# tchamp1912/Spittle

Measured on AMD Instinct MI355X. Metric: RTFx (audio-sec/wall-sec) Whisper-large-v3 30s chunks @1/2/4/8 MI355X, higher is better.
Workload: dtype bf16; 1 GPU; whisper-large-v3 30s chunks, batch 8/GPU, greedy en, 4-token prompt + 128 decode steps, host PCM in, text out; model=synthetic:large-v3, global_batch=8, seq_len=1500, decode_steps=128, parallelism=replicas x1 (utterance shards)

## Files before the change

include/spittle_hip.h:

```cpp
#ifndef SPITTLE_HIP_H
#define SPITTLE_HIP_H

#include <stddef.h>
#include <stdint.h>

#ifdef __cplusplus
extern "C" {
#endif

#define SPT_ABI_VERSION 14

typedef enum {
    SPT_OK = 0,
    SPT_ERR_INVALID_ARG = 1,
    SPT_ERR_LOAD = 2,
    SPT_ERR_DEVICE = 3,
    SPT_ERR_OOM = 4,
    SPT_ERR_UNSUPPORTED = 5,
    SPT_ERR_INTERNAL = 6
} spt_status;

typedef enum {
    SPT_DTYPE_F32 = 0, SPT_DTYPE_BF16 = 1,
    SPT_DTYPE_F16 = 2 ,
// ... 28 lines not shown
    const int32_t* prompt_tokens;
    int32_t n_prompt_tokens;
    float temperature_inc;
    int32_t best_of;
    float entropy_thold;
    float logprob_thold;
    float max_initial_ts;
    int32_t reserved0;
    uint64_t seed;
} spt_infer_params;

typedef struct {
    int64_t t0, t1;
    char* text;
    int32_t i0, n_tokens;
} spt_segment;

typedef struct {
    char* text;
    int32_t* tokens;
    float* top1;
    float* top2;
    int32_t n_tokens;
    int32_t n_windows;
    int32_t language;
    int32_t n_segments;
    spt_segment* segments;
    int32_t n_fallbacks;
    int32_t reserved0;
} spt_result;

typedef struct {
    int32_t n_mels, d, n_head, n_enc, n_dec, n_vocab, n_audio_ctx, n_text_ctx;
    int32_t dtype, max_batch;
    int64_t weight_bytes;
    int64_t workspace_bytes;
} spt_model_info;

typedef struct {
    double mel_ms, encoder_ms, cross_kv_ms, decode_ms, total_ms, h2d_ms;
    int32_t n_decode_passes;
    int32_t batch;
} spt_timings;

typedef struct spt_ctx spt_ctx;

const char* spt_version(void);
void spt_default_model_params(spt_model_params* p);
void spt_default_infer_params(spt_infer_params* p);

spt_status spt_ctx_create(const char* model_spec, const spt_model_params* params, spt_ctx** out,
                          char* err, size_t errlen);
void spt_ctx_destroy(spt_ctx* ctx);
const char* spt_last_error(const spt_ctx* ctx);
spt_status spt_ctx_info(const spt_ctx* ctx, spt_model_info* info);

spt_status spt_transcribe(spt_ctx* ctx, const float* pcm16k, size_t n_samples, const spt_infer_params* params,
                          spt_result** out);
spt_status spt_transcribe_batch(spt_ctx* ctx, const float* const* pcm, const size_t* n_samples, size_t batch,
                                const spt_infer_params* params, spt_result** out);
spt_status spt_transcribe_batch_device(spt_ctx* ctx, const float* pcm_dev, size_t stride, const size_t* n_samples,
                                       size_t batch, const spt_infer_params* params, spt_result** out);
void spt_result_free(spt_result* r);
const char* spt_language_code(int32_t lang_id);

spt_status spt_tokenize(spt_ctx* ctx, const char* text, int32_t* tokens, int32_t n_max, int32_t* n_out);
const char* spt_token_to_str(const spt_ctx* ctx, int32_t id);

spt_status spt_get_timings(const spt_ctx* ctx, spt_timings* t);

typedef struct {
    int32_t engine_calls;
    int32_t decoder_passes;
    int32_t beam_steps;
    int32_t encoder_windows;
    double device_ms;
    double encoder_ms;
    double decode_ms;
    int32_t pd_passes;
    int32_t pd_fallbacks;
} spt_call_stats;

spt_status spt_get_call_stats(const spt_ctx* ctx, spt_call_stats* s);

spt_status spt_weights_export(spt_ctx* ctx, void* dev_dst, size_t bytes);
spt_status spt_weights_import(spt_ctx* ctx, const void* dev_src, size_t bytes);
spt_status spt_weights_arena(spt_ctx* ctx, void** dev_ptr, size_t* bytes);
spt_status spt_weights_commit(spt_ctx* ctx);

spt_status spt_ctx_create_replicas(const char* model_spec, const spt_model_params* params, const int32_t* devices,
                                   int32_t n_devices, spt_ctx** out, double* bcast_ms, char* err, size_t errlen);
spt_status spt_transcribe_batch_replicas(spt_ctx* const* ctxs, int32_t n_ctx, const float* const* pcm,
                                         const size_t* n_samples, size_t batch, const spt_infer_params* params,
                                         spt_result** out);

typedef enum {
    SPT_PROBE_DEC_CROSS_ATTN = 0,
    SPT_PROBE_DEC_SELF_ATTN = 1,
    SPT_PROBE_DEC_LOGITS = 2,
    SPT_PROBE_DEC_FC1 = 3,
    SPT_PROBE_ENC_FC1_GEMM = 4,
    SPT_PROBE_ENC_ATTN = 5
} spt_probe_kind;
spt_status spt_probe_kernel(spt_ctx* ctx, int32_t kind, int32_t iters, double* avg_us, double* work,
                            int32_t* work_is_flops);

spt_status spt_debug_mel(spt_ctx* ctx, const float* pcm16k, size_t n_samples, float* out);
spt_status spt_debug_mel_at(spt_ctx* ctx, const float* pcm16k, size_t n_samples, int32_t seek, float* out);
spt_status spt_debug_encode(spt_ctx* ctx, const float* mel, float* out);
spt_status spt_debug_weight_checksum(spt_ctx* ctx, int32_t tensor_id, double* out2);
spt_status spt_debug_ggml_tokenize(const char* model_path, const char* text, int32_t* tokens, int32_t n_max,
                                   int32_t* n_out);
spt_status spt_debug_ggml_dequant(int32_t ggml_type, const void* src, int64_t n, float* dst);

typedef struct spt_pk_ctx spt_pk_ctx;

typedef struct {
    int32_t dtype;
    int32_t device;
    int32_t max_batch;
    float max_seconds;
    uint64_t seed;
    uint32_t flags;
    int32_t reserved0;
} spt_pk_model_params;

#define SPT_PK_WEIGHTS_EMPTY 1u

typedef enum { SPT_PK_TS_TOKEN = 0, SPT_PK_TS_WORD = 1, SPT_PK_TS_SEGMENT = 2 } spt_pk_granularity;

typedef struct {
    int32_t max_symbols;
    int32_t timestamp_granularity;
} spt_pk_infer_params;

typedef struct {
    double start, end;
    char* text;
    int32_t i0, n_tokens;
} spt_pk_segment;

typedef struct {
    char* text;
    int32_t* tokens;
    int32_t* frames;
    float* logit;
    float* runner_up;
    int32_t n_tokens;
    int32_t n_segments;
    spt_pk_segment* segments;
    int32_t n_chunks;
    int32_t reserved0;
} spt_pk_result;

typedef struct {
    int32_t n_mels, d, n_layers, n_heads, ff, sub_ch, conv_k, pred, n_vocab, n_dur;
    int32_t dtype, max_batch, max_samples, reserved0;
    int64_t weight_bytes, workspace_bytes;
} spt_pk_model_info;

typedef struct {
    double mel_ms, encoder_ms, decode_ms, total_ms, h2d_ms;
    int32_t n_steps;
    int32_t batch;
    int32_t enc_frames;
    int32_t reserved0;
// ... 236 lines not shown
```

rust/spittle-hip-sys/src/lib.rs:

```rust
#![allow(non_camel_case_types)]

use std::os::raw::{c_char, c_int, c_void};

pub const SPT_ABI_VERSION: c_int = 14;
pub const SPT_PK_STAGE_COUNT: c_int = 9;

pub type spt_status = c_int;
pub const SPT_OK: spt_status = 0;
pub const SPT_ERR_INVALID_ARG: spt_status = 1;
pub const SPT_ERR_LOAD: spt_status = 2;
pub const SPT_ERR_DEVICE: spt_status = 3;
pub const SPT_ERR_OOM: spt_status = 4;
pub const SPT_ERR_UNSUPPORTED: spt_status = 5;
pub const SPT_ERR_INTERNAL: spt_status = 6;

pub type spt_dtype = c_int;
pub const SPT_DTYPE_F32: spt_dtype = 0;
pub const SPT_DTYPE_BF16: spt_dtype = 1;
pub const SPT_DTYPE_F16: spt_dtype = 2;
pub const SPT_DTYPE_I8: spt_dtype = 3;
pub const SPT_PK_ACT_NONE: i32 = 0;
pub const SPT_PK_ACT_RELU: i32 = 1;
pub const SPT_PK_ACT_SWISH: i32 = 2;

// ... 94 lines not shown
    pub pd_fallbacks: i32,
}

#[repr(C)]
#[derive(Clone, Copy, Debug, Default)]
pub struct spt_timings {
    pub mel_ms: f64,
    pub encoder_ms: f64,
    pub cross_kv_ms: f64,
    pub decode_ms: f64,
    pub total_ms: f64,
    pub h2d_ms: f64,
    pub n_decode_passes: i32,
    pub batch: i32,
}

#[repr(C)]
pub struct spt_ctx {
    _private: [u8; 0],
}

pub type spt_probe_kind = c_int;
pub const SPT_PROBE_DEC_CROSS_ATTN: spt_probe_kind = 0;
pub const SPT_PROBE_DEC_SELF_ATTN: spt_probe_kind = 1;
pub const SPT_PROBE_DEC_LOGITS: spt_probe_kind = 2;
pub const SPT_PROBE_DEC_FC1: spt_probe_kind = 3;
pub const SPT_PROBE_ENC_FC1_GEMM: spt_probe_kind = 4;
pub const SPT_PROBE_ENC_ATTN: spt_probe_kind = 5;

extern "C" {
    pub fn spt_version() -> *const c_char;
    pub fn spt_default_model_params(p: *mut spt_model_params);
    pub fn spt_default_infer_params(p: *mut spt_infer_params);

    pub fn spt_ctx_create(
        model_spec: *const c_char,
        params: *const spt_model_params,
        out: *mut *mut spt_ctx,
        err: *mut c_char,
        errlen: usize,
    ) -> spt_status;
    pub fn spt_ctx_destroy(ctx: *mut spt_ctx);
    pub fn spt_last_error(ctx: *const spt_ctx) -> *const c_char;
    pub fn spt_ctx_info(ctx: *const spt_ctx, info: *mut spt_model_info) -> spt_status;

    pub fn spt_transcribe(
        ctx: *mut spt_ctx,
        pcm16k: *const f32,
        n_samples: usize,
        params: *const spt_infer_params,
        out: *mut *mut spt_result,
    ) -> spt_status;
    pub fn spt_transcribe_batch(
        ctx: *mut spt_ctx,
        pcm: *const *const f32,
        n_samples: *const usize,
        batch: usize,
        params: *const spt_infer_params,
        out: *mut *mut spt_result,
    ) -> spt_status;
    pub fn spt_transcribe_batch_device(
        ctx: *mut spt_ctx,
        pcm_dev: *const f32,
        stride: usize,
        n_samples: *const usize,
        batch: usize,
        params: *const spt_infer_params,
        out: *mut *mut spt_result,
    ) -> spt_status;
    pub fn spt_result_free(r: *mut spt_result);
    pub fn spt_language_code(lang_id: i32) -> *const c_char;

    pub fn spt_tokenize(
        ctx: *mut spt_ctx,
        text: *const c_char,
        tokens: *mut i32,
        n_max: i32,
        n_out: *mut i32,
    ) -> spt_status;
    pub fn spt_token_to_str(ctx: *const spt_ctx, id: i32) -> *const c_char;

    pub fn spt_get_timings(ctx: *const spt_ctx, t: *mut spt_timings) -> spt_status;
    pub fn spt_get_call_stats(ctx: *const spt_ctx, s: *mut spt_call_stats) -> spt_status;

    pub fn spt_weights_export(ctx: *mut spt_ctx, dev_dst: *mut c_void, bytes: usize) -> spt_status;
    pub fn spt_weights_import(ctx: *mut spt_ctx, dev_src: *const c_void, bytes: usize) -> spt_status;
    pub fn spt_weights_arena(ctx: *mut spt_ctx, dev_ptr: *mut *mut c_void, bytes: *mut usize) -> spt_status;
    pub fn spt_weights_commit(ctx: *mut spt_ctx) -> spt_status;

    pub fn spt_ctx_create_replicas(
        model_spec: *const c_char,
        params: *const spt_model_params,
        devices: *const i32,
        n_devices: i32,
        out: *mut *mut spt_ctx,
        bcast_ms: *mut f64,
        err: *mut c_char,
        errlen: usize,
    ) -> spt_status;
    pub fn spt_transcribe_batch_replicas(
        ctxs: *const *mut spt_ctx,
        n_ctx: i32,
        pcm: *const *const f32,
        n_samples: *const usize,
        batch: usize,
        params: *const spt_infer_params,
        out: *mut *mut spt_result,
    ) -> spt_status;

    pub fn spt_probe_kernel(
        ctx: *mut spt_ctx,
        kind: i32,
        iters: i32,
        avg_us: *mut f64,
        work: *mut f64,
        work_is_flops: *mut i32,
    ) -> spt_status;

    pub fn spt_debug_mel(ctx: *mut spt_ctx, pcm16k: *const f32, n_samples: usize, out: *mut f32) -> spt_status;
    pub fn spt_debug_mel_at(ctx: *mut spt_ctx, pcm16k: *const f32, n_samples: usize, seek: i32, out: *mut f32) -> spt_status;
    pub fn spt_debug_encode(ctx: *mut spt_ctx, mel: *const f32, out: *mut f32) -> spt_status;
    pub fn spt_debug_weight_checksum(ctx: *mut spt_ctx, tensor_id: i32, out2: *mut f64) -> spt_status;
    pub fn spt_debug_ggml_tokenize(
        model_path: *const c_char,
        text: *const c_char,
        tokens: *mut i32,
        n_max: i32,
        n_out: *mut i32,
    ) -> spt_status;
    pub fn spt_debug_ggml_dequant(ggml_type: i32, src: *const c_void, n: i64, dst: *mut f32) -> spt_status;

    pub fn spt_parakeet_default_model_params(p: *mut spt_pk_model_params);
    pub fn spt_parakeet_default_infer_params(p: *mut spt_pk_infer_params);
    pub fn spt_parakeet_create(
        model_spec: *const c_char,
        params: *const spt_pk_model_params,
        out: *mut *mut spt_pk_ctx,
        err: *mut c_char,
        errlen: usize,
    ) -> spt_status;
    pub fn spt_parakeet_destroy(ctx: *mut spt_pk_ctx);
    pub fn spt_parakeet_last_error(ctx: *const spt_pk_ctx) -> *const c_char;
    pub fn spt_parakeet_info(ctx: *const spt_pk_ctx, info: *mut spt_pk_model_info) -> spt_status;
    pub fn spt_parakeet_tensor_numel(ctx: *const spt_pk_ctx, tensor_id: i32, n: *mut i64) -> spt_status;
    pub fn spt_parakeet_set_tensor(ctx: *mut spt_pk_ctx, tensor_id: i32, data: *const f32, n: i64) -> spt_status;
    pub fn spt_parakeet_set_vocab(ctx: *mut spt_pk_ctx, pieces: *const *const c_char, n: i32) -> spt_status;
    pub fn spt_parakeet_transcribe(
        ctx: *mut spt_pk_ctx,
        pcm16k: *const f32,
        n_samples: usize,
        params: *const spt_pk_infer_params,
        out: *mut *mut spt_pk_result,
    ) -> spt_status;
    pub fn spt_parakeet_transcribe_batch(
        ctx: *mut spt_pk_ctx,
        pcm: *const *const f32,
        n_samples: *const usize,
        batch: usize,
        params: *const spt_pk_infer_params,
        out: *mut *mut spt_pk_result,
    ) -> spt_status;
    pub fn spt_parakeet_transcribe_batch_device(
        ctx: *mut spt_pk_ctx,
        pcm_dev: *const f32,
        stride: usize,
        n_samples: *const usize,
// ... 479 lines not shown
```

spittle_amd/_lib.py:

```python
from __future__ import annotations

import ctypes as C
import os

HERE = os.path.dirname(os.path.abspath(__file__))
LIB_PATH = os.path.join(HERE, "libspittle_hip.so")

SPT_OK, SPT_ERR_INVALID_ARG, SPT_ERR_LOAD, SPT_ERR_DEVICE, SPT_ERR_OOM, SPT_ERR_UNSUPPORTED, SPT_ERR_INTERNAL = range(7)
STATUS_NAMES = {0: "OK", 1: "INVALID_ARG", 2: "LOAD", 3: "DEVICE", 4: "OOM", 5: "UNSUPPORTED", 6: "INTERNAL"}
SPT_DTYPE_F32, SPT_DTYPE_BF16, SPT_DTYPE_F16, SPT_DTYPE_I8 = 0, 1, 2, 3
SPT_SUPPRESS_BLANK, SPT_NO_TIMESTAMPS, SPT_IGNORE_EOT, SPT_SUPPRESS_NST = 1, 2, 4, 8

EXPORTS = [
    "spt_version", "spt_default_model_params", "spt_default_infer_params", "spt_ctx_create",
    "spt_ctx_destroy", "spt_last_error", "spt_ctx_info", "spt_transcribe", "spt_transcribe_batch",
    "spt_transcribe_batch_device", "spt_result_free", "spt_get_timings", "spt_get_call_stats", "spt_debug_mel",
    "spt_debug_mel_at", "spt_debug_encode", "spt_debug_weight_checksum", "spt_probe_kernel", "spt_language_code",
    "spt_tokenize", "spt_token_to_str", "spt_debug_ggml_tokenize", "spt_debug_ggml_dequant",
    "spt_weights_export", "spt_weights_import", "spt_weights_arena", "spt_weights_commit",
    "spt_ctx_create_replicas", "spt_transcribe_batch_replicas",
    "spt_parakeet_default_model_params", "spt_parakeet_default_infer_params", "spt_parakeet_create",
    "spt_parakeet_destroy", "spt_parakeet_last_error", "spt_parakeet_info", "spt_parakeet_tensor_numel",
    "spt_parakeet_set_tensor", "spt_parakeet_set_vocab", "spt_parakeet_transcribe", "spt_parakeet_transcribe_batch",
    "spt_parakeet_transcribe_batch_device", "spt_parakeet_result_free", "spt_parakeet_get_timings",
    "spt_parakeet_debug_mel", "spt_parakeet_debug_encode", "spt_parakeet_debug_decode", "spt_parakeet_debug_last_encoder",
    "spt_parakeet_debug_weight_checksum", "spt_parakeet_onnx_open", "spt_parakeet_onnx_tensor",
    "spt_parakeet_onnx_piece", "spt_parakeet_onnx_close",
    "spt_resampler_create", "spt_resampler_info", "spt_resample_output_len", "spt_resample",
    "spt_resampler_last_error", "spt_resampler_destroy",
    "spt_vad_default_params", "spt_vad_create", "spt_vad_push", "spt_vad_result_free", "spt_vad_reset",
    "spt_vad_last_error", "spt_vad_destroy",
    "spt_parakeet_profile_encoder",
    "spt_parakeet_onnx_qtensor", "spt_parakeet_debug_qgemm", "spt_parakeet_debug_tap", "spt_parakeet_debug_tap_read",
    "spt_moonshine_default_model_params", "spt_moonshine_default_infer_params", "spt_moonshine_create",
    "spt_moonshine_destroy", "spt_moonshine_last_error", "spt_moonshine_info", "spt_moonshine_tensor_numel",
    "spt_moonshine_set_tensor", "spt_moonshine_missing_tensors", "spt_moonshine_set_vocab", "spt_moonshine_transcribe",
    "spt_moonshine_transcribe_batch", "spt_moonshine_result_free", "spt_moonshine_get_timings",
    "spt_moonshine_debug_stem", "spt_moonshine_debug_encode", "spt_moonshine_debug_logits",
    "spt_sensevoice_default_model_params", "spt_sensevoice_default_infer_params", "spt_sensevoice_create",
    "spt_sensevoice_destroy", "spt_sensevoice_last_error", "spt_sensevoice_info", "spt_sensevoice_tensor_numel",
    "spt_sensevoice_set_tensor", "spt_sensevoice_missing_tensors", "spt_sensevoice_set_cmvn",
    "spt_sensevoice_set_vocab", "spt_sensevoice_n_rows", "spt_sensevoice_transcribe",
    "spt_sensevoice_transcribe_batch", "spt_sensevoice_result_free", "spt_sensevoice_get_timings",
    "spt_sensevoice_debug_features", "spt_sensevoice_debug_encode", "spt_sensevoice_debug_frames",
]
SPT_SV_LANG_AUTO, SPT_SV_LANG_ZH, SPT_SV_LANG_EN, SPT_SV_LANG_YUE, SPT_SV_LANG_JA, SPT_SV_LANG_KO = range(6)
SPT_PK_WEIGHTS_EMPTY = 1
SPT_PK_TS_TOKEN, SPT_PK_TS_WORD, SPT_PK_TS_SEGMENT = 0, 1, 2
SPT_MODEL_WEIGHTS_EXTERNAL = 1
PK_STAGES = ("subsampling", "pos", "layernorm", "ffn", "qkv_out", "attn", "conv_pw", "conv_dw", "joint_enc")
PROBES = {"dec_cross_attn": 0, "dec_self_attn": 1, "dec_logits": 2, "dec_fc1": 3, "enc_fc1_gemm": 4,
          "enc_attn": 5}


class ModelParams(C.Structure):
    _fields_ = [("dtype", C.c_int32), ("device", C.c_int32), ("max_batch", C.c_int32),
                ("flags", C.c_uint32), ("seed", C.c_uint64)]


class InferParams(C.Structure):
    _fields_ = [("language", C.c_char_p), ("translate", C.c_int32), ("initial_prompt", C.c_char_p),
                ("flags", C.c_uint32), ("max_new_tokens", C.c_int32), ("temperature", C.c_float),
                ("beam_size", C.c_int32), ("forced_tokens", C.POINTER(C.c_int32)), ("n_forced", C.c_int32),
                ("prompt_tokens", C.POINTER(C.c_int32)), ("n_prompt_tokens", C.c_int32),
                ("temperature_inc", C.c_float), ("best_of", C.c_int32), ("entropy_thold", C.c_float),
                ("logprob_thold", C.c_float), ("max_initial_ts", C.c_float), ("reserved0", C.c_int32),
                ("seed", C.c_uint64)]


class Segment(C.Structure):
    _fields_ = [("t0", C.c_int64), ("t1", C.c_int64), ("text", C.c_char_p), ("i0", C.c_int32),
                ("n_tokens", C.c_int32)]


class Result(C.Structure):
    _fields_ = [("text", C.c_char_p), ("tokens", C.POINTER(C.c_int32)), ("top1", C.POINTER(C.c_float)),
                ("top2", C.POINTER(C.c_float)), ("n_tokens", C.c_int32), ("n_windows", C.c_int32),
                ("language", C.c_int32), ("n_segments", C.c_int32), ("segments", C.POINTER(Segment)),
                ("n_fallbacks", C.c_int32), ("reserved0", C.c_int32)]


class ModelInfo(C.Structure):
    _fields_ = [(n, C.c_int32) for n in ("n_mels", "d", "n_head", "n_enc", "n_dec", "n_vocab", "n_audio_ctx",
                                          "n_text_ctx", "dtype", "max_batch")] + \
               [("weight_bytes", C.c_int64), ("workspace_bytes", C.c_int64)]


class Timings(C.Structure):
    _fields_ = [(n, C.c_double) for n in ("mel_ms", "encoder_ms", "cross_kv_ms", "decode_ms", "total_ms",
                                           "h2d_ms")] + [("n_decode_passes", C.c_int32), ("batch", C.c_int32)]


class CallStats(C.Structure):
    _fields_ = [(n, C.c_int32) for n in ("engine_calls", "decoder_passes", "beam_steps", "encoder_windows")] + \
               [(n, C.c_double) for n in ("device_ms", "encoder_ms", "decode_ms")] + \
               [(n, C.c_int32) for n in ("pd_passes", "pd_fallbacks")]


class PkModelParams(C.Structure):
# ... 53 lines not shown
    _fields_ = [(n, C.c_double) for n in ("stem_ms", "encoder_ms", "cross_kv_ms", "decode_ms", "total_ms")] + \
               [("n_steps", C.c_int32), ("batch", C.c_int32)]


class SvModelParams(C.Structure):
    _fields_ = [("dtype", C.c_int32), ("device", C.c_int32), ("max_batch", C.c_int32), ("max_samples", C.c_int32),
                ("seed", C.c_uint64), ("ln_eps", C.c_float), ("sanm_shift", C.c_int32), ("lfr_m", C.c_int32),
                ("lfr_n", C.c_int32), ("blank_id", C.c_int32), ("n_prefix", C.c_int32), ("lang_rows", C.c_int32 * 6),
                ("event_row", C.c_int32), ("emo_row", C.c_int32), ("itn_row", C.c_int32), ("no_itn_row", C.c_int32)]


class SvInferParams(C.Structure):
    _fields_ = [("language", C.c_int32), ("use_itn", C.c_int32)]


class SvResult(C.Structure):
    _fields_ = [("text", C.c_char_p), ("tokens", C.POINTER(C.c_int32)), ("frames", C.POINTER(C.c_int32)),
                ("top1", C.POINTER(C.c_float)), ("top2", C.POINTER(C.c_float)), ("n_tokens", C.c_int32),
                ("prefix", C.c_int32 * 4)]


class SvModelInfo(C.Structure):
    _fields_ = [(n, C.c_int32) for n in ("d", "n_heads", "head_dim", "ff", "n_enc0_layers", "n_enc_layers",
                                          "n_tp_layers", "n_vocab", "input_dim", "dtype", "max_batch",
                                          "max_samples", "max_rows", "reserved")] + \
               [("weight_bytes", C.c_int64), ("workspace_bytes", C.c_int64)]


class SvTimings(C.Structure):
    _fields_ = [(n, C.c_double) for n in ("frontend_ms", "encoder_ms", "ctc_ms", "total_ms")] + \
               [("rows", C.c_int32), ("batch", C.c_int32)]


class VadParams(C.Structure):
    _fields_ = [("threshold", C.c_float), ("prefill_frames", C.c_int32), ("hangover_frames", C.c_int32),
                ("onset_frames", C.c_int32), ("device", C.c_int32), ("reserved0", C.c_int32)]


class VadResult(C.Structure):
    _fields_ = [("samples", C.POINTER(C.c_float)), ("n_samples", C.c_size_t), ("prob", C.POINTER(C.c_float)),
                ("kind", C.POINTER(C.c_uint8)), ("n_frames", C.c_int32), ("reserved0", C.c_int32),
                ("device_ms", C.c_double)]


_lib = None


def load():
    global _lib
    if _lib is not None:
        return _lib
    path = LIB_PATH
    if os.environ.get("SPT_DEBUG_LIB"):
        path = os.path.join(os.path.dirname(LIB_PATH), "libspittle_hip_dbg.so")
    if not os.path.exists(path):
        raise ImportError(f"spittle_amd: HIP library not built: {path} (run `make -C spittle_amd/csrc`)")
    L = C.CDLL(path)
    vp, fp = C.c_void_p, C.POINTER(C.c_float)
    L.spt_version.restype = C.c_char_p
    L.spt_default_model_params.argtypes = [C.POINTER(ModelParams)]
    L.spt_default_infer_params.argtypes = [C.POINTER(InferParams)]
    L.spt_ctx_create.argtypes = [C.c_char_p, C.POINTER(ModelParams), C.POINTER(vp), C.c_char_p, C.c_size_t]
    L.spt_ctx_create.restype = C.c_int
    L.spt_ctx_destroy.argtypes = [vp]
    L.spt_last_error.argtypes = [vp]
    L.spt_last_error.restype = C.c_char_p
    L.spt_ctx_info.argtypes = [vp, C.POINTER(ModelInfo)]
    L.spt_transcribe.argtypes = [vp, fp, C.c_size_t, C.POINTER(InferParams), C.POINTER(C.POINTER(Result))]
    L.spt_transcribe_batch.argtypes = [vp, C.POINTER(fp), C.POINTER(C.c_size_t), C.c_size_t,
                                       C.POINTER(InferParams), C.POINTER(C.POINTER(Result))]
    L.spt_transcribe_batch_device.argtypes = [vp, C.c_void_p, C.c_size_t, C.POINTER(C.c_size_t), C.c_size_t,
                                              C.POINTER(InferParams), C.POINTER(C.POINTER(Result))]
    L.spt_result_free.argtypes = [C.POINTER(Result)]
    L.spt_language_code.argtypes = [C.c_int32]
    L.spt_language_code.restype = C.c_char_p
    ip = C.POINTER(C.c_int32)
    L.spt_tokenize.argtypes = [vp, C.c_char_p, ip, C.c_int32, ip]
    L.spt_token_to_str.argtypes = [vp, C.c_int32]
    L.spt_token_to_str.restype = C.c_char_p
    L.spt_debug_ggml_tokenize.argtypes = [C.c_char_p, C.c_char_p, ip, C.c_int32, ip]
    L.spt_debug_ggml_dequant.argtypes = [C.c_int32, C.c_void_p, C.c_int64, fp]
    L.spt_get_timings.argtypes = [vp, C.POINTER(Timings)]
    L.spt_get_call_stats.argtypes = [vp, C.POINTER(CallStats)]
    L.spt_debug_mel.argtypes = [vp, fp, C.c_size_t, fp]
    L.spt_debug_mel_at.argtypes = [vp, fp, C.c_size_t, C.c_int32, fp]
    L.spt_debug_encode.argtypes = [vp, fp, fp]
    L.spt_debug_weight_checksum.argtypes = [vp, C.c_int32, C.POINTER(C.c_double)]
    L.spt_probe_kernel.argtypes = [vp, C.c_int32, C.c_int32, C.POINTER(C.c_double), C.POINTER(C.c_double),
                                   C.POINTER(C.c_int32)]
    L.spt_weights_export.argtypes = [vp, C.c_void_p, C.c_size_t]
    L.spt_weights_import.argtypes = [vp, C.c_void_p, C.c_size_t]
    L.spt_weights_arena.argtypes = [vp, C.POINTER(vp), C.POINTER(C.c_size_t)]
    L.spt_weights_commit.argtypes = [vp]
    L.spt_ctx_create_replicas.argtypes = [C.c_char_p, C.POINTER(ModelParams), C.POINTER(C.c_int32), C.c_int32,
                                          C.POINTER(vp), C.POINTER(C.c_double), C.c_char_p, C.c_size_t]
    L.spt_transcribe_batch_replicas.argtypes = [C.POINTER(vp), C.c_int32, C.POINTER(fp), C.POINTER(C.c_size_t),
                                                C.c_size_t, C.POINTER(InferParams), C.POINTER(C.POINTER(Result))]
    PR = C.POINTER(C.POINTER(PkResult))
    L.spt_parakeet_default_model_params.argtypes = [C.POINTER(PkModelParams)]
    L.spt_parakeet_default_infer_params.argtypes = [C.POINTER(PkInferParams)]
    L.spt_parakeet_create.argtypes = [C.c_char_p, C.POINTER(PkModelParams), C.POINTER(vp), C.c_char_p, C.c_size_t]
    L.spt_parakeet_onnx_open.argtypes = [C.c_char_p, C.POINTER(vp), C.POINTER(PkModelInfo), C.c_char_p, C.c_size_t]
    L.spt_parakeet_onnx_tensor.restype = C.c_int64
    L.spt_parakeet_onnx_tensor.argtypes = [vp, C.c_int32, C.POINTER(C.POINTER(C.c_float))]
    L.spt_parakeet_onnx_qtensor.restype = C.c_int64
    L.spt_parakeet_onnx_qtensor.argtypes = [vp, C.c_int32, C.POINTER(C.POINTER(C.c_int16)), C.POINTER(fp),
                                            C.POINTER(C.POINTER(C.c_int32)), C.POINTER(C.c_int32)]
    L.spt_parakeet_onnx_piece.restype = C.c_char_p
    L.spt_parakeet_onnx_piece.argtypes = [vp, C.c_int32]
    L.spt_parakeet_onnx_close.argtypes = [vp]
    L.spt_parakeet_destroy.argtypes = [vp]
    L.spt_parakeet_last_error.argtypes = [vp]
    L.spt_parakeet_last_error.restype = C.c_char_p
    L.spt_parakeet_info.argtypes = [vp, C.POINTER(PkModelInfo)]
    L.spt_parakeet_tensor_numel.argtypes = [vp, C.c_int32, C.POINTER(C.c_int64)]
    L.spt_parakeet_set_tensor.argtypes = [vp, C.c_int32, fp, C.c_int64]
    L.spt_parakeet_set_vocab.argtypes = [vp, C.POINTER(C.c_char_p), C.c_int32]
    L.spt_parakeet_transcribe.argtypes = [vp, fp, C.c_size_t, C.POINTER(PkInferParams), PR]
    L.spt_parakeet_transcribe_batch.argtypes = [vp, C.POINTER(fp), C.POINTER(C.c_size_t), C.c_size_t,
                                                C.POINTER(PkInferParams), PR]
    L.spt_parakeet_transcribe_batch_device.argtypes = [vp, C.c_void_p, C.c_size_t, C.POINTER(C.c_size_t), C.c_size_t,
                                                       C.POINTER(PkInferParams), PR]
    L.spt_parakeet_result_free.argtypes = [C.POINTER(PkResult)]
    L.spt_parakeet_get_timings.argtypes = [vp, C.POINTER(PkTimings)]
    L.spt_parakeet_profile_encoder.argtypes = [vp, C.c_int32, C.POINTER(C.c_double), C.c_int32]
    L.spt_parakeet_debug_mel.argtypes = [vp, fp, C.c_size_t, fp]
    L.spt_parakeet_debug_encode.argtypes = [vp, fp, C.c_int32, fp]
    L.spt_parakeet_debug_decode.argtypes = [vp, fp, C.c_int32, C.c_int32, PR]
    L.spt_parakeet_debug_last_encoder.argtypes = [vp, C.c_int32, fp, C.POINTER(C.c_int32)]
    L.spt_parakeet_debug_weight_checksum.argtypes = [vp, C.c_int32, C.POINTER(C.c_double)]
    i32p = C.POINTER(C.c_int32)
    L.spt_parakeet_debug_qgemm.argtypes = [C.c_int32, fp, C.c_int32, C.c_int32, i32p, C.c_int32, C.POINTER(C.c_int16),
                                           C.c_int32, fp, i32p, C.c_int32, fp, C.c_int32, C.POINTER(C.c_uint8), fp, i32p,
                                           i32p, fp, C.c_char_p, C.c_size_t]
    L.spt_parakeet_debug_tap.argtypes = [vp, C.c_int32]
    L.spt_parakeet_debug_tap_read.argtypes = [vp, i32p, fp, C.c_int64, fp, C.c_int64]
    L.spt_resampler_create.argtypes = [C.c_int32, C.c_int32, C.c_int32, C.c_int32, C.POINTER(vp), C.c_char_p,
                                       C.c_size_t]
    L.spt_resampler_create.restype = C.c_int
    L.spt_resampler_info.argtypes = [vp, C.POINTER(C.c_int32), C.POINTER(C.c_int32)]
    L.spt_resampler_info.restype = C.c_int
    L.spt_resample_output_len.argtypes = [vp, C.c_size_t]
    L.spt_resample_output_len.restype = C.c_size_t
    L.spt_resample.argtypes = [vp, fp, C.c_size_t, fp, C.c_size_t, C.POINTER(C.c_size_t)]
    L.spt_resample.restype = C.c_int
    L.spt_resampler_last_error.argtypes = [vp]
    L.spt_resampler_last_error.restype = C.c_char_p
    L.spt_resampler_destroy.argtypes = [vp]
    L.spt_resampler_destroy.restype = None
    L.spt_vad_default_params.argtypes = [C.POINTER(VadParams)]
    L.spt_vad_default_params.restype = None
    L.spt_vad_create.argtypes = [C.c_char_p, C.POINTER(VadParams), C.POINTER(vp), C.c_char_p, C.c_size_t]
    L.spt_vad_create.restype = C.c_int
    L.spt_vad_push.argtypes = [vp, fp, C.c_size_t, C.POINTER(C.POINTER(VadResult))]
    L.spt_vad_push.restype = C.c_int
    L.spt_vad_result_free.argtypes = [C.POINTER(VadResult)]
    L.spt_vad_result_free.restype = None
    L.spt_vad_reset.argtypes = [vp, C.c_int32]
    L.spt_vad_reset.restype = C.c_int
    L.spt_vad_last_error.argtypes = [vp]
    L.spt_vad_last_error.restype = C.c_char_p
    L.spt_vad_destroy.argtypes = [vp]
    L.spt_vad_destroy.restype = None
    MR = C.POINTER(C.POINTER(MsResult))
    L.spt_moonshine_default_model_params.argtypes = [C.POINTER(MsModelParams)]
    L.spt_moonshine_default_model_params.restype = None
    L.spt_moonshine_default_infer_params.argtypes = [C.POINTER(MsInferParams)]
    L.spt_moonshine_default_infer_params.restype = None
    L.spt_moonshine_create.argtypes = [C.c_char_p, C.POINTER(MsModelParams), C.POINTER(vp), C.c_char_p, C.c_size_t]
    L.spt_moonshine_destroy.argtypes = [vp]
    L.spt_moonshine_destroy.restype = None
    L.spt_moonshine_last_error.argtypes = [vp]
    L.spt_moonshine_last_error.restype = C.c_char_p
    L.spt_moonshine_info.argtypes = [vp, C.POINTER(MsModelInfo)]
    L.spt_moonshine_tensor_numel.argtypes = [vp, C.c_char_p, C.POINTER(C.c_int64)]
    L.spt_moonshine_set_tensor.argtypes = [vp, C.c_char_p, fp, C.c_int64]
    L.spt_moonshine_missing_tensors.argtypes = [vp]
    L.spt_moonshine_missing_tensors.restype = C.c_int32
    L.spt_moonshine_set_vocab.argtypes = [vp, C.POINTER(C.c_char_p), C.c_int32]
    L.spt_moonshine_transcribe.argtypes = [vp, fp, C.c_size_t, C.POINTER(MsInferParams), MR]
    L.spt_moonshine_transcribe_batch.argtypes = [vp, C.POINTER(fp), C.POINTER(C.c_size_t), C.c_size_t,
                                                 C.POINTER(MsInferParams), MR]
    L.spt_moonshine_result_free.argtypes = [C.POINTER(MsResult)]
    L.spt_moonshine_result_free.restype = None
    L.spt_moonshine_get_timings.argtypes = [vp, C.POINTER(MsTimings)]
    L.spt_moonshine_debug_stem.argtypes = [vp, fp, C.c_size_t, fp]
    L.spt_moonshine_debug_encode.argtypes = [vp, fp, C.c_size_t, fp]
    L.spt_moonshine_debug_logits.argtypes = [vp, fp, C.c_size_t, i32p, C.c_int32, fp]
    for fn in ("spt_moonshine_create", "spt_moonshine_info", "spt_moonshine_tensor_numel", "spt_moonshine_set_tensor",
               "spt_moonshine_set_vocab", "spt_moonshine_transcribe", "spt_moonshine_transcribe_batch",
               "spt_moonshine_get_timings", "spt_moonshine_debug_stem", "spt_moonshine_debug_encode",
               "spt_moonshine_debug_logits"):
        getattr(L, fn).restype = C.c_int
    SR = C.POINTER(C.POINTER(SvResult))
    svip = C.POINTER(SvInferParams)
    L.spt_sensevoice_default_model_params.argtypes = [C.POINTER(SvModelParams)]
    L.spt_sensevoice_default_model_params.restype = None
    L.spt_sensevoice_default_infer_params.argtypes = [svip]
    L.spt_sensevoice_default_infer_params.restype = None
    L.spt_sensevoice_create.argtypes = [C.c_char_p, C.POINTER(SvModelParams), C.POINTER(vp), C.c_char_p, C.c_size_t]
    L.spt_sensevoice_destroy.argtypes = [vp]
    L.spt_sensevoice_destroy.restype = None
    L.spt_sensevoice_last_error.argtypes = [vp]
    L.spt_sensevoice_last_error.restype = C.c_char_p
    L.spt_sensevoice_info.argtypes = [vp, C.POINTER(SvModelInfo)]
    L.spt_sensevoice_tensor_numel.argtypes = [vp, C.c_char_p, C.POINTER(C.c_int64)]
    L.spt_sensevoice_set_tensor.argtypes = [vp, C.c_char_p, fp, C.c_int64]
    L.spt_sensevoice_missing_tensors.argtypes = [vp]
    L.spt_sensevoice_missing_tensors.restype = C.c_int32
    L.spt_sensevoice_set_cmvn.argtypes = [vp, fp, fp, C.c_int32]
    L.spt_sensevoice_set_vocab.argtypes = [vp, C.POINTER(C.c_char_p), C.c_int32]
    L.spt_sensevoice_n_rows.argtypes = [vp, C.c_size_t]
    L.spt_sensevoice_n_rows.restype = C.c_int32
    L.spt_sensevoice_transcribe.argtypes = [vp, fp, C.c_size_t, svip, SR]
    L.spt_sensevoice_transcribe_batch.argtypes = [vp, C.POINTER(fp), C.POINTER(C.c_size_t), C.c_size_t, svip, SR]
    L.spt_sensevoice_result_free.argtypes = [C.POINTER(SvResult)]
    L.spt_sensevoice_result_free.restype = None
    L.spt_sensevoice_get_timings.argtypes = [vp, C.POINTER(SvTimings)]
    L.spt_sensevoice_debug_features.argtypes = [vp, fp, C.c_size_t, fp]
    L.spt_sensevoice_debug_encode.argtypes = [vp, fp, C.c_size_t, svip, fp]
    L.spt_sensevoice_debug_frames.argtypes = [vp, fp, C.c_size_t, svip, i32p, fp, fp]
    for fn in ("spt_sensevoice_create", "spt_sensevoice_info", "spt_sensevoice_tensor_numel", "spt_sensevoice_set_tensor",
               "spt_sensevoice_set_cmvn", "spt_sensevoice_set_vocab", "spt_sensevoice_transcribe",
               "spt_sensevoice_transcribe_batch", "spt_sensevoice_get_timings", "spt_sensevoice_debug_features",
               "spt_sensevoice_debug_encode", "spt_sensevoice_debug_frames"):
        getattr(L, fn).restype = C.c_int
    for fn in EXPORTS:
        if fn.startswith("spt_parakeet_") and fn not in ("spt_parakeet_default_model_params",
                                                          "spt_parakeet_default_infer_params", "spt_parakeet_destroy",
                                                          "spt_parakeet_last_error", "spt_parakeet_result_free",
                                                          "spt_parakeet_onnx_tensor", "spt_parakeet_onnx_piece",
                                                          "spt_parakeet_onnx_close", "spt_parakeet_onnx_qtensor"):
            getattr(L, fn).restype = C.c_int
    for fn in ("spt_weights_arena", "spt_weights_commit", "spt_ctx_create_replicas", "spt_transcribe_batch_replicas",
               "spt_weights_export", "spt_weights_import", "spt_ctx_info", "spt_transcribe", "spt_transcribe_batch", "spt_transcribe_batch_device",
               "spt_get_timings", "spt_get_call_stats", "spt_debug_mel", "spt_debug_mel_at", "spt_debug_encode", "spt_debug_weight_checksum",
               "spt_probe_kernel", "spt_tokenize", "spt_debug_ggml_tokenize", "spt_debug_ggml_dequant"):
        getattr(L, fn).restype = C.c_int
    _lib = L
    return L
```

spittle_amd/csrc/capi.cpp:

```cpp
#include <hip/hip_runtime.h>
#include <string.h>

#include <algorithm>
#include <memory>
#include <new>
#include <string>
#include <vector>

#include "../../include/spittle_hip.h"
#include "common.h"
#include "engine.h"
#include "full.h"
#include "ggml_file.h"
#include "vocab.h"

using spt::Engine;

#include "capi_internal.h"

namespace {

constexpr int kWindow = 480000;

void set_err(char* buf, size_t len, const std::string& msg) {
// ... 495 lines not shown
        std::vector<int> ns(batch);
        if (autolang) {
            rq.lang_tok.resize(batch);
            for (size_t b = 0; b < batch; ++b) rq.lang_tok[b] = -(int)(b + 1);
        }
        for (size_t b = 0; b < batch; ++b) {
            if (n_samples[b] > (size_t)kWindow) return fail(ctx, SPT_ERR_INVALID_ARG, "device windows hold <= 480000 samples");
            ns[b] = (int)n_samples[b];
        }
        Engine& e = *ctx->eng;
        const int B = (int)batch;
        std::vector<int> otok((size_t)B * rq.n_steps), lang(B, -1);
        std::vector<float> o1((size_t)B * rq.n_steps), o2((size_t)B * rq.n_steps);
        e.transcribe_device(pcm_dev, (int64_t)stride, ns.data(), B, rq, otok.data(), o1.data(), o2.data(), lang.data());
        const spt::Specials sp = spt::specials_for(e.dims().n_vocab);
        const int eot = sp.eot;
        for (int b = 0; b < B; ++b) {
            std::vector<int> t; std::vector<float> a, c2; std::string txt;
            for (int s2 = 0; s2 < rq.n_steps; ++s2) {
                const int tk = otok[(size_t)b * rq.n_steps + s2];
                if (tk < 0) break;
                t.push_back(tk);
                a.push_back(o1[(size_t)b * rq.n_steps + s2]);
                c2.push_back(o2[(size_t)b * rq.n_steps + s2]);
                if (tk < eot) append_text(ctx, &txt, tk);
                if (tk == eot && !(rq.flags & SPT_IGNORE_EOT)) break;
            }
            out[b] = make_result(1, lang_index(lang[b], sp), &t, &a, &c2, &txt);
        }
        return SPT_OK;
    } catch (const std::exception& e) {
        return fail(ctx, classify(e), e.what());
    }
}

void spt_result_free(spt_result* r) {
    if (!r) return;
    for (int32_t i = 0; i < r->n_segments && r->segments; ++i) free(r->segments[i].text);
    free(r->segments);
    free(r->text);
    free(r->tokens);
    free(r->top1);
    free(r->top2);
    free(r);
}

spt_status spt_tokenize(spt_ctx* ctx, const char* text, int32_t* tokens, int32_t n_max, int32_t* n_out) {
    if (!ctx || !text || !n_out || (n_max > 0 && !tokens)) return fail(ctx, SPT_ERR_INVALID_ARG, "null argument");
    if (!ctx->vocab) return fail(ctx, SPT_ERR_UNSUPPORTED, "synthetic models have no vocabulary");
    try {
        const std::vector<int> t = ctx->vocab->tokenize(text, nullptr);
        *n_out = (int32_t)t.size();
        if ((int64_t)t.size() > n_max) return fail(ctx, SPT_ERR_INVALID_ARG, "token buffer too small");
        for (size_t i = 0; i < t.size(); ++i) tokens[i] = t[i];
        return SPT_OK;
    } catch (const std::exception& e) {
        return fail(ctx, classify(e), e.what());
    }
}

const char* spt_token_to_str(const spt_ctx* ctx, int32_t id) {
    if (!ctx || !ctx->vocab || id < 0 || id >= ctx->vocab->size()) return nullptr;
    return ctx->vocab->str(id).c_str();
}

spt_status spt_get_timings(const spt_ctx* ctx, spt_timings* t) {
    if (!ctx || !t) return SPT_ERR_INVALID_ARG;
    const spt::Timings& m = ctx->eng->timings();
    t->mel_ms = m.mel_ms; t->encoder_ms = m.encoder_ms; t->cross_kv_ms = m.cross_kv_ms; t->decode_ms = m.decode_ms;
    t->total_ms = m.total_ms; t->h2d_ms = m.h2d_ms; t->n_decode_passes = m.n_decode_passes; t->batch = m.batch;
    return SPT_OK;
}

spt_status spt_get_call_stats(const spt_ctx* ctx, spt_call_stats* s) {
    if (!ctx || !s) return SPT_ERR_INVALID_ARG;
    const spt::CallStats& c = ctx->eng->call_stats();
    s->engine_calls = c.engine_calls; s->decoder_passes = c.decoder_passes; s->beam_steps = c.beam_steps;
    s->encoder_windows = c.encoder_windows;
    s->device_ms = c.device_ms; s->encoder_ms = c.encoder_ms; s->decode_ms = c.decode_ms;
    s->pd_passes = c.pd_passes; s->pd_fallbacks = c.pd_fallbacks;
    return SPT_OK;
}

spt_status spt_weights_export(spt_ctx* ctx, void* dev_dst, size_t bytes) {
    if (!ctx || !dev_dst) return fail(ctx, SPT_ERR_INVALID_ARG, "null argument");
    try {
        ctx->eng->export_weights(dev_dst, (int64_t)bytes);
        return SPT_OK;
    } catch (const std::exception& e) {
        return fail(ctx, classify(e), e.what());
    }
}

spt_status spt_weights_import(spt_ctx* ctx, const void* dev_src, size_t bytes) {
    if (!ctx || !dev_src) return fail(ctx, SPT_ERR_INVALID_ARG, "null argument");
    try {
        ctx->eng->import_weights(dev_src, (int64_t)bytes);
        return SPT_OK;
    } catch (const std::exception& e) {
        return fail(ctx, classify(e), e.what());
    }
}

spt_status spt_debug_mel(spt_ctx* ctx, const float* pcm16k, size_t n_samples, float* out) {
    if (!ctx || !out || (n_samples && !pcm16k)) return fail(ctx, SPT_ERR_INVALID_ARG, "null argument");
    if (n_samples > (size_t)kWindow) return fail(ctx, SPT_ERR_INVALID_ARG, "window longer than 30 s");
    return spt_debug_mel_at(ctx, pcm16k, n_samples, 0, out);
}

spt_status spt_debug_mel_at(spt_ctx* ctx, const float* pcm16k, size_t n_samples, int32_t seek, float* out) {
    if (!ctx || !out || (n_samples && !pcm16k)) return fail(ctx, SPT_ERR_INVALID_ARG, "null argument");
    if (n_samples > (size_t)INT32_MAX / 2) return fail(ctx, SPT_ERR_INVALID_ARG, "utterance too long");
    try {
        ctx->eng->debug_mel(pcm16k, (int)n_samples, seek, out);
        return SPT_OK;
    } catch (const std::exception& e) {
        return fail(ctx, classify(e), e.what());
    }
}

spt_status spt_debug_encode(spt_ctx* ctx, const float* mel, float* out) {
    if (!ctx || !mel || !out) return fail(ctx, SPT_ERR_INVALID_ARG, "null argument");
    try {
        ctx->eng->debug_encode(mel, out);
        return SPT_OK;
    } catch (const std::exception& e) {
        return fail(ctx, classify(e), e.what());
    }
}

spt_status spt_debug_weight_checksum(spt_ctx* ctx, int32_t tensor_id, double* out2) {
    if (!ctx || !out2) return fail(ctx, SPT_ERR_INVALID_ARG, "null argument");
    try {
        if (!ctx->eng->debug_weight_checksum(tensor_id, out2)) return fail(ctx, SPT_ERR_INVALID_ARG, "unknown tensor id");
        return SPT_OK;
    } catch (const std::exception& e) {
        return fail(ctx, classify(e), e.what());
    }
}

spt_status spt_debug_ggml_tokenize(const char* model_path, const char* text, int32_t* tokens, int32_t n_max,
                                   int32_t* n_out) {
    if (!model_path || !text || !n_out || (n_max > 0 && !tokens)) return SPT_ERR_INVALID_ARG;
    spt::GgmlFile f;
    std::string err;
    if (!f.open(model_path, &err)) return SPT_ERR_LOAD;
    spt::Vocab v(f.vocab(), f.hparams().n_vocab, spt::specials_for(f.hparams().n_vocab));
    const std::vector<int> t = v.tokenize(text, nullptr);
    *n_out = (int32_t)t.size();
    if ((int64_t)t.size() > n_max) return SPT_ERR_INVALID_ARG;
    for (size_t i = 0; i < t.size(); ++i) tokens[i] = t[i];
    return SPT_OK;
}

spt_status spt_debug_ggml_dequant(int32_t ggml_type, const void* src, int64_t n, float* dst) {
    if (!src || !dst || n < 0) return SPT_ERR_INVALID_ARG;
    int blck, bytes;
    spt::GgmlFile::type_block(ggml_type, &blck, &bytes);
    if (!blck) return SPT_ERR_UNSUPPORTED;
    if (n % blck) return SPT_ERR_INVALID_ARG;
    return spt::ggml_dequant_host(ggml_type, (const uint8_t*)src, n, dst) ? SPT_OK : SPT_ERR_UNSUPPORTED;
}

}

extern "C" spt_status spt_probe_kernel(spt_ctx* ctx, int32_t kind, int32_t iters, double* avg_us, double* work,
// ... 12 lines not shown
```

spittle_amd/csrc/dec_attn.h:

```cpp
#pragma once
#include "common.h"

namespace spt {
namespace {

constexpr int AW = 8;
constexpr float kLog2Scale = 0.125f * 1.4426950408889634f;

template <typename T> struct KVChunk;
template <> struct KVChunk<bf16> {
    bf16x8 v;
    __device__ __forceinline__ void load(const bf16* p) { v = *(const bf16x8*)p; }
    __device__ __forceinline__ float at(int e) const { return bf2f((bf16)v[e]); }
};
template <> struct KVChunk<f16> {
    f16x8 v;
    __device__ __forceinline__ void load(const f16* p) { v = *(const f16x8*)p; }
    __device__ __forceinline__ float at(int e) const { return (float)v[e]; }
};
template <> struct KVChunk<float> {
    f32x4 a, b;
    __device__ __forceinline__ void load(const float* p) { a = *(const f32x4*)p; b = *(const f32x4*)(p + 4); }
    __device__ __forceinline__ float at(int e) const { return e < 4 ? a[e] : b[e - 4]; }
};
// ... 47 lines not shown
                for (int e = 0; e < 8; ++e) v = __builtin_fmaf(qv[t][e], kc[i].at(e), v);
                v += __shfl_xor(v, 1, 64);
                v += __shfl_xor(v, 2, 64);
                v += __shfl_xor(v, 4, 64);
                if (kbase + 8 * i + slot >= lim[t]) v = -INFINITY;
                s[i] = v;
                mb = fmaxf(mb, v);
            }
            mb = fmaxf(mb, __shfl_xor(mb, 8, 64));
            mb = fmaxf(mb, __shfl_xor(mb, 16, 64));
            mb = fmaxf(mb, __shfl_xor(mb, 32, 64));
            if (mb == -INFINITY) continue;
            const float mn = fmaxf(m[t], mb);
            const float alpha = exp2f(m[t] - mn);
            float ls = 0.f;
#pragma unroll
            for (int e = 0; e < 8; ++e) o[t][e] *= alpha;
#pragma unroll
            for (int i = 0; i < NI; ++i) {
                const float p = exp2f(s[i] - mn);
                ls += p;
#pragma unroll
                for (int e = 0; e < 8; ++e) o[t][e] = __builtin_fmaf(p, vc[i].at(e), o[t][e]);
            }
            l[t] = __builtin_fmaf(l[t], alpha, ls);
            m[t] = mn;
        }
    }
    template <int MAXB>
    __device__ __forceinline__ void run(int blk, int nblk, const float (&qv)[NQ][8], const int (&lim)[NQ], int Tq) {
        if (blk >= nblk) return;
        const int cnt = (nblk - 1 - blk) / NW + 1;
        const int mine = blk + (cnt - 1) * NW;
        if (MAXB <= 8 && cnt <= MAXB) {
#pragma unroll
            for (int d = 0; d < PF - 1 && d < MAXB; ++d) load_blk(kc_[d], vc_[d], min(blk + d * NW, mine));
#pragma unroll
            for (int i = 0; i < (MAXB <= 8 ? MAXB : 1); ++i) {
                if (i >= cnt) break;
                if (i + PF - 1 < (MAXB <= 8 ? MAXB : 1))
                    load_blk(kc_[(i + PF - 1) % PF], vc_[(i + PF - 1) % PF], min(blk + (i + PF - 1) * NW, mine));
                process(kc_[i % PF], vc_[i % PF], (blk + i * NW) * KB, qv, lim, Tq);
            }
            return;
        }
        load_blk(kc_[0], vc_[0], blk);
        while (blk < nblk) {
            load_blk(kc_[1], vc_[1], min(blk + NW, mine));
            process(kc_[0], vc_[0], blk * KB, qv, lim, Tq);
            blk += NW;
            if (blk >= nblk) break;
            load_blk(kc_[0], vc_[0], min(blk + NW, mine));
            process(kc_[1], vc_[1], blk * KB, qv, lim, Tq);
            blk += NW;
        }
    }
    template <int MAXB>
    __device__ __forceinline__ void run_pre(int blk, int nblk, const float (&qv)[NQ][8], const int (&lim)[NQ], int Tq) {
        if (blk >= nblk) return;
        const int cnt = (nblk - 1 - blk) / NW + 1;
        const int mine = blk + (cnt - 1) * NW;
        if (MAXB <= 8 && cnt <= MAXB) {
#pragma unroll
            for (int d = 1; d < PF - 1 && d < MAXB; ++d) load_blk(kc_[d], vc_[d], min(blk + d * NW, mine));
#pragma unroll
            for (int i = 0; i < (MAXB <= 8 ? MAXB : 1); ++i) {
                if (i >= cnt) break;
                if (i + PF - 1 < (MAXB <= 8 ? MAXB : 1))
                    load_blk(kc_[(i + PF - 1) % PF], vc_[(i + PF - 1) % PF], min(blk + (i + PF - 1) * NW, mine));
                process(kc_[i % PF], vc_[i % PF], (blk + i * NW) * KB, qv, lim, Tq);
            }
            return;
        }
        while (blk < nblk) {
            load_blk(kc_[1], vc_[1], min(blk + NW, mine));
            process(kc_[0], vc_[0], blk * KB, qv, lim, Tq);
            blk += NW;
            if (blk >= nblk) break;
            load_blk(kc_[0], vc_[0], min(blk + NW, mine));
            process(kc_[1], vc_[1], blk * KB, qv, lim, Tq);
            blk += NW;
        }
    }
    __device__ __forceinline__ void to_lds(float (*s_m)[NQ], float (*s_l)[NQ], float (*s_o)[NQ][64], int wid,
                                           int lane) {
        const int g = lane & 7;
#pragma unroll
        for (int t = 0; t < NQ; ++t) {
            float lt = l[t];
            lt += __shfl_xor(lt, 8, 64);
            lt += __shfl_xor(lt, 16, 64);
            lt += __shfl_xor(lt, 32, 64);
#pragma unroll
            for (int e = 0; e < 8; ++e) {
                float v = o[t][e];
                v += __shfl_xor(v, 8, 64);
                v += __shfl_xor(v, 16, 64);
                v += __shfl_xor(v, 32, 64);
                o[t][e] = v;
            }
            if (lane < 8) {
#pragma unroll
                for (int e = 0; e < 8; ++e) s_o[wid][t][8 * g + e] = o[t][e];
            }
            if (lane == 0) {
                s_m[wid][t] = m[t];
                s_l[wid][t] = lt;
            }
        }
    }
};

template <int NQ, int NW = AW>
__device__ __forceinline__ void attn_merge(const float (*s_m)[NQ], const float (*s_l)[NQ], const float (*s_o)[NQ][64],
                                           int t, int e, float& M, float& L, float& O) {
#pragma clang fp contract(off)
    M = -INFINITY;
#pragma unroll
    for (int w = 0; w < NW; ++w) M = fmaxf(M, s_m[w][t]);
    L = 0.f;
    O = 0.f;
#pragma unroll
    for (int w = 0; w < NW; ++w) {
        if (s_m[w][t] == -INFINITY) continue;
        const float f = exp2f(s_m[w][t] - M);
        L = __builtin_fmaf(s_l[w][t], f, L);
        O = __builtin_fmaf(s_o[w][t][e], f, O);
    }
}

}
}
```

spittle_amd/csrc/engine.cpp:

```cpp
#include "engine.h"
#include "ggml_file.h"

#include <cstdio>

#include <math.h>
#include <string.h>

#include <algorithm>
#include <functional>
#include <cstdlib>
#include <sstream>
#include <stdexcept>

#include "common.h"

namespace spt {

bool parse_synthetic_spec(const std::string& spec, ModelDims* dm, uint64_t* seed, std::string* err) {
    const std::string pfx = "synthetic:";
    if (spec.compare(0, pfx.size(), pfx) != 0) return false;
    std::vector<std::string> parts;
    std::stringstream ss(spec.substr(pfx.size()));
    std::string tok;
    while (std::getline(ss, tok, ':')) parts.push_back(tok);
    if (parts.empty()) { *err = "empty synthetic spec"; return true; }
    struct Cfg { const char* name; int n_mels, d, h, ne, nd, V; };
    static const Cfg cfgs[] = {
        {"tiny.en", 80, 384, 6, 4, 4, 51864},     {"tiny", 80, 384, 6, 4, 4, 51865},
        {"base.en", 80, 512, 8, 6, 6, 51864},     {"base", 80, 512, 8, 6, 6, 51865},
        {"small.en", 80, 768, 12, 12, 12, 51864}, {"small", 80, 768, 12, 12, 12, 51865},
        {"medium.en", 80, 1024, 16, 24, 24, 51864}, {"medium", 80, 1024, 16, 24, 24, 51865},
        {"large-v3", 128, 1280, 20, 32, 32, 51866}, {"large-v3-turbo", 128, 1280, 20, 32, 4, 51866},
    };
    bool found = false;
    for (const Cfg& c : cfgs)
        if (parts[0] == c.name) {
            dm->name = c.name;
            dm->n_mels = c.n_mels; dm->d = c.d; dm->n_head = c.h; dm->n_enc = c.ne; dm->n_dec = c.nd;
            dm->n_vocab = c.V;
            found = true;
        }
    if (!found) { *err = "unknown synthetic model '" + parts[0] + "'"; return true; }
    for (size_t i = 1; i < parts.size(); ++i) {
        const std::string& p = parts[i];
        const size_t eq = p.find('=');
        if (eq == std::string::npos) { *err = "bad option '" + p + "'"; return true; }
        const std::string k = p.substr(0, eq), v = p.substr(eq + 1);
        char* end = nullptr;
        const unsigned long long x = strtoull(v.c_str(), &end, 10);
        if (!end || *end) { *err = "bad value in '" + p + "'"; return true; }
        if (k == "enc") dm->n_enc = (int)x;
        else if (k == "dec") dm->n_dec = (int)x;
        else if (k == "seed") *seed = (uint64_t)x;
        else { *err = "unknown option '" + k + "'"; return true; }
    }
    if (dm->n_enc < 0 || dm->n_dec < 1 || dm->n_enc > 64 || dm->n_dec > 64) *err = "layer count out of range";
    return true;
}

namespace {
int fanin_exp(int K) { return (int)floor(log2(sqrt(3.0 / (double)K)) + 0.5); }

struct Carver {
    char* base;
    int64_t off = 0;
    void* take(int64_t bytes) {
        off = (off + 255) & ~(int64_t)255;
        void* p = base ? base + off : nullptr;
        off += bytes;
        return p;
    }
};
}

void Engine::select() const { HIP_CHECK(hipSetDevice(dev_)); }

Engine::Engine(const ModelDims& dm, int dtype, int device, int max_batch, uint64_t seed, const GgmlFile* src,
               bool external_weights)
    : dm_(dm), dt_(dtype), dev_(device), max_batch_(max_batch), seed_(seed) {
    if (dm_.d % 128 || dm_.d / 64 != dm_.n_head) throw std::runtime_error("unsupported model width");
    if (max_batch_ < 1 || max_batch_ > 64) throw std::runtime_error("max_batch must be in 1..64");
    if (dt_ == DT_F32 && dm_.d > 1024)
        throw std::runtime_error("the f32 engine supports model widths up to 1024 (tiny..medium); load " +
                                 std::to_string(dm_.d) + "-wide models in bf16");
    if (dt_ != DT_F32 && dt_ != DT_BF16 && dt_ != DT_F16) throw std::runtime_error("unsupported engine dtype");
    esz_ = dtype_size(dt_);
    cp_ = ((dm_.n_mels + 63) / 64) * 64;
    if ((3 * cp_ * esz_) % 128) cp_ = ((dm_.n_mels + 127) / 128) * 128;
    if (const char* g = getenv("SPT_DECODE_GROUPS")) n_groups_ = std::max(1, std::min(4, atoi(g)));
    if (const char* v = getenv("SPT_XATTN_SPLIT")) xsplit_ = std::max(1, std::min(4, atoi(v)));
    select();
    HIP_CHECK(hipStreamCreateWithFlags(&st_, hipStreamNonBlocking));
    ev_.resize(12);
    for (auto& e : ev_) HIP_CHECK(hipEventCreate(&e));
    enc_st_.assign(kEncGroupsMax - 1, nullptr);
    for (auto& s : enc_st_) HIP_CHECK(hipStreamCreateWithFlags(&s, hipStreamNonBlocking));
    enc_ev_.assign(kEncGroupsMax, nullptr);
    for (auto& e : enc_ev_) HIP_CHECK(hipEventCreateWithFlags(&e, hipEventDisableTiming));
    max_rows_ = gemv_max_image_rows(dt_, dm_.d);
    groups_.resize(std::max(n_groups_, cdiv(max_batch_, max_rows_)));
    for (auto& g : groups_) {
        HIP_CHECK(hipStreamCreateWithFlags(&g.st, hipStreamNonBlocking));
        HIP_CHECK(hipEventCreateWithFlags(&g.ev, hipEventDisableTiming));
    }
    try {
        gemv_prepare(dt_);
        gemm_prepare();
        alloc_weights();
        if (external_weights) {
            HIP_CHECK(hipMemsetAsync(warena_, 0, wbytes_, st_));
        } else if (src) {
            load_ggml(*src);
        } else {
            generate_weights();
        }
        weights_ready_ = !external_weights;
        upload_tables(src ? &src->mel_filters() : nullptr);
        alloc_workspace();
        HIP_CHECK(hipStreamSynchronize(st_));
    } catch (...) {
        release();
        throw;
    }
}

Engine::~Engine() { release(); }

void Engine::release() {
    (void)hipSetDevice(dev_);
    if (st_) (void)hipStreamSynchronize(st_);
    for (auto& g : groups_) {
        if (g.st) (void)hipStreamSynchronize(g.st);
        for (auto& kv : g.graphs) (void)hipGraphExecDestroy(kv.second);
        if (g.ev) (void)hipEventDestroy(g.ev);
        if (g.st) (void)hipStreamDestroy(g.st);
    }
    for (auto& kv : enc_graphs_) (void)hipGraphExecDestroy(kv.second);
    enc_graphs_.clear();
    for (auto& s : enc_st_)
        if (s) {
            (void)hipStreamSynchronize(s);
            (void)hipStreamDestroy(s);
        }
    enc_st_.clear();
    for (auto& e : enc_ev_)
        if (e) (void)hipEventDestroy(e);
    enc_ev_.clear();
    if (warena_) (void)hipFree(warena_);
    if (aarena_) (void)hipFree(aarena_);
    if (kvtmp_) (void)hipFree(kvtmp_);
    for (void* p : {(void*)upcm_, (void*)umel_, (void*)uinfo_})
        if (p) (void)hipFree(p);
    upcm_ = umel_ = nullptr;
    uinfo_ = nullptr;
    upcm_cap_ = umel_cap_ = 0;
    uinfo_cap_ = 0;
    for (void* p : {(void*)hann_, (void*)sinv_, (void*)cosv_, (void*)filt_, (void*)grp_})
        if (p) (void)hipFree(p);
    for (auto& e : ev_) (void)hipEventDestroy(e);
    for (auto& e : probe_ev_) (void)hipEventDestroy(e);
    probe_ev_.clear();
    if (st_) (void)hipStreamDestroy(st_);
    groups_.clear();
    ev_.clear();
    warena_ = aarena_ = nullptr;
    kvtmp_ = nullptr;
    hann_ = sinv_ = cosv_ = filt_ = nullptr;
    grp_ = nullptr;
    st_ = nullptr;
}

void Engine::require_weights() const {
    if (!weights_ready_)
        throw std::runtime_error("weights not loaded: the context was created with SPT_MODEL_WEIGHTS_EXTERNAL and "
                                 "spt_weights_import has not been called");
}

void Engine::export_weights(void* dev_dst, int64_t bytes) {
    require_weights();
    if (!dev_dst || bytes != wbytes_)
        throw std::runtime_error("weight export: expected " + std::to_string(wbytes_) + " bytes, got " +
                                 std::to_string(bytes));
    select();
    HIP_CHECK(hipMemcpyAsync(dev_dst, warena_, (size_t)wbytes_, hipMemcpyDeviceToDevice, st_));
    HIP_CHECK(hipStreamSynchronize(st_));
}

void Engine::import_weights(const void* dev_src, int64_t bytes) {
    if (!dev_src || bytes != wbytes_)
        throw std::runtime_error("weight import: expected " + std::to_string(wbytes_) + " bytes (this model and dtype), got " +
                                 std::to_string(bytes));
    select();
    HIP_CHECK(hipMemcpyAsync(warena_, dev_src, (size_t)wbytes_, hipMemcpyDeviceToDevice, st_));
    HIP_CHECK(hipStreamSynchronize(st_));
    weights_ready_ = true;
}

void Engine::commit_weights() {
    select();
    HIP_CHECK(hipDeviceSynchronize());
    weights_ready_ = true;
}

void Engine::alloc_weights() {
    const int64_t d = dm_.d, dd = d * d, V = dm_.n_vocab, L = dm_.n_dec;
    enc_.resize(dm_.n_enc);
    dec_.resize(dm_.n_dec);
    for (int pass = 0; pass < 2; ++pass) {
        Carver c{pass ? warena_ : nullptr};
        auto W = [&](int64_t n) { return c.take(n * esz_); };
        auto F = [&](int64_t n) { return (float*)c.take(n * 4); };
        conv1_w_ = W(d * 3 * cp_); conv1_b_ = F(d);
        conv2_w_ = W(dd * 3); conv2_b_ = F(d);
        enc_pos_ = F((int64_t)dm_.n_audio_ctx * d);
        lnp_w_ = F(d); lnp_b_ = F(d);
        for (auto& e : enc_) {
// ... 255 lines not shown
void Engine::upload_tables(const std::vector<float>* filters) {
    std::vector<float> hann(400), sv(400), cv(400);
    for (int i = 0; i < 400; ++i) {
        const double theta = (2 * M_PI * i) / 400;
        sv[i] = sinf((float)theta);
        cv[i] = cosf((float)theta);
        hann[i] = (float)(0.5 * (1.0 - cosf((float)((2.0 * M_PI * i) / 400))));
    }
    const int nm = dm_.n_mels;
    auto hz2mel = [](double f) {
        const double lg = 27.0 / log(6.4);
        return f >= 1000.0 ? 15.0 + log(f / 1000.0) * lg : 3.0 * f / 200.0;
    };
    auto mel2hz = [](double m) {
        const double lg = log(6.4) / 27.0;
        return m >= 15.0 ? 1000.0 * exp(lg * (m - 15.0)) : 200.0 * m / 3.0;
    };
    std::vector<double> ff(nm + 2);
    const double mmin = hz2mel(0.0), mmax = hz2mel(8000.0);
    for (int i = 0; i < nm + 2; ++i) {
        double mm = mmin + (mmax - mmin) * i / (double)(nm + 1);
        if (i == nm + 1) mm = mmax;
        ff[i] = mel2hz(mm);
    }
    std::vector<float> filt((size_t)nm * 201);
    std::vector<int> grp(2 * nm);
    if (filters) filt = *filters;
    for (int j = 0; j < nm; ++j) {
        const double en = 2.0 / (ff[j + 2] - ff[j]);
        int lo = -1, hi = -1;
        for (int k = 0; k < 201; ++k) {
            if (!filters) {
                const double fk = 8000.0 * k / 200.0;
                const double down = -(ff[j] - fk) / (ff[j + 1] - ff[j]);
                const double up = (ff[j + 2] - fk) / (ff[j + 2] - ff[j + 1]);
                double v = std::min(down, up);
                if (v < 0) v = 0;
                filt[(size_t)j * 201 + k] = (float)(v * en);
            }
            const float fv = filt[(size_t)j * 201 + k];
            if (fv != 0.0f) {
                if (lo < 0) lo = k;
                hi = k;
            }
        }
        if (lo < 0) { grp[2 * j] = 0; grp[2 * j + 1] = 0; }
        else {
            grp[2 * j] = lo < 200 ? lo / 4 : 50;
            grp[2 * j + 1] = (hi < 200 ? hi / 4 : 50) + 1;
        }
    }
    HIP_CHECK(hipMalloc(&hann_, 400 * 4));
    HIP_CHECK(hipMalloc(&sinv_, 400 * 4));
    HIP_CHECK(hipMalloc(&cosv_, 400 * 4));
    HIP_CHECK(hipMalloc(&filt_, filt.size() * 4));
    HIP_CHECK(hipMalloc(&grp_, grp.size() * 4));
    HIP_CHECK(hipMemcpy(hann_, hann.data(), 1600, hipMemcpyHostToDevice));
    HIP_CHECK(hipMemcpy(sinv_, sv.data(), 1600, hipMemcpyHostToDevice));
    HIP_CHECK(hipMemcpy(cosv_, cv.data(), 1600, hipMemcpyHostToDevice));
    HIP_CHECK(hipMemcpy(filt_, filt.data(), filt.size() * 4, hipMemcpyHostToDevice));
    HIP_CHECK(hipMemcpy(grp_, grp.data(), grp.size() * 4, hipMemcpyHostToDevice));
}

void Engine::alloc_workspace() {
    const int64_t B = max_batch_, d = dm_.d, T = dm_.n_audio_ctx, L = dm_.n_dec, ctx = dm_.n_text_ctx;
    const int64_t V = dm_.n_vocab, R = B * 4;
    for (int pass = 0; pass < 2; ++pass) {
        Carver c{pass ? aarena_ : nullptr};
        auto A = [&](int64_t n) { return c.take(n * esz_); };
        win_utt_ = (int*)c.take(B * 4);
        win_seek_ = (int*)c.take(B * 4);
        mel_in_ = A(B * MEL_ROWS * cp_);
        y1p_ = A(B * MEL_ROWS * d);
        x_ = (float*)c.take(B * T * d * 4);
        xn_ = A(B * T * d);
        qkv_ = A(B * T * 3 * d);
        ao_ = A(B * T * d);
        ff_ = A(B * T * 4 * d);
        enc_out_ = A(B * T * d);
        ckv_ = A(L * kv_layer_elems((int)B, dm_.n_head, (int)T));
        suppress_ = (uint32_t*)c.take((V / 32 + 1) * 4);
        suppress_lang_ = (uint32_t*)c.take((V / 32 + 1) * 4);
        scratch_ = (double*)c.take(64);
        for (DecGroup& g : groups_) {
            g.dx = (float*)c.take(R * d * 4);
            g.dq = A(R * d);
            g.dao = A(R * d);
            g.dff = A(R * 4 * d);
            g.skv = A(L * 2 * B * ctx * d);
            g.logits = (float*)c.take(B * V * 4);
            g.part = c.take(B * ((V + 15) / 16) * 16);
            g.arrive = (unsigned*)c.take(64);
            g.tok_in = (int*)c.take(R * 4);
            g.out_tok = (int*)c.take(B * ctx * 4);
            g.out_t1 = (float*)c.take(B * ctx * 4);
            g.out_t2 = (float*)c.take(B * ctx * 4);
            g.done = (int*)c.take(B * 4);
            g.forced = (int*)c.take(B * ctx * 4);
            g.ds = (DecState*)c.take(sizeof(DecState));
            g.dx2 = (float*)c.take(R * d * 4);
            g.pend = (float*)c.take((int64_t)kMaxPend * R * d * 4);
            g.xpart = (float*)c.take((int64_t)R * dm_.n_head * 8 * 66 * 4);
            g.seek = (int*)c.take(B * 4);
            g.seek_end = (int*)c.take(B * 4);
            g.ts_state = (int*)c.take(B * 16);
            g.ts_stat = (float*)c.take((int64_t)B * TS_CHUNKS * 6 * 4);
            g.beam_stat = (float*)c.take((int64_t)B * TS_CHUNKS * BEAM_STAT * 4);
            g.prm = (TsParams*)c.take(sizeof(TsParams));
            g.beam_row = (int*)c.take(B * 16);
            g.beam_step = (int*)c.take(64);
            g.beam_src = (int*)c.take(B * 4);
            g.cand_id = (int*)c.take(B * 8 * 4);
            g.cand_lp = (float*)c.take(B * 8 * 4);
            g.beam_tid = (int*)c.take(B * 4);
            g.kvrow = (int*)c.take(B * 4);
        }
        zero_ = (float*)c.take(R * d * 4);
        if (!pass) {
            abytes_ = c.off;
            if (hipMalloc(&aarena_, abytes_) != hipSuccess) {
                aarena_ = nullptr;
                throw std::runtime_error("out of device memory for workspace (" + std::to_string(abytes_) + " B)");
            }
        }
    }
    HIP_CHECK(hipMemsetAsync(aarena_, 0, abytes_, st_));
}

void Engine::ensure_capacity(void** p, int64_t* cap, int64_t need, size_t esz, const char* what) {
    if (need <= *cap) return;
    const int64_t want = std::max<int64_t>(need, *cap + *cap / 4);
    HIP_CHECK(hipDeviceSynchronize());
    if (*p) HIP_CHECK(hipFree(*p));
    *p = nullptr;
    *cap = 0;
    if (hipMalloc(p, (size_t)want * esz) != hipSuccess) {
        *p = nullptr;
        (void)hipGetLastError();
        throw std::runtime_error(std::string("out of device memory for ") + what + " (" +
                                 std::to_string((size_t)want * esz) + " B)");
    }
    *cap = want;
}

void Engine::run_mel_utts(const float* pcm, const std::vector<int64_t>& pcm_off, const int* n, int U) {
    if (U < 1) throw std::runtime_error("no utterances");
    int64_t rows = 0;
    int max_rows = 0;
    uhost_.assign((size_t)U * 3, 0);
    for (int u = 0; u < U; ++u) {
        if (n[u] < 0) throw std::runtime_error("negative sample count");
        const int r = mel_rows(n[u]);
        uhost_[u] = pcm_off[u];
        uhost_[U + u] = rows;
        rows += r;
        max_rows = std::max(max_rows, r);
    }
    void* pm = umel_;
    ensure_capacity(&pm, &umel_cap_, std::max<int64_t>(rows, 1), (size_t)dm_.n_mels * 4, "the utterance log-mel");
    umel_ = (float*)pm;
    const int64_t info_bytes = (int64_t)U * 24;
    if (U > uinfo_cap_) {
        int64_t cap = uinfo_cap_ ? (int64_t)uinfo_cap_ * 24 : 0;
        void* pi = uinfo_;
        ensure_capacity(&pi, &cap, info_bytes, 1, "utterance descriptors");
        uinfo_ = (char*)pi;
        uinfo_cap_ = (int)(cap / 24);
    }
    mel_img_.assign((size_t)info_bytes, 0);
    memcpy(mel_img_.data(), uhost_.data(), (size_t)U * 16);
    for (int u = 0; u < U; ++u) memcpy(mel_img_.data() + (size_t)U * 16 + 4 * u, &n[u], 4);
    HIP_CHECK(hipMemcpyAsync(uinfo_, mel_img_.data(), (size_t)U * 20, hipMemcpyHostToDevice, st_));
    mu_.pcm_off = (const int64_t*)uinfo_;
    mu_.row_off = (const int64_t*)(uinfo_ + (size_t)U * 8);
    mu_.n = (const int*)(uinfo_ + (size_t)U * 16);
    umax_ = (unsigned*)(uinfo_ + (size_t)U * 20);
    un_.assign(n, n + U);
    HIP_CHECK(hipEventRecord(ev_[0], st_));
    MelTables t{hann_, sinv_, cosv_, filt_, grp_};
    mel_frames(pcm, mu_, U, max_rows, dm_.n_mels, t, umel_, umax_, st_);
    HIP_CHECK(hipEventRecord(ev_[1], st_));
    mel_pending_ = true;
    enc_E_ = 0;
}

void Engine::load_utterances(const float* const* pcm, const int* n, int U) {
    select();
    require_weights();
    std::vector<int64_t> off(U);
    int64_t tot = 0;
    for (int u = 0; u < U; ++u) {
        if (n[u] < 0) throw std::runtime_error("negative sample count");
        if (n[u] > 0 && !pcm[u]) throw std::runtime_error("null pcm");
        off[u] = tot;
        tot += n[u];
    }
    void* pp = upcm_;
    ensure_capacity(&pp, &upcm_cap_, std::max<int64_t>(tot, 1), 4, "utterance PCM");
// ... 110 lines not shown
    gemm_nt(dt_, EPI_BIAS_GELU_POS, g, B, st_);
    const int G = enc_groups(B);
    int b0[kEncGroupsMax + 1];
    for (int i = 0; i <= G; ++i) b0[i] = (int)((int64_t)B * i / G);
    auto stream_of = [&](int i) { return i == 0 ? st_ : enc_st_[i - 1]; };
    if (G > 1) {
        HIP_CHECK(hipEventRecord(enc_ev_[0], st_));
        for (int i = 1; i < G; ++i) HIP_CHECK(hipStreamWaitEvent(stream_of(i), enc_ev_[0], 0));
    }
    auto rows = [&](void* base, int64_t row, int64_t ld, int es) { return (char*)base + row * ld * es; };
    enc_groups_cur_ = G;
    for (int l = 0; l < dm_.n_enc; ++l)
        for (int i = 0; i < G; ++i)
            enc_layer(l, b0[i + 1] - b0[i], (int64_t)b0[i] * T, stream_of(i));
    for (int i = 0; i < G; ++i) {
        const int64_t r0 = (int64_t)b0[i] * T;
        layernorm(dt_, (float*)rows(x_, r0, d, 4), (b0[i + 1] - b0[i]) * T, d, lnp_w_, lnp_b_,
                  rows(enc_out_, r0, d, esz_), stream_of(i));
    }
    for (int i = 1; i < G; ++i) {
        HIP_CHECK(hipEventRecord(enc_ev_[i], stream_of(i)));
        HIP_CHECK(hipStreamWaitEvent(st_, enc_ev_[i], 0));
    }
}

int Engine::enc_groups(int B) const {
    int G = B >= 8 ? 2 : 1;
    if (const char* v = getenv("SPT_ENC_GROUPS")) G = atoi(v);
    return std::max(1, std::min({G, kEncGroupsMax, B}));
}

void Engine::enqueue_encoder(int B) {
    static const bool eager = getenv("SPT_NO_GRAPH") || (getenv("SPT_ENC_GRAPH") && atoi(getenv("SPT_ENC_GRAPH")) == 0);
    const std::pair<int, int> key{B, enc_groups(B)};
    if (eager || !enc_seen_.count(key)) {
        enc_seen_.insert(key);
        run_encoder(B);
        return;
    }
    auto it = enc_graphs_.find(key);
    if (it == enc_graphs_.end()) {
        hipGraph_t graph;
        HIP_CHECK(hipStreamBeginCapture(st_, hipStreamCaptureModeThreadLocal));
        try {
            run_encoder(B);
        } catch (...) {
            (void)hipStreamEndCapture(st_, &graph);
            throw;
        }
        HIP_CHECK(hipStreamEndCapture(st_, &graph));
        hipGraphExec_t exec;
        HIP_CHECK(hipGraphInstantiate(&exec, graph, nullptr, nullptr, 0));
        HIP_CHECK(hipGraphDestroy(graph));
        it = enc_graphs_.emplace(key, exec).first;
    }
    HIP_CHECK(hipGraphLaunch(it->second, st_));
}

void Engine::run_cross_kv(int B) {
    const int d = dm_.d, T = dm_.n_audio_ctx;
    GemmArgs g{};
    g.A = enc_out_; g.lda = d; g.W = ckv_w_; g.ldw = d; g.M = B * T; g.N = dm_.n_dec * 2 * d; g.K = d;
    g.bias = ckv_b_; g.C = ckv_; g.kv_B = B; g.kv_T = T; g.kv_H = dm_.n_head;
    gemm_nt(dt_, EPI_KVSPLIT, g, 1, st_);
}

void Engine::enqueue_decoder_pass(DecGroup& g, int E, int Tq, const DecodeRequest& rq, int out_cap) {
    float* x = enqueue_layers(g, E, Tq);
    enqueue_head(g, Tq, rq, out_cap, x, suppress_, (rq.flags & 1u) != 0);
}

float* Engine::enqueue_layers(DecGroup& g, int E, int Tq) {
    const int d = dm_.d, H = dm_.n_head, ctx = dm_.n_text_ctx, T = dm_.n_audio_ctx, B = g.B, R = B * Tq;
    const int64_t self_layer = (int64_t)2 * B * H * ctx * 64, cross_layer = kv_layer_elems(E, H, T);
    const bool mapped = g.share > 0;
    const int runs = B / std::max(1, g.share);
    const int vw_env = getenv("SPT_XATTN_VW") ? atoi(getenv("SPT_XATTN_VW")) : 1;
    const bool vw = vw_env == 2 || (vw_env != 0 && runs * H < 96);
    const bool per_query = vw && Tq == 1 && vw_env != 3;
    const bool vw_merge = vw && R > 1;
    const int xs = vw ? (vw_merge ? 1 : 8) : mapped ? 1 : xsplit_;
    const int ks = esz_ == 2 ? 128 : 64;
    hipStream_t st = g.st;
    float* xc = g.dx;
    float* xo = g.dx2;
    int np = 0;
    pend_fold_ = !getenv("SPT_DEC_XFOLD") || atoi(getenv("SPT_DEC_XFOLD")) != 0;
    auto ln_input = [&](GemvArgs& a) {
        ln_source(a, xc, g.pend, np, (int64_t)R * d);
        a.x_out = np > 0 ? xo : nullptr;
    };
    auto consumed = [&] {
        if (np > 0) std::swap(xc, xo);
        np = 0;
    };
    auto pmark = [&](int kind, int l, int which) {
        if (probe_kind_ == kind) HIP_CHECK(hipEventRecord(probe_ev_[2 * l + which], st));
    };
    auto partial = [&](GemvArgs& a, int split) {
        a.C = g.pend; a.ldc = d; a.c_split = (int64_t)R * d;
        a.ksplit = split;
        a.p_resid = pend_fold_ ? xc : nullptr;
        if (a.K / ks < split) throw std::runtime_error("decoder projection too narrow for its K split");
        np = split;
    };
    for (int l = 0; l < dm_.n_dec; ++l) {
        const DecL& e = dec_[l];
        void* skv_l = (char*)g.skv + self_layer * l * esz_;
        const void* ckv_l = (const char*)ckv_ + (cross_layer * l + (mapped ? 0 : (int64_t)g.b0 * H * 4096)) * esz_;
        {
            GemvArgs a{};
            ln_input(a); a.lda = d; a.ln_w = e.ln1_w; a.ln_b = e.ln1_b; a.R = R;
            a.W = e.qkv_w; a.N = 3 * d; a.K = d; a.bias = e.qkv_b; a.C = g.dq; a.ldc = d;
            a.cache = skv_l; a.cache_B = B; a.cache_H = H; a.cache_ctx = ctx; a.Tq = Tq; a.st = g.ds;
            gemv(dt_, GV_QKV_CACHE, A_LN, a, st);
            consumed();
            pmark(1, l, 0);
            dec_self_attn(dt_, g.dq, skv_l, B, H, ctx, Tq, g.ds, g.dao, st);
            pmark(1, l, 1);
        }
        GemvArgs a{};
        a.A = g.dao; a.lda = d; a.R = R; a.W = e.so_w; a.N = d; a.K = d; a.bias = e.so_b;
        a.C = xc; a.ldc = d;
        gemv(dt_, GV_BIAS_RESID, A_DIRECT, a, st);
        a = GemvArgs{};
        ln_input(a); a.lda = d; a.ln_w = e.ln2_w; a.ln_b = e.ln2_b; a.R = R;
        a.W = e.cq_w; a.N = d; a.K = d; a.bias = e.cq_b; a.C = g.dq; a.ldc = d;
        gemv(dt_, GV_BIAS, A_LN, a, st);
        consumed();
        pmark(0, l, 0);
        if (vw)
        {
            dec_cross_attn_vw(dt_, g.dq, ckv_l, B, E, H, T, Tq, g.xpart, st, mapped ? g.kvrow : nullptr,
                              mapped ? g.share : 1, per_query);
            if (vw_merge) dec_attn_part_merge(dt_, g.xpart, R, H, g.dao, st);
        }
        else
            dec_cross_attn(dt_, g.dq, ckv_l, B, E, H, T, Tq, g.dao, st, xs, g.xpart, mapped ? g.kvrow : nullptr,
                           mapped ? g.share : 1);
        pmark(0, l, 1);
        a = GemvArgs{};
        a.A = g.dao; a.lda = d; a.R = R; a.W = e.co_w; a.N = d; a.K = d; a.bias = e.co_b; a.C = xc; a.ldc = d;
        if (xs > 1) { a.apart = g.xpart; a.a_splits = xs; a.a_heads = H; }
        gemv(dt_, GV_BIAS_RESID, xs > 1 ? A_ATTN : A_DIRECT, a, st);
        a = GemvArgs{};
        ln_input(a); a.lda = d; a.ln_w = e.ln3_w; a.ln_b = e.ln3_b; a.R = R;
        a.W = e.fc1_w; a.N = 4 * d; a.K = d; a.bias = e.fc1_b; a.C = g.dff; a.ldc = 4 * d;
        pmark(3, l, 0);
        gemv(dt_, GV_BIAS_GELU, A_LN, a, st);
        pmark(3, l, 1);
        consumed();
        a = GemvArgs{};
        a.A = g.dff; a.lda = 4 * d; a.R = R; a.W = e.fc2_w; a.N = d; a.K = 4 * d; a.bias = e.fc2_b;
        partial(a, fc2_split_);
        gemv(dt_, GV_PARTIAL, A_DIRECT, a, st);
    }
    return xc;
}

void Engine::ln_source(GemvArgs& a, float* xc, float* pend, int np, int64_t slab) const {
    const int f = np > 0 && pend_fold_ ? 1 : 0;
    a.A = f ? pend : xc;
    for (int p = 0; p < kMaxPend; ++p) a.pend[p] = p < np - f ? pend + (int64_t)(p + f) * slab : zero_;
    a.n_pend = np - f;
}

void Engine::enqueue_head(DecGroup& g, int Tq, const DecodeRequest& rq, int out_cap, float* xc,
                          const uint32_t* sup, bool blank) {
    const int d = dm_.d, ctx = dm_.n_text_ctx, B = g.B, R = B * Tq;
    hipStream_t st = g.st;
    const Specials sp = specials_for(dm_.n_vocab);
    const int n_tiles = (dm_.n_vocab + 15) / 16;
    GemvArgs a{};
    ln_source(a, xc, g.pend, fc2_split_, (int64_t)R * d);
    a.lda = Tq * d; a.a_row0 = (Tq - 1) * d; a.ln_w = lnf_w_; a.ln_b = lnf_b_; a.R = B;
    a.W = tok_emb_; a.N = dm_.n_vocab; a.K = d; a.C = g.logits; a.ldc = dm_.n_vocab; a.st = g.ds;
    a.suppress = sup;
    a.blank0 = blank ? sp.eot : -1;
    a.blank1 = blank ? 220 : -1;
    a.part = g.part; a.n_tiles = n_tiles;
    gemv(dt_, GV_LOGITS, A_LN, a, st);
    if (rq.beam_k > 0) {
        BeamArgs bm{};
        bm.logits = g.logits; bm.ldl = dm_.n_vocab;
        bm.n_vocab = dm_.n_vocab; bm.eot = sp.eot; bm.beg = sp.beg; bm.blank = rq.blank_tok;
        bm.suppress = sup; bm.prm = g.prm; bm.row = g.beam_row; bm.step = g.beam_step; bm.k = rq.beam_k;
        bm.cand_id = g.cand_id; bm.cand_lp = g.cand_lp; bm.tid = g.beam_tid;
        static const bool one_wg = getenv("SPT_BEAM_ONE_WG") != nullptr;
        bm.stat = one_wg ? nullptr : g.beam_stat;
        dec_beam_topk(bm, B, st);
        dec_advance(g.ds, Tq, st);
        return;
    }
    if (rq.full) {
        TsArgs t{};
        t.logits = g.logits; t.ldl = dm_.n_vocab;
        t.n_vocab = dm_.n_vocab; t.eot = sp.eot; t.beg = sp.beg; t.blank = rq.blank_tok;
        t.suppress = sup; t.prm = g.prm; t.seek = g.seek; t.seek_end = g.seek_end; t.state = g.ts_state;
        t.forced = rq.n_forced > 0 ? g.forced : nullptr; t.forced_len = rq.n_forced;
        t.next_tok = g.tok_in; t.out_tok = g.out_tok; t.out_plog = g.out_t1; t.out_tid = g.out_t2; t.out_cap = out_cap;
        t.done = g.done;
        t.emb = tok_emb_; t.pos = dec_pos_; t.d = d; t.ctx = ctx; t.Tq = Tq; t.x = g.dx;
        t.ds = g.ds; t.arrive = g.arrive; t.stat = g.ts_stat;
        dec_ts_stats(t, B, st);
        dec_finalize_ts(dt_, t, B, st);
        return;
    }
    FinalizeArgs f{};
    f.part = g.part; f.n_tiles = n_tiles;
    f.eot = sp.eot; f.ignore_eot = (rq.flags & 4u) ? 1 : 0; f.n_vocab = dm_.n_vocab;
    f.forced = rq.n_forced > 0 ? g.forced : nullptr; f.forced_len = rq.n_forced;
    f.next_tok = g.tok_in; f.out_tok = g.out_tok; f.out_top1 = g.out_t1; f.out_top2 = g.out_t2; f.out_cap = out_cap;
    f.done = g.done;
    f.emb = tok_emb_; f.pos = dec_pos_; f.d = d; f.ctx = ctx; f.Tq = Tq; f.x = g.dx;
    f.ds = g.ds; f.arrive = g.arrive;
// ... 52 lines not shown
    const uint32_t sflags = (rq.flags & 2u) | (rq.full ? 0x100u : 0u);
    if (suppress_flags_ != sflags || suppress_extra_ != rq.extra_suppress) {
        const int V = dm_.n_vocab;
        host_suppress_.assign(V / 32 + 1, 0u);
        auto set = [&](int i) { if (i >= 0 && i < V) host_suppress_[i >> 5] |= 1u << (i & 31); };
        set(sp.not_);
        if ((rq.flags & 2u) && !rq.full)
            for (int i = sp.beg; i < V; ++i) set(i);
        set(sp.sot); set(sp.nosp); set(sp.solm); set(sp.translate); set(sp.transcribe); set(sp.prev);
        for (int i = 0; i < sp.n_langs; ++i) set(sp.sot + 1 + i);
        for (int i : rq.extra_suppress) set(i);
        HIP_CHECK(hipMemcpyAsync(suppress_, host_suppress_.data(), host_suppress_.size() * 4, hipMemcpyHostToDevice, st_));
        HIP_CHECK(hipStreamSynchronize(st_));
        suppress_flags_ = sflags;
        suppress_extra_ = rq.extra_suppress;
    }
    if (rq.full && ((int)rq.seek.size() != B || (int)rq.seek_end.size() != B))
        throw std::runtime_error("whisper_full decoding needs seek / seek_end per sequence");
    if (!rq.row_prefix.empty()) {
        if ((int)rq.row_prefix.size() != B) throw std::runtime_error("row_prefix needs one prefix per sequence");
        for (const auto& r : rq.row_prefix) {
            if (r.size() != rq.row_prefix[0].size()) throw std::runtime_error("row prefixes must have equal lengths");
            for (int t : r)
                if (t < 0 || t >= dm_.n_vocab) throw std::runtime_error("prompt token out of the vocabulary");
        }
    }
    HIP_CHECK(hipEventRecord(ev_[6], st_));
    std::vector<DecGroup*> act;
    kvrow_host_ = rq.kv_row;
    for (int gi = 0, b0 = 0; gi < G; ++gi) {
        DecGroup& g = groups_[gi];
        g.b0 = b0;
        g.B = (nU / G + (gi < nU % G ? 1 : 0)) * unit;
        g.share = S;
        b0 += g.B;
        act.push_back(&g);
        HIP_CHECK(hipStreamWaitEvent(g.st, ev_[6], 0));
        if (S > 0)
            HIP_CHECK(hipMemcpyAsync(g.kvrow, kvrow_host_.data() + g.b0, (size_t)g.B * 4, hipMemcpyHostToDevice, g.st));
        g.host_tok.assign((size_t)g.B * (P + Tq + 8), 0);
        g.host_used = 0;
        if (rq.n_forced > 0)
            HIP_CHECK(hipMemcpyAsync(g.forced, rq.forced + (size_t)g.b0 * rq.n_forced, (size_t)g.B * rq.n_forced * 4,
                                     hipMemcpyHostToDevice, g.st));
        if (rq.full) {
            HIP_CHECK(hipMemcpyAsync(g.seek, rq.seek.data() + g.b0, g.B * 4, hipMemcpyHostToDevice, g.st));
            HIP_CHECK(hipMemcpyAsync(g.seek_end, rq.seek_end.data() + g.b0, g.B * 4, hipMemcpyHostToDevice, g.st));
            HIP_CHECK(hipMemcpyAsync(g.prm, &rq.ts, sizeof(TsParams), hipMemcpyHostToDevice, g.st));
        }
    }
    auto upload_tokens = [&](DecGroup& g, const std::function<int(int, int)>& tok, int n) {
        int* h = g.host_tok.data() + g.host_used;
        for (int b = 0; b < g.B; ++b)
            for (int t = 0; t < n; ++t) h[b * n + t] = tok(g.b0 + b, t);
        g.host_used += g.B * n;
        HIP_CHECK(hipMemcpyAsync(g.tok_in, h, (size_t)g.B * n * 4, hipMemcpyHostToDevice, g.st));
    };
    ts_init_.clear();
    for (int b = 0; b < B; ++b) ts_init_.insert(ts_init_.end(), {0, 3000, 0, 0});
    auto reset_outputs = [&](DecGroup& g) {
        HIP_CHECK(hipMemsetAsync(g.done, 0, g.B * 4, g.st));
        HIP_CHECK(hipMemsetAsync(g.out_tok, 0xFF, (size_t)g.B * out_cap * 4, g.st));
        fill_f32(g.out_t1, (int64_t)g.B * out_cap, -INFINITY, g.st);
        fill_f32(g.out_t2, (int64_t)g.B * out_cap, -INFINITY, g.st);
        dec_reset(g.ds, g.arrive, g.st);
        if (rq.full)
            HIP_CHECK(hipMemcpyAsync(g.ts_state, ts_init_.data() + (size_t)g.b0 * 4, g.B * 16, hipMemcpyHostToDevice,
                                     g.st));
    };
    std::vector<int> lang(B, -1);
    bool detect = false;
    for (int v : rq.lang_tok) detect = detect || v < 0;
    if (detect) {
        if (sp.n_langs <= 0) throw std::runtime_error("language detection needs a multilingual model");
        if (!suppress_lang_ready_) {
            const int V = dm_.n_vocab;
            std::vector<uint32_t> m(V / 32 + 1, ~0u);
            for (int i = 0; i < sp.n_langs; ++i) m[(sp.sot + 1 + i) >> 5] &= ~(1u << ((sp.sot + 1 + i) & 31));
            HIP_CHECK(hipMemcpy(suppress_lang_, m.data(), m.size() * 4, hipMemcpyHostToDevice));
            suppress_lang_ready_ = true;
        }
        DecodeRequest dq;
        dq.flags = 4u;
        for (DecGroup* g : act) {
            reset_outputs(*g);
            upload_tokens(*g, [&](int, int) { return sp.sot; }, 1);
            dec_embed(dt_, g->tok_in, g->B, 1, dm_.d, tok_emb_, dec_pos_, g->ds, g->dx, g->st);
            float* x = enqueue_layers(*g, E, 1);
            enqueue_head(*g, 1, dq, out_cap, x, suppress_lang_, false);
        }
        std::vector<int> first((size_t)B * out_cap);
        for (DecGroup* g : act) {
            HIP_CHECK(hipMemcpyAsync(first.data() + (size_t)g->b0 * out_cap, g->out_tok, (size_t)g->B * out_cap * 4,
                                     hipMemcpyDeviceToHost, g->st));
            HIP_CHECK(hipStreamSynchronize(g->st));
        }
        for (int b = 0; b < B; ++b) {
            const int v = rq.lang_tok[b];
            lang[b] = v >= 0 ? v : first[(size_t)(-v - 1) * out_cap];
            if (lang[b] <= sp.sot || lang[b] > sp.sot + sp.n_langs) throw std::runtime_error("language detection failed");
        }
    } else if (!rq.lang_tok.empty()) {
        for (int b = 0; b < B; ++b) lang[b] = rq.lang_tok[b];
    }
    if (lang_out)
        for (int b = 0; b < B; ++b) lang_out[b] = lang[b] >= 0 ? lang[b] : (Tq >= 3 ? rq.prompt[1] : -1);
    for (DecGroup* gp : act) {
        DecGroup& g = *gp;
        reset_outputs(g);
        const bool rows = !rq.row_prefix.empty();
        const int P = rows ? (int)rq.row_prefix[0].size() : (int)rq.prefix.size();
        for (int c0 = 0; c0 < P; c0 += cmax) {
            const int n = std::min(cmax, P - c0);
            upload_tokens(g, [&](int b, int t) { return rows ? rq.row_prefix[b][c0 + t] : rq.prefix[c0 + t]; }, n);
            dec_embed(dt_, g.tok_in, g.B * n, n, dm_.d, tok_emb_, dec_pos_, g.ds, g.dx, g.st);
            enqueue_layers(g, E, n);
            dec_advance(g.ds, n, g.st);
        }
        auto prompt_tok = [&](int b, int t) { return (t == 1 && lang[b] >= 0) ? lang[b] : rq.prompt[t]; };
        for (int c0 = 0; c0 < Tq - Tq_head; c0 += cmax) {
            const int n = std::min(cmax, Tq - Tq_head - c0);
            upload_tokens(g, [&](int b, int t) { return prompt_tok(b, c0 + t); }, n);
            dec_embed(dt_, g.tok_in, g.B * n, n, dm_.d, tok_emb_, dec_pos_, g.ds, g.dx, g.st);
            enqueue_layers(g, E, n);
            dec_advance(g.ds, n, g.st);
        }
        upload_tokens(g, [&](int b, int t) { return prompt_tok(b, Tq - Tq_head + t); }, Tq_head);
        dec_embed(dt_, g.tok_in, g.B * Tq_head, Tq_head, dm_.d, tok_emb_, dec_pos_, g.ds, g.dx, g.st);
        if (rq.beam_k > 0) {
            beam_host_.assign((size_t)g.B * 4 + 1, 0);
            for (int b = 0; b < g.B; ++b) beam_host_[b * 4 + 3] = 3000;
            HIP_CHECK(hipMemcpyAsync(g.beam_row, beam_host_.data(), (size_t)g.B * 16, hipMemcpyHostToDevice, g.st));
            HIP_CHECK(hipMemcpyAsync(g.beam_step, beam_host_.data() + (size_t)g.B * 4, 4, hipMemcpyHostToDevice, g.st));
        }
        enqueue_decoder_pass(g, E, Tq_head, rq, out_cap);
    }
    if (rq.beam_k > 0) {
        tm_.n_decode_passes = 1;
        for (DecGroup* g : act) {
            HIP_CHECK(hipEventRecord(g->ev, g->st));
            HIP_CHECK(hipStreamWaitEvent(st_, g->ev, 0));
        }
        return;
    }
    int passes = 1;
    static const bool no_graph = getenv("SPT_NO_GRAPH") != nullptr;
    static const bool sync_debug = getenv("SPT_DEBUG_SYNC") != nullptr;
    if (rq.n_steps > 1 && no_graph) {
        for (int s = 1; s < rq.n_steps; ++s, ++passes)
            for (DecGroup* g : act) {
                enqueue_decoder_pass(*g, E, 1, rq, out_cap);
                if (!sync_debug) continue;
                const hipError_t e = hipStreamSynchronize(g->st);
                DecState h{};
                if (e == hipSuccess) HIP_CHECK(hipMemcpy(&h, g->ds, sizeof(h), hipMemcpyDeviceToHost));
                if (e != hipSuccess || h.step != s + 1 || (s % 16) == 0)
                    fprintf(stderr, "[spt] pass %d: %s step=%d pos0=%d\n", s, hipGetErrorString(e), h.step, h.pos0);
                if (e != hipSuccess) throw HipError(std::string("pass failed: ") + hipGetErrorString(e));
            }
    } else if (rq.n_steps > 1) {
        std::vector<hipGraphExec_t> ex;
        for (DecGroup* g : act) {
            GraphKey key{g->B, E, g->b0, out_cap, rq.n_forced, rq.flags, rq.full};
            key.share = S;
            auto it = g->graphs.find(key);
            if (it == g->graphs.end()) {
                hipGraph_t graph;
                HIP_CHECK(hipStreamBeginCapture(g->st, hipStreamCaptureModeThreadLocal));
                enqueue_decoder_pass(*g, E, 1, rq, out_cap);
                HIP_CHECK(hipStreamEndCapture(g->st, &graph));
                hipGraphExec_t exec;
                HIP_CHECK(hipGraphInstantiate(&exec, graph, nullptr, nullptr, 0));
                HIP_CHECK(hipGraphDestroy(graph));
                it = g->graphs.emplace(key, exec).first;
            }
            ex.push_back(it->second);
        }
        const bool early_exit = !(rq.flags & 4u);
        std::vector<int> hdone(B);
        for (int s = 1; s < rq.n_steps; ++s) {
            for (size_t i = 0; i < act.size(); ++i) HIP_CHECK(hipGraphLaunch(ex[i], act[i]->st));
            ++passes;
            if (early_exit && (s % 16) == 0) {
                bool all = true;
                for (DecGroup* g : act) {
                    HIP_CHECK(hipMemcpyAsync(hdone.data(), g->done, g->B * 4, hipMemcpyDeviceToHost, g->st));
                    HIP_CHECK(hipStreamSynchronize(g->st));
                    all = all && std::all_of(hdone.begin(), hdone.begin() + g->B, [](int v) { return v != 0; });
                }
                if (all) break;
            }
        }
    }
    tm_.n_decode_passes = passes;
    for (DecGroup* g : act) {
        const size_t off = (size_t)g->b0 * out_cap, n = (size_t)g->B * out_cap * 4;
        HIP_CHECK(hipMemcpyAsync(tokens + off, g->out_tok, n, hipMemcpyDeviceToHost, g->st));
        if (top1) HIP_CHECK(hipMemcpyAsync(top1 + off, g->out_t1, n, hipMemcpyDeviceToHost, g->st));
        if (top2) HIP_CHECK(hipMemcpyAsync(top2 + off, g->out_t2, n, hipMemcpyDeviceToHost, g->st));
        if (ts_state_out && rq.full)
            HIP_CHECK(hipMemcpyAsync(ts_state_out + (size_t)g->b0 * 4, g->ts_state, (size_t)g->B * 16,
                                     hipMemcpyDeviceToHost, g->st));
        HIP_CHECK(hipEventRecord(g->ev, g->st));
        HIP_CHECK(hipStreamWaitEvent(st_, g->ev, 0));
    }
}

void Engine::decode(int B, const DecodeRequest& rq, int* tokens, float* top1, float* top2, int* lang_out,
                    int* ts_state_out) {
    select();
    require_weights();
    HIP_CHECK(hipEventRecord(ev_[6], st_));
    run_decode(B, rq, tokens, top1, top2, lang_out, ts_state_out);
    HIP_CHECK(hipEventRecord(ev_[7], st_));
    HIP_CHECK(hipStreamSynchronize(st_));
    HIP_CHECK(hipGetLastError());
    tm_.batch = B;
    cs_.engine_calls++;
    cs_.decoder_passes += tm_.n_decode_passes;
    finish_call_timing();
}

void Engine::finish_call_timing() {
    float ms;
    HIP_CHECK(hipEventElapsedTime(&ms, ev_[6], ev_[7]));
    tm_.decode_ms = ms;
    double total = ms;
    if (enc_pending_) {
        float m_norm, m_enc, m_kv;
        HIP_CHECK(hipEventElapsedTime(&m_norm, ev_[2], ev_[3]));
        HIP_CHECK(hipEventElapsedTime(&m_enc, ev_[3], ev_[4]));
        HIP_CHECK(hipEventElapsedTime(&m_kv, ev_[4], ev_[5]));
        tm_.encoder_ms = m_enc;
        tm_.cross_kv_ms = m_kv;
        tm_.mel_ms = m_norm;
        cs_.encoder_ms += m_enc;
        total += m_norm + m_enc + m_kv;
    } else {
        tm_.encoder_ms = tm_.cross_kv_ms = tm_.mel_ms = 0.0;
    }
    if (mel_pending_) {
        HIP_CHECK(hipEventElapsedTime(&ms, ev_[0], ev_[1]));
        tm_.mel_ms += ms;
        total += ms;
    }
    tm_.total_ms = total;
    cs_.device_ms += total;
    cs_.decode_ms += tm_.decode_ms;
    mel_pending_ = enc_pending_ = false;
}

void Engine::transcribe_device(const float* pcm_dev, int64_t stride, const int* n_samples, int B,
                               const DecodeRequest& rq, int* tokens, float* top1, float* top2, int* lang_out,
                               int* ts_state_out) {
    if (B < 1 || B > max_batch_) throw std::runtime_error("batch exceeds the context's max_batch");
    for (int b = 0; b < B; ++b)
        if (n_samples[b] < 0 || n_samples[b] > 480000 || (int64_t)n_samples[b] > stride)
            throw std::runtime_error("each window must hold 0..480000 samples within its stride");
    load_utterances_device(pcm_dev, stride, n_samples, B);
    std::vector<int> utt(B), seek(B, 0);
    for (int b = 0; b < B; ++b) utt[b] = b;
    encode_windows(utt.data(), seek.data(), B);
    decode(B, rq, tokens, top1, top2, lang_out, ts_state_out);
}

void Engine::transcribe_host(const float* const* pcm, const int* n_samples, int B, const DecodeRequest& rq,
                             int* tokens, float* top1, float* top2, int* lang_out, int* ts_state_out) {
    if (B < 1 || B > max_batch_) throw std::runtime_error("batch exceeds the context's max_batch");
    for (int b = 0; b < B; ++b)
        if (n_samples[b] < 0 || n_samples[b] > 480000) throw std::runtime_error("window longer than 30 s");
    load_utterances(pcm, n_samples, B);
    std::vector<int> utt(B), seek(B, 0);
    for (int b = 0; b < B; ++b) utt[b] = b;
    encode_windows(utt.data(), seek.data(), B);
    decode(B, rq, tokens, top1, top2, lang_out, ts_state_out);
}

void Engine::read_cands(int B, BeamCands* out) {
    DecGroup& g = groups_[0];
    out->id.resize((size_t)B * 8);
    out->lp.resize((size_t)B * 8);
    out->tid.resize(B);
    const char* lo = (const char*)g.cand_id;
    const size_t o_lp = (const char*)g.cand_lp - lo, o_tid = (const char*)g.beam_tid - lo;
    beam_rd_.resize(o_tid + (size_t)B * 4);
    HIP_CHECK(hipMemcpyAsync(beam_rd_.data(), lo, beam_rd_.size(), hipMemcpyDeviceToHost, g.st));
    HIP_CHECK(hipStreamSynchronize(g.st));
    memcpy(out->id.data(), beam_rd_.data(), (size_t)B * 32);
    memcpy(out->lp.data(), beam_rd_.data() + o_lp, (size_t)B * 32);
    memcpy(out->tid.data(), beam_rd_.data() + o_tid, (size_t)B * 4);
}

void Engine::beam_begin(int B, const DecodeRequest& rq, BeamCands* out, int* lang_out) {
    select();
    require_weights();
    if (rq.beam_k < 1 || rq.beam_k > 8) throw std::runtime_error("beam size must be in 1..8");
    if (n_groups_ != 1) throw std::runtime_error("beam search needs one decode group");
    if (B > max_rows_)
        throw std::runtime_error("beam search rows (utterances x beam_size) exceed the decoder's " +
                                 std::to_string(max_rows_) + " rows per pass for this model");
    if (!kvtmp_) {
        const size_t bytes = (size_t)dm_.n_dec * 2 * max_batch_ * dm_.n_head * dm_.n_text_ctx * 64 * esz_;
        if (hipMalloc(&kvtmp_, bytes) != hipSuccess) {
            kvtmp_ = nullptr;
            throw std::runtime_error("out of device memory for the beam search scratch");
        }
        HIP_CHECK(hipMemset(kvtmp_, 0, bytes));
    }
    beam_rq_ = rq;
    beam_B_ = B;
    beam_side_ = 0;
    std::vector<int> tok((size_t)B * rq.n_steps);
    decode(B, rq, tok.data(), nullptr, nullptr, lang_out, nullptr);
    read_cands(B, out);
}

void Engine::beam_next(const int* src, const int* tokens, const int* rowstate, int step, BeamCands* out) {
    select();
    const int B = beam_B_;
    if (B < 1) throw std::runtime_error("beam_next without beam_begin");
    DecGroup& g = groups_[0];
    for (int b = 0; b < B; ++b)
        if (src[b] < 0 || src[b] >= B || tokens[b] < 0 || tokens[b] >= dm_.n_vocab)
            throw std::runtime_error("beam_next: bad source row or token");
    char* lo = (char*)g.beam_row;
    const size_t o_step = (char*)g.beam_step - lo, o_src = (char*)g.beam_src - lo;
    beam_host_.assign((o_src + (size_t)B * 4 + 3) / 4, 0);
    char* hb = (char*)beam_host_.data();
    memcpy(hb, rowstate, (size_t)B * 16);
    memcpy(hb + o_step, &step, 4);
    memcpy(hb + o_src, src, (size_t)B * 4);
    beam_tok_.assign(tokens, tokens + B);
    HIP_CHECK(hipMemcpyAsync(lo, hb, o_src + (size_t)B * 4, hipMemcpyHostToDevice, g.st));
    HIP_CHECK(hipMemcpyAsync(g.tok_in, beam_tok_.data(), (size_t)B * 4, hipMemcpyHostToDevice, g.st));
    const int side = beam_side_;
    void* const own = g.skv;
    void* const kv_from = side ? kvtmp_ : own;
    void* const kv_to = side ? own : kvtmp_;
    auto beam_pass = [&] {
        dec_kv_gather(dt_, kv_from, kv_to, g.beam_src, dm_.n_dec, B, dm_.n_head, dm_.n_text_ctx, g.ds, g.st);
        dec_embed(dt_, g.tok_in, B, 1, dm_.d, tok_emb_, dec_pos_, g.ds, g.dx, g.st);
        struct SkvSide {
            DecGroup& g;
            void* own;
            ~SkvSide() { g.skv = own; }
        } side_guard{g, own};
        g.skv = kv_to;
        float* x = enqueue_layers(g, enc_E_, 1);
        g.skv = own;
        enqueue_head(g, 1, beam_rq_, beam_rq_.n_steps, x, suppress_, (beam_rq_.flags & 1u) != 0);
    };
    static const bool no_graph = getenv("SPT_NO_GRAPH") != nullptr;
    HIP_CHECK(hipEventRecord(ev_[8], g.st));
    if (no_graph) {
        beam_pass();
    } else {
        GraphKey key{B, enc_E_, side, beam_rq_.n_steps, -beam_rq_.beam_k, beam_rq_.flags, beam_rq_.full};
        key.share = g.share;
        auto it = g.graphs.find(key);
        if (it == g.graphs.end()) {
            hipGraph_t graph;
            HIP_CHECK(hipStreamBeginCapture(g.st, hipStreamCaptureModeThreadLocal));
            beam_pass();
            HIP_CHECK(hipStreamEndCapture(g.st, &graph));
            hipGraphExec_t exec;
            HIP_CHECK(hipGraphInstantiate(&exec, graph, nullptr, nullptr, 0));
            HIP_CHECK(hipGraphDestroy(graph));
            it = g.graphs.emplace(key, exec).first;
        }
        HIP_CHECK(hipGraphLaunch(it->second, g.st));
    }
    HIP_CHECK(hipEventRecord(ev_[9], g.st));
    read_cands(B, out);
    beam_side_ ^= 1;
    float ms = 0.0f;
    HIP_CHECK(hipEventElapsedTime(&ms, ev_[8], ev_[9]));
    cs_.beam_steps++;
    cs_.decoder_passes++;
    cs_.device_ms += ms;
    cs_.decode_ms += ms;
}

void Engine::debug_mel(const float* pcm_host, int n, int seek, float* out_host) {
    select();
    const float* p = pcm_host;
    load_utterances(&p, &n, 1);
    const int u = 0;
    upload_windows(&u, &seek, 1);
    mel_pending_ = false;
    float* dbg = nullptr;
    const size_t bytes = (size_t)dm_.n_mels * 3000 * 4;
    HIP_CHECK(hipMalloc(&dbg, bytes));
    mel_norm(dt_, umel_, umax_, mu_, win_utt_, win_seek_, 1, dm_.n_mels, cp_, mel_in_, dbg, st_);
    HIP_CHECK(hipMemcpyAsync(out_host, dbg, bytes, hipMemcpyDeviceToHost, st_));
    HIP_CHECK(hipStreamSynchronize(st_));
    HIP_CHECK(hipFree(dbg));
}

void Engine::debug_encode(const float* mel_host, float* out_host) {
    select();
    require_weights();
    const int nm = dm_.n_mels, d = dm_.d, T = dm_.n_audio_ctx;
    std::vector<char> img((size_t)MEL_ROWS * cp_ * esz_, 0);
    for (int t = 0; t < 3000; ++t)
        for (int c = 0; c < nm; ++c) {
            const float v = mel_host[(size_t)c * 3000 + t];
            const size_t o = (size_t)(t + 1) * cp_ + c;
            if (dt_ == DT_F16) ((uint16_t*)img.data())[o] = f2h_bits(v);
            else if (esz_ == 2) ((uint16_t*)img.data())[o] = f2bf(v);
            else ((float*)img.data())[o] = v;
        }
    HIP_CHECK(hipMemcpyAsync(mel_in_, img.data(), img.size(), hipMemcpyHostToDevice, st_));
    run_encoder(1);
    float* tmp = nullptr;
    HIP_CHECK(hipMalloc(&tmp, (size_t)T * d * 4));
    to_f32(dt_, enc_out_, tmp, (int64_t)T * d, st_);
    HIP_CHECK(hipMemcpyAsync(out_host, tmp, (size_t)T * d * 4, hipMemcpyDeviceToHost, st_));
    HIP_CHECK(hipStreamSynchronize(st_));
    HIP_CHECK(hipFree(tmp));
}

bool Engine::debug_weight_checksum(int tid, double* out2) {
    select();
    auto it = tref_.find(tid);
    if (it == tref_.end()) return false;
    HIP_CHECK(hipMemsetAsync(scratch_, 0, 16, st_));
    tensor_checksum(it->second.dt, it->second.p, it->second.n, scratch_, st_);
    HIP_CHECK(hipMemcpyAsync(out2, scratch_, 16, hipMemcpyDeviceToHost, st_));
    HIP_CHECK(hipStreamSynchronize(st_));
    return true;
}

}

namespace spt {

double Engine::probe(int kind, int iters, double* work, int* is_flops) {
    select();
    const int B = enc_E_;
    if (B < 1 || tm_.batch < 1) throw std::runtime_error("probe needs a completed transcription call first");
    if (iters < 1 || iters > 100000) throw std::runtime_error("iters out of range");
    const int d = dm_.d, H = dm_.n_head, T = dm_.n_audio_ctx, ctx = dm_.n_text_ctx, V = dm_.n_vocab;
    DecGroup& g = groups_[0];
    const int Bg = g.B > 0 ? g.B : B;
    const int nl = (kind == 0 || kind == 3) ? std::min(8, dm_.n_dec) : 1;
    std::function<void()> launch;
    *is_flops = 0;
    switch (kind) {
        case 0:
            launch = [&] {
                for (int l = 0; l < nl; ++l)
                    dec_cross_attn(dt_, g.dq, (const char*)ckv_ + kv_layer_elems(B, H, T) * l * esz_, std::min(Bg, B), B,
                                   H, T, 1, g.dao, st_, xsplit_, g.xpart);
// ... 149 lines not shown
```

spittle_amd/csrc/engine.h:

```cpp
#pragma once
#include <hip/hip_runtime.h>
#include <stdint.h>

#include <map>
#include <set>
#include <string>
#include <vector>

#include "kernels.h"
#include "vocab.h"

namespace spt {

class GgmlFile;

struct ModelDims {
    std::string name;
    int n_mels = 80, d = 384, n_head = 6, n_enc = 4, n_dec = 4, n_vocab = 51864;
    int n_audio_ctx = 1500, n_text_ctx = 448;
};


struct DecodeRequest {
    std::vector<int> prompt;
    std::vector<int> prefix;
    std::vector<int> lang_tok;
    int n_steps = 128;
    uint32_t flags = 3;
    const int32_t* forced = nullptr;
    int n_forced = 0;
    bool full = false;
    TsParams ts{};
    std::vector<int> seek, seek_end;
    std::vector<std::vector<int>> row_prefix;
    std::vector<int> extra_suppress;
    int blank_tok = 220;
    int beam_k = 0;
    std::vector<int> kv_row;
};

struct BeamCands {
    std::vector<int> id;
    std::vector<float> lp;
    std::vector<int> tid;
};

struct Timings {
    double mel_ms = 0, encoder_ms = 0, cross_kv_ms = 0, decode_ms = 0, total_ms = 0, h2d_ms = 0;
    int n_decode_passes = 0, batch = 0;
};

struct CallStats {
    int engine_calls = 0, decoder_passes = 0, beam_steps = 0, encoder_windows = 0;
    int pd_passes = 0;
    int pd_fallbacks = 0;
    double device_ms = 0, encoder_ms = 0, decode_ms = 0;
};

class Engine {
public:
    Engine(const ModelDims& dm, int dtype, int device, int max_batch, uint64_t seed, const GgmlFile* src = nullptr,
           bool external_weights = false);
    ~Engine();
    Engine(const Engine&) = delete;
    Engine& operator=(const Engine&) = delete;

    const ModelDims& dims() const { return dm_; }
    int dtype() const { return dt_; }
    int max_batch() const { return max_batch_; }
    int max_rows() const { return max_rows_; }
    int64_t weight_bytes() const { return wbytes_; }
    bool weights_ready() const { return weights_ready_; }
    void export_weights(void* dev_dst, int64_t bytes);
    void import_weights(const void* dev_src, int64_t bytes);
    void* weight_arena() const { return warena_; }
    int device() const { return dev_; }
    void commit_weights();
    int64_t workspace_bytes() const { return abytes_; }
    const Timings& timings() const { return tm_; }
    const CallStats& call_stats() const { return cs_; }
    void reset_call_stats() { cs_ = CallStats(); }

    void load_utterances(const float* const* pcm_host, const int* n, int U);
    void load_utterances_device(const float* pcm_dev, int64_t stride, const int* n, int U);
    void encode_windows(const int* utt, const int* seek, int E);
    int encoded_windows() const { return enc_E_; }
    void decode(int B, const DecodeRequest& rq, int* tokens, float* top1, float* top2, int* lang_out = nullptr,
                int* ts_state_out = nullptr);

    void transcribe_device(const float* pcm_dev, int64_t stride, const int* n_samples, int B, const DecodeRequest& rq,
                           int* tokens, float* top1, float* top2, int* lang_out = nullptr, int* ts_state_out = nullptr);
    void transcribe_host(const float* const* pcm, const int* n_samples, int B, const DecodeRequest& rq, int* tokens,
                         float* top1, float* top2, int* lang_out = nullptr, int* ts_state_out = nullptr);

    void beam_begin(int B, const DecodeRequest& rq, BeamCands* out, int* lang_out);
    void beam_next(const int* src, const int* tokens, const int* rowstate, int step, BeamCands* out);

    void debug_mel(const float* pcm_host, int n, int seek, float* out_host);
    void debug_encode(const float* mel_host, float* out_host);
    bool debug_weight_checksum(int tid, double* out2);
    double probe(int kind, int iters, double* work, int* is_flops);

private:
    struct GraphKey {
        int B, B_total, b0, out_cap, n_forced;
        uint32_t flags;
        bool full;
        int share = 0;
        bool operator<(const GraphKey& o) const {
            if (full != o.full) return full < o.full;
            if (B != o.B) return B < o.B;
            if (share != o.share) return share < o.share;
            if (B_total != o.B_total) return B_total < o.B_total;
            if (b0 != o.b0) return b0 < o.b0;
            if (out_cap != o.out_cap) return out_cap < o.out_cap;
            if (n_forced != o.n_forced) return n_forced < o.n_forced;
            return flags < o.flags;
        }
    };
    struct DecGroup {
        hipStream_t st = nullptr;
        hipEvent_t ev = nullptr;
        int b0 = 0, B = 0;
        float* dx = nullptr;
        void *dq = nullptr, *dao = nullptr, *dff = nullptr;
        void* skv = nullptr;
        float* logits = nullptr;
        void* part = nullptr;
        unsigned* arrive = nullptr;
        int *tok_in = nullptr, *out_tok = nullptr, *done = nullptr, *forced = nullptr;
        float *out_t1 = nullptr, *out_t2 = nullptr;
        DecState* ds = nullptr;
        float* dx2 = nullptr;
        float* pend = nullptr;
        float* xpart = nullptr;
        int *seek = nullptr, *seek_end = nullptr, *ts_state = nullptr;
        float* ts_stat = nullptr;
        float* beam_stat = nullptr;
        TsParams* prm = nullptr;
        int *beam_row = nullptr, *beam_step = nullptr, *beam_src = nullptr;
        int *cand_id = nullptr, *beam_tid = nullptr;
        float* cand_lp = nullptr;
        int* kvrow = nullptr;
        int share = 0;
        std::map<GraphKey, hipGraphExec_t> graphs;
        std::vector<int> host_tok;
        size_t host_used = 0;
    };

    void select() const;
    void release();
    void alloc_weights();
    void generate_weights();
    void load_ggml(const GgmlFile& f);
    void alloc_workspace();
    void upload_tables(const std::vector<float>* filters);
    void run_mel_utts(const float* pcm, const std::vector<int64_t>& pcm_off, const int* n, int U);
    void upload_windows(const int* utt, const int* seek, int E);
    void finish_call_timing();
    void run_encoder(int B);
    void enc_layer(int l, int Bg, int64_t r0, hipStream_t s, int probe = 0, hipEvent_t e0 = nullptr,
                   hipEvent_t e1 = nullptr);
    int enc_groups_cur_ = 1;
    void enqueue_encoder(int B);
    void run_cross_kv(int B);
    void run_decode(int B, const DecodeRequest& rq, int* tokens, float* top1, float* top2, int* lang_out,
                    int* ts_state_out);
    void enqueue_decoder_pass(DecGroup& g, int E, int Tq, const DecodeRequest& rq, int out_cap);
    float* enqueue_layers(DecGroup& g, int E, int Tq);
    void enqueue_head(DecGroup& g, int Tq, const DecodeRequest& rq, int out_cap, float* xc, const uint32_t* sup,
                      bool blank);

    ModelDims dm_;
    int dt_, dev_, max_batch_;
    uint64_t seed_;
    int esz_;
    int cp_;
    static constexpr int fc2_split_ = 2;
    bool pend_fold_ = true;
    void ln_source(GemvArgs& a, float* xc, float* pend, int np, int64_t slab) const;
    int xsplit_ = 1;
    int n_groups_ = 1;
    int max_rows_ = 64;
    hipStream_t st_ = nullptr;
    std::vector<hipEvent_t> ev_;
    static constexpr int kEncGroupsMax = 4;
    std::vector<hipStream_t> enc_st_;
    std::vector<hipEvent_t> enc_ev_;
    int enc_groups(int B) const;
    int probe_kind_ = -1;
    std::vector<hipEvent_t> probe_ev_;

    char* warena_ = nullptr;
    int64_t wbytes_ = 0;
    bool weights_ready_ = false;
    void require_weights() const;
    struct EncL { float *ln1_w, *ln1_b; void* qkv_w; float* qkv_b; void* o_w; float* o_b; float *ln2_w, *ln2_b;
                  void* fc1_w; float* fc1_b; void* fc2_w; float* fc2_b; };
    struct DecL { float *ln1_w, *ln1_b; void* qkv_w; float* qkv_b; void* so_w; float* so_b; float *ln2_w, *ln2_b;
                  void* cq_w; float* cq_b; void* co_w; float* co_b; float *ln3_w, *ln3_b; void* fc1_w; float* fc1_b;
                  void* fc2_w; float* fc2_b; };
    void *conv1_w_, *conv2_w_, *ckv_w_, *tok_emb_;
    float *conv1_b_, *conv2_b_, *enc_pos_, *lnp_w_, *lnp_b_, *ckv_b_, *dec_pos_, *lnf_w_, *lnf_b_;
    std::vector<EncL> enc_;
    std::vector<DecL> dec_;
    struct TRef { void* p; int64_t n; int dt; };
    std::map<int, TRef> tref_;
    std::map<std::pair<int, int>, hipGraphExec_t> enc_graphs_;
    std::set<std::pair<int, int>> enc_seen_;

    float *hann_ = nullptr, *sinv_ = nullptr, *cosv_ = nullptr, *filt_ = nullptr;
    int* grp_ = nullptr;

    char* aarena_ = nullptr;
    int64_t abytes_ = 0;
    int *win_utt_ = nullptr, *win_seek_ = nullptr;
    void* mel_in_ = nullptr;
    void* y1p_ = nullptr;
    float* x_ = nullptr;
    void *xn_ = nullptr, *qkv_ = nullptr, *ao_ = nullptr, *ff_ = nullptr, *enc_out_ = nullptr;
    void* ckv_ = nullptr;
    uint32_t* suppress_ = nullptr;
    uint32_t* suppress_lang_ = nullptr;
    bool suppress_lang_ready_ = false;
    double* scratch_ = nullptr;
    float* zero_ = nullptr;
    std::vector<DecGroup> groups_;

    std::vector<uint32_t> host_suppress_;
    uint32_t suppress_flags_ = ~0u;
    std::vector<int> suppress_extra_;
    std::vector<int> ts_init_;
    DecodeRequest beam_rq_;
    int beam_B_ = 0;
    int beam_side_ = 0;
    void* kvtmp_ = nullptr;
    std::vector<int> beam_host_;
    std::vector<int> beam_tok_;
    std::vector<char> beam_rd_;
    void read_cands(int B, BeamCands* out);

    float* upcm_ = nullptr;
    int64_t upcm_cap_ = 0;
    float* umel_ = nullptr;
    int64_t umel_cap_ = 0;
    char* uinfo_ = nullptr;
    int uinfo_cap_ = 0;
    MelUtts mu_{};
    unsigned* umax_ = nullptr;
    std::vector<int> un_;
    std::vector<int64_t> uhost_;
    std::vector<char> mel_img_;
    std::vector<int> whost_;
    std::vector<int> kvrow_host_;
    int enc_E_ = 0;
    bool mel_pending_ = false, enc_pending_ = false;
    void ensure_capacity(void** p, int64_t* cap, int64_t need, size_t esz, const char* what);

    Timings tm_;
    CallStats cs_;
};

bool ggml_dims(const GgmlFile& f, ModelDims* dm, std::string* err);
// ... 5 lines not shown
```

spittle_amd/csrc/k_dec.hip:

```cpp
#include "common.h"
#include "kernels.h"

#include <stdio.h>
#include <stdlib.h>

#include <algorithm>
#include <type_traits>

#ifndef SPT_STAMP
#define SPT_STAMP 0
#endif

namespace spt {

#if SPT_STAMP
__device__ unsigned long long* g_xattn_stamp;
void set_xattn_stamp(void* p) { HIP_CHECK(hipMemcpyToSymbol(HIP_SYMBOL(g_xattn_stamp), &p, sizeof(p))); }
#define XA_STAMP(i)                                                                          \
    do {                                                                                     \
        if (g_xattn_stamp && threadIdx.x == 0)                                               \
            g_xattn_stamp[3 * blockIdx.x + (i)] = __builtin_amdgcn_s_memrealtime();          \
    } while (0)
#else
#define XA_STAMP(i) do {} while (0)
#endif

namespace {

template <typename T>
__global__ void embed_kernel(const int* __restrict__ tok, int Tq, int d, const T* __restrict__ emb,
                             const float* __restrict__ pos, const DecState* __restrict__ ds, float* __restrict__ x) {
    const int r = blockIdx.x, t = r % Tq;
    const int p = ds->pos0 + t;
    const T* e = emb + (size_t)tok[r] * d;
    const float* pp = pos + (size_t)p * d;
    for (int i = threadIdx.x; i < d; i += blockDim.x) x[(size_t)r * d + i] = to_f<T>(e[i]) + pp[i];
}

template <typename T> struct GV;
template <> struct GV<bf16> {
    static constexpr int KS = 128;
    typedef bf16x8 frag;
};
template <> struct GV<f16> {
    static constexpr int KS = 128;
    typedef f16x8 frag;
};
template <> struct GV<float> {
    static constexpr int KS = 64;
    typedef f32x4 frag;
};

constexpr int GV_LDS_BYTES = 98304;
__host__ __device__ inline int gv_img_bytes(int R, int K, int esz) {
    return ((R * (K + 16 / esz) * esz) + 15) & ~15;
}

struct alignas(16) TopP { float v1; int i1; float v2; int pad; };
__device__ __forceinline__ TopP top_merge(TopP a, TopP b) {
    const bool aw = (a.v1 > b.v1) || (a.v1 == b.v1 && a.i1 < b.i1);
    TopP r;
    r.pad = 0;
    if (aw) { r.v1 = a.v1; r.i1 = a.i1; r.v2 = fmaxf(a.v2, b.v1); }
    else { r.v1 = b.v1; r.i1 = b.i1; r.v2 = fmaxf(b.v2, a.v1); }
    return r;
}
__device__ __forceinline__ TopP top_shfl(TopP t, int mask) {
    TopP u;
    u.v1 = __shfl_xor(t.v1, mask, 64);
    u.i1 = __shfl_xor(t.i1, mask, 64);
    u.v2 = __shfl_xor(t.v2, mask, 64);
    u.pad = 0;
    return u;
}

#ifndef SPT_GV_NT
#define SPT_GV_NT 0
#endif
template <typename F>
__device__ __forceinline__ F load_w(const F* p) {
#if SPT_GV_NT
    return __builtin_nontemporal_load(p);
#else
    return *p;
#endif
}

constexpr int LN_SRC(int np) { return 16 + np; }
constexpr bool is_ln(int asrc) { return asrc >= 16 && asrc < 32; }
constexpr int ln_np(int asrc) { return asrc - 16; }
constexpr int ATTN_SRC(int s) { return 32 + s; }
constexpr bool is_attn(int asrc) { return asrc >= 32; }
constexpr int attn_s(int asrc) { return asrc - 32; }

#define GV_STAMP(i)                                                                                       \
    do {                                                                                                  \
        if (SPT_STAMP && a.stamp && threadIdx.x == 0)                                                     \
            a.stamp[2 * (blockIdx.x + blockIdx.y * gridDim.x) + (i)] = __builtin_amdgcn_s_memrealtime(); \
    } while (0)

template <typename T, int MODE, int ASRC, int RG, int NWV, int CT, int MAXJ, bool EXACT = false>
__global__ __launch_bounds__(64 * NWV) void gemv_kernel(GemvArgs a) {
    GV_STAMP(0);
    constexpr int KS = GV<T>::KS;
    constexpr int CPE = 16 / sizeof(T);
    constexpr int KSPLIT = NWV / CT;
    constexpr bool IMG = ASRC != A_DIRECT;
    typedef typename GV<T>::frag frag;
    extern __shared__ __attribute__((aligned(16))) char smem[];
    const int tid = threadIdx.x, lane = tid & 63, wid = tid >> 6;
    const int fr = lane & 15, fq = lane >> 4;
    const int ct = wid % CT, ks = wid / CT;
    const int tile = blockIdx.x * CT + ct;
    const int n0 = tile * 16;
    const int K = a.K;
    const int lds_ld = K + CPE;
    const int kz = blockIdx.y, kzc = gridDim.y;
    const int nss_all = K / KS, per = (nss_all + kzc - 1) / kzc;
    const int ss0 = kz * per, ss1 = min(nss_all, ss0 + per);
    const T* wrow = (const T*)a.W + (size_t)min(n0 + fr, a.N - 1) * K + fq * CPE;

    frag w[MAXJ][4];
    auto load_chunk = [&](int j0) {
#pragma unroll
        for (int j = 0; j < MAXJ; ++j) {
            const int ss = ss0 + ks + (j0 + j) * KSPLIT;
            if (EXACT || ss < ss1) {
#pragma unroll
                for (int i = 0; i < 4; ++i) w[j][i] = load_w((const frag*)(wrow + (size_t)ss * KS + i * 4 * CPE));
            }
        }
    };
    constexpr int NP = is_ln(ASRC) ? ln_np(ASRC) : 0;
    float4 x0[NP + 1][6];
    if constexpr (is_ln(ASRC)) {
        if (wid < a.R) {
            const size_t ro = (size_t)wid * a.lda + a.a_row0;
#pragma unroll
            for (int i = 0; i < 6; ++i) {
                const int k = lane * 4 + 256 * i;
                if (k < K) {
                    x0[0][i] = *(const float4*)((const float*)a.A + ro + k);
#pragma unroll
                    for (int p = 0; p < NP; ++p) x0[p + 1][i] = *(const float4*)(a.pend[p] + ro + k);
                }
            }
        }
    }
    const int n_ep = n0 + fr;
    const bool ep_lane = ks == 0 && n_ep < a.N;
    float bias_pre = 0.f;
    if constexpr (MODE != GV_LOGITS) {
        if (ep_lane && a.bias && kz == 0) bias_pre = a.bias[n_ep];
    }
    float resid_pre[RG][4];
    const float* resid = MODE == GV_BIAS_RESID ? (const float*)a.C
                         : MODE == GV_PARTIAL && kz == 0 ? a.p_resid : nullptr;
    if constexpr (MODE == GV_BIAS_RESID || MODE == GV_PARTIAL) {
#pragma unroll
        for (int g = 0; g < RG; ++g)
#pragma unroll
            for (int r = 0; r < 4; ++r) {
                const int row = g * 16 + 4 * fq + r;
                resid_pre[g][r] = (resid && ep_lane && row < a.R) ? resid[(size_t)row * a.ldc + n_ep] : 0.f;
            }
    }
    int st_pre = 0;
    if constexpr (MODE == GV_QKV_CACHE) st_pre = a.st->pos0;
    if constexpr (MODE == GV_LOGITS) st_pre = a.st->step;
    uint32_t sup_pre = 0;
    if constexpr (MODE == GV_LOGITS) {
        if (n_ep < a.N) sup_pre = a.suppress[n_ep >> 5];
    }
    float4 lnw_pre[6], lnb_pre[6];
    if constexpr (is_ln(ASRC)) {
#pragma unroll
        for (int i = 0; i < 6; ++i) {
            const int k = lane * 4 + 256 * i;
            if (k < K) {
                lnw_pre[i] = *(const float4*)(a.ln_w + k);
                lnb_pre[i] = *(const float4*)(a.ln_b + k);
            }
        }
    }
    load_chunk(0);
// ... 112 lines not shown
                } else {
#pragma unroll
                    for (int i = 0; i < 4; ++i) af[i] = frag{};
                }
                if constexpr (std::is_same<T, f16>::value) {
#pragma unroll
                    for (int i = 0; i < 4; ++i)
                        acc[g] = __builtin_amdgcn_mfma_f32_16x16x32_f16(af[i], w[j][i], acc[g], 0, 0, 0);
                } else if constexpr (sizeof(T) == 2) {
#pragma unroll
                    for (int i = 0; i < 4; ++i)
                        acc[g] = __builtin_amdgcn_mfma_f32_16x16x32_bf16(af[i], w[j][i], acc[g], 0, 0, 0);
                } else {
#pragma unroll
                    for (int i = 0; i < 4; ++i)
#pragma unroll
                        for (int e = 0; e < 4; ++e)
                            acc[g] = __builtin_amdgcn_mfma_f32_16x16x4f32(af[i][e], w[j][i][e], acc[g], 0, 0, 0);
                }
            }
        }
    };
    if constexpr (EXACT) {
        compute_chunk(0);
    } else {
        for (int j0 = 0; ss0 + ks + j0 * KSPLIT < ss1; j0 += MAXJ) {
            if (j0 > 0) load_chunk(j0);
            compute_chunk(j0);
        }
    }

    if constexpr (KSPLIT > 1) {
        f32x4* red = (f32x4*)(smem + (IMG ? gv_img_bytes(a.R, K, sizeof(T)) : 0));
        if (IMG) __syncthreads();
#pragma unroll
        for (int g = 0; g < RG; ++g) red[(wid * RG + g) * 64 + lane] = acc[g];
        __syncthreads();
        if (ks != 0) return;
#pragma unroll
        for (int g = 0; g < RG; ++g) {
            f32x4 v = acc[g];
#pragma unroll
            for (int s = 1; s < KSPLIT; ++s) v += red[(((s * CT) + ct) * RG + g) * 64 + lane];
            acc[g] = v;
        }
    }
    const int n = n0 + fr;
    if constexpr (MODE == GV_LOGITS) {
        const int step = st_pre;
        const bool nvalid = n < a.N;
        bool sup = !nvalid;
        if (nvalid) {
            sup = (sup_pre >> (n & 31)) & 1u;
            if (step == 0 && (n == a.blank0 || n == a.blank1)) sup = true;
        }
#pragma unroll
        for (int g = 0; g < RG; ++g) {
#pragma unroll
            for (int r = 0; r < 4; ++r) {
                const int row = g * 16 + 4 * fq + r;
                const float v = acc[g][r];
                if (nvalid && row < a.R) ((float*)a.C)[(size_t)row * a.ldc + n] = v;
                TopP t{sup ? -INFINITY : v, nvalid ? n : 0x7fffffff, -INFINITY, 0};
                t = top_merge(t, top_shfl(t, 1));
                t = top_merge(t, top_shfl(t, 2));
                t = top_merge(t, top_shfl(t, 4));
                t = top_merge(t, top_shfl(t, 8));
                if (fr == 0 && row < a.R && tile < a.n_tiles) ((TopP*)a.part)[(size_t)row * a.n_tiles + tile] = t;
            }
        }
        GV_STAMP(1);
        return;
    }
    if (n >= a.N) return;
    const float bv = bias_pre;
#pragma unroll
    for (int g = 0; g < RG; ++g) {
#pragma unroll
        for (int r = 0; r < 4; ++r) {
            const int row = g * 16 + 4 * fq + r;
            if (row >= a.R) continue;
            const float y = acc[g][r] + bv;
            if constexpr (MODE == GV_BIAS) {
                ((T*)a.C)[(size_t)row * a.ldc + n] = from_f<T>(y);
            } else if constexpr (MODE == GV_BIAS_GELU) {
                ((T*)a.C)[(size_t)row * a.ldc + n] = from_f<T>(gelu_tanh(y));
            } else if constexpr (MODE == GV_PARTIAL) {
                ((float*)a.C + (size_t)kz * a.c_split)[(size_t)row * a.ldc + n] = resid ? resid_pre[g][r] + y : y;
            } else if constexpr (MODE == GV_BIAS_RESID) {
                ((float*)a.C)[(size_t)row * a.ldc + n] = resid_pre[g][r] + y;
            } else if constexpr (MODE == GV_QKV_CACHE) {
                const int d = a.cache_H * 64;
                if (n < d) {
                    ((T*)a.C)[(size_t)row * a.ldc + n] = from_f<T>(y);
                } else {
                    const int part = n / d - 1;
                    const int rem = n - (part + 1) * d;
                    const int hh = rem >> 6, e = rem & 63;
                    const int bb = row / a.Tq, t = row - bb * a.Tq;
                    const int pos = st_pre + t;
                    const size_t off = ((((size_t)part * a.cache_B + bb) * a.cache_H + hh) * a.cache_ctx + pos) * 64 + e;
                    ((T*)a.cache)[off] = to_cache<T>(y);
                }
            }
        }
    }
    GV_STAMP(1);
}

template <typename T, int MODE, int ASRC, int RG, int NWV, int CT, int MAXJ, bool EXACT = false>
void gemv_attr() {
    const int red = NWV * RG * 64 * (int)sizeof(f32x4);
    ensure_lds_attr((const void*)gemv_kernel<T, MODE, ASRC, RG, NWV, CT, MAXJ, EXACT>, GV_LDS_BYTES + red);
}

template <typename T, int MODE, int ASRC, int RG, int NWV, int CT, int MAXJ, bool EXACT = false>
void gemv_launch_cfg(const GemvArgs& a, hipStream_t st) {
    if (EXACT && cdiv(a.K / GV<T>::KS, a.ksplit) != MAXJ * (NWV / CT))
        throw std::runtime_error("gemv: exact configuration does not match the K slice");
    const int red = NWV * RG * 64 * (int)sizeof(f32x4);
    const int lds = (ASRC != A_DIRECT ? gv_img_bytes(a.R, a.K, sizeof(T)) : 0) + (NWV / CT > 1 ? red : 0);
    hipLaunchKernelGGL((gemv_kernel<T, MODE, ASRC, RG, NWV, CT, MAXJ, EXACT>), dim3(cdiv(a.N, 16 * CT), a.ksplit),
                       dim3(64 * NWV), lds, st, a);
    SPT_LAUNCH_CHECK();
}

#define SPT_GV_CONFIGS(X)   \
    X(4, 1, 2)   \
    X(8, 1, 2)   \
    X(16, 1, 3)

#define SPT_GV_PAIRS(X)                 \
    X(GV_QKV_CACHE, LN_SRC(0))          \
    X(GV_QKV_CACHE, LN_SRC(1))          \
    X(GV_QKV_CACHE, LN_SRC(2))          \
    X(GV_QKV_CACHE, LN_SRC(4))          \
    X(GV_BIAS, LN_SRC(0))               \
    X(GV_BIAS, LN_SRC(2))               \
    X(GV_BIAS_GELU, LN_SRC(0))          \
    X(GV_LOGITS, LN_SRC(0))             \
    X(GV_LOGITS, LN_SRC(1))             \
    X(GV_LOGITS, LN_SRC(2))             \
    X(GV_LOGITS, LN_SRC(4))             \
    X(GV_PARTIAL, A_DIRECT)             \
    X(GV_BIAS_RESID, A_DIRECT)          \
    X(GV_BIAS_RESID, ATTN_SRC(2))       \
    X(GV_BIAS_RESID, ATTN_SRC(3))       \
    X(GV_BIAS_RESID, ATTN_SRC(4))       \
    X(GV_BIAS_RESID, ATTN_SRC(8))

template <typename T, int MODE, int ASRC>
void gemv_attr_all() {
#define SPT_ATTR(NWV, CT, MAXJ)                          \
    gemv_attr<T, MODE, ASRC, 1, NWV, CT, MAXJ>();         \
    gemv_attr<T, MODE, ASRC, 2, NWV, CT, MAXJ>();         \
    gemv_attr<T, MODE, ASRC, 4, NWV, CT, MAXJ>();
    if constexpr (MODE == GV_LOGITS) {
        SPT_ATTR(4, 4, 4)
        SPT_ATTR(8, 8, 4)
    } else if constexpr (ASRC == A_DIRECT || is_attn(ASRC)) {
        SPT_GV_CONFIGS(SPT_ATTR)
        gemv_attr<T, MODE, ASRC, 1, 12, 1, 1, true>();
        gemv_attr<T, MODE, ASRC, 2, 12, 1, 1, true>();
        gemv_attr<T, MODE, ASRC, 4, 12, 1, 1, true>();
    } else {
        SPT_ATTR(4, 1, 2)
        SPT_ATTR(8, 1, 2)
        SPT_ATTR(8, 2, 3)
        gemv_attr<T, MODE, ASRC, 1, 10, 1, 1, true>();
        gemv_attr<T, MODE, ASRC, 2, 10, 1, 1, true>();
        gemv_attr<T, MODE, ASRC, 4, 10, 1, 1, true>();
        gemv_attr<T, MODE, ASRC, 1, 10, 2, 2, true>();
        gemv_attr<T, MODE, ASRC, 2, 10, 2, 2, true>();
        gemv_attr<T, MODE, ASRC, 4, 10, 2, 2, true>();
        gemv_attr<T, MODE, ASRC, 1, 12, 1, 1, true>();
        gemv_attr<T, MODE, ASRC, 2, 12, 1, 1, true>();
        gemv_attr<T, MODE, ASRC, 4, 12, 1, 1, true>();
    }
#undef SPT_ATTR
}
template <typename T>
void gemv_attr_modes() {
#define SPT_PAIR(M, S) gemv_attr_all<T, M, S>();
    SPT_GV_PAIRS(SPT_PAIR)
#undef SPT_PAIR
}

template <typename T, int MODE, int ASRC, int RG>
void gemv_launch_rg(const GemvArgs& a, hipStream_t st) {
    const int nss = cdiv(a.K / GV<T>::KS, a.ksplit);
// ... 61 lines not shown
    const int tid = threadIdx.x, lane = tid & 63, wid = tid >> 6, g = lane & 7;
    AttnWave<T, NQ, NIX> aw;
    aw.init(kv + (((size_t)0 * B + b) * H + h) * (size_t)ctx * 64 + 8 * g,
            kv + (((size_t)1 * B + b) * H + h) * (size_t)ctx * 64 + 8 * g, ctx, lane);
    aw.load_blk(aw.kc_[0], aw.vc_[0], wid);
    const int pos0 = ds->pos0;
    const int n_keys = pos0 + Tq;
    aw.n_keys = n_keys;
    float qv[NQ][8];
    int lim[NQ];
#pragma unroll
    for (int t = 0; t < NQ; ++t) {
        const int tt = t < Tq ? t : Tq - 1;
        const T* qr = q + (size_t)(b * Tq + tt) * q_ld + h * 64 + 8 * g;
#pragma unroll
        for (int e = 0; e < 8; ++e) qv[t][e] = to_f<T>(qr[e]) * kLog2Scale;
        lim[t] = pos0 + tt + 1;
    }
    aw.template run_pre<(448 / AttnWave<T, NQ, NIX>::KB + 1 + AW - 1) / AW>(wid, cdiv(n_keys, AttnWave<T, NQ, NIX>::KB), qv, lim, Tq);
    aw.to_lds(s_m, s_l, s_o, wid, lane);
    __syncthreads();
    if (tid < 64 * Tq) {
        const int t = tid >> 6, e = tid & 63;
        float M, L, O;
        attn_merge<NQ>(s_m, s_l, s_o, t, e, M, L, O);
        out[(size_t)(b * Tq + t) * (H * 64) + h * 64 + e] = from_f<T>(O / L);
    }
}

template <typename T, int NQ, bool SPLIT, int NW = AW, int NIX = 0, int PF = 2>
__global__ __launch_bounds__(64 * NW) void cross_attn_kernel(const T* __restrict__ q, const T* __restrict__ kv,
                                                             int B_layout, int H, int T_enc, int Tq,
                                                             T* __restrict__ out, float* __restrict__ part,
                                                             const int* __restrict__ kvrow, int share) {
    typedef AttnWave<T, NQ, NIX, NW, PF> W;
    XA_STAMP(0);
    __shared__ float s_m[NW][NQ], s_l[NW][NQ];
    __shared__ float s_o[NW][NQ][64];
    const int bh = blockIdx.x, j = bh / H, h = bh - j * H;
    const int tid = threadIdx.x, lane = tid & 63, wid = tid >> 6, g = lane & 7;
    const int nq_all = share * Tq;
    const int c0 = SPLIT ? 0 : (int)blockIdx.y * NQ;
    const int nq = min(NQ, nq_all - c0);
    const int kb = kvrow ? kvrow[j * share] : j;
    W aw;
    const size_t kvo = ((size_t)kb * H + h) * 4096 + 8 * g;
    aw.init(kv + kvo, kv + kvo + 2048, T_enc, lane, (int64_t)B_layout * H * 4096);
    const size_t qrow0 = (size_t)j * nq_all + c0;
    float qv[NQ][8];
    int lim[NQ];
#pragma unroll
    for (int t = 0; t < NQ; ++t) {
        const int tt = t < nq ? t : nq - 1;
        const T* qr = q + (qrow0 + tt) * (H * 64) + h * 64 + 8 * g;
#pragma unroll
        for (int e = 0; e < 8; ++e) qv[t][e] = to_f<T>(qr[e]) * kLog2Scale;
        lim[t] = T_enc;
    }
    const int nblk_all = cdiv(T_enc, W::KB);
    const int S = SPLIT ? (int)gridDim.y : 1, sp = SPLIT ? (int)blockIdx.y : 0;
    const int per = cdiv(nblk_all, S), blk0 = sp * per, nblk = min(nblk_all, blk0 + per);
    aw.template run<(1500 / W::KB + 1 + NW - 1) / NW>(blk0 + wid, nblk, qv, lim, nq);
    if (wid == 0) XA_STAMP(1);
    aw.to_lds(s_m, s_l, s_o, wid, lane);
    __syncthreads();
    XA_STAMP(2);
    for (int i = tid; i < 64 * nq; i += 64 * NW) {
        const int t = i >> 6, e = i & 63;
        float M, L, O;
        attn_merge<NQ, NW>(s_m, s_l, s_o, t, e, M, L, O);
        if constexpr (SPLIT) {
            float* pp = part + (((qrow0 + t) * H + h) * S + sp) * 66;
            pp[e] = O;
            if (e == 0) {
                pp[64] = M;
                pp[65] = L;
            }
        } else {
            out[(qrow0 + t) * (H * 64) + h * 64 + e] = from_f<T>(O / L);
        }
    }
}

template <typename T, int NQ, int NIX = 0, int PF = 2>
__global__ __launch_bounds__(64) void cross_attn_vw_kernel(const T* __restrict__ q, const T* __restrict__ kv,
                                                           int B_layout, int H, int T_enc, int Tq,
                                                           float* __restrict__ part, const int* __restrict__ kvrow,
                                                           int share) {
    typedef AttnWave<T, NQ, NIX, AW, PF> W;
    __shared__ float s_m[1][NQ], s_l[1][NQ];
    __shared__ float s_o[1][NQ][64];
    const int bh = blockIdx.x, j = bh / H, h = bh - j * H;
    const int vw = blockIdx.y;
    const int lane = threadIdx.x, g = lane & 7;
    const int nq_all = share * Tq;
    const int c0 = (int)blockIdx.z * NQ;
    const int nq = min(NQ, nq_all - c0);
    const int kb = kvrow ? kvrow[j * share] : j;
    W aw;
    const size_t kvo = ((size_t)kb * H + h) * 4096 + 8 * g;
    aw.init(kv + kvo, kv + kvo + 2048, T_enc, lane, (int64_t)B_layout * H * 4096);
    const size_t qrow0 = (size_t)j * nq_all + c0;
    float qv[NQ][8];
    int lim[NQ];
#pragma unroll
    for (int t = 0; t < NQ; ++t) {
        const int tt = t < nq ? t : nq - 1;
        const T* qr = q + (qrow0 + tt) * (H * 64) + h * 64 + 8 * g;
#pragma unroll
        for (int e = 0; e < 8; ++e) qv[t][e] = to_f<T>(qr[e]) * kLog2Scale;
        lim[t] = T_enc;
    }
    aw.template run<(1500 / W::KB + 1 + AW - 1) / AW>(vw, cdiv(T_enc, W::KB), qv, lim, nq);
    aw.to_lds(s_m, s_l, s_o, 0, lane);
    __syncthreads();
    for (int i = lane; i < 64 * nq; i += 64) {
        const int t = i >> 6, e = i & 63;
        float* pp = part + (((qrow0 + t) * H + h) * AW + vw) * 66;
        pp[e] = s_o[0][t][e];
        if (e == 0) {
            pp[64] = s_m[0][t];
            pp[65] = s_l[0][t];
        }
    }
}

template <typename T>
__global__ __launch_bounds__(64) void attn_part_merge_kernel(const float* __restrict__ part, int H, T* __restrict__ out) {
#pragma clang fp contract(off)
    const int rh = blockIdx.x, e = threadIdx.x;
    const float* pp = part + (size_t)rh * AW * 66;
    float mw[AW], lw[AW], ow[AW];
#pragma unroll
    for (int w = 0; w < AW; ++w) {
        mw[w] = pp[w * 66 + 64];
        lw[w] = pp[w * 66 + 65];
        ow[w] = pp[w * 66 + e];
    }
    float M = -INFINITY;
#pragma unroll
    for (int w = 0; w < AW; ++w) M = fmaxf(M, mw[w]);
    float L = 0.f, O = 0.f;
#pragma unroll
    for (int w = 0; w < AW; ++w) {
        if (mw[w] == -INFINITY) continue;
        const float f = exp2f(mw[w] - M);
        L = __builtin_fmaf(lw[w], f, L);
        O = __builtin_fmaf(ow[w], f, O);
    }
    out[(size_t)rh * 64 + e] = from_f<T>(O / L);
}

constexpr int FIN_T = 1024;
template <typename T>
__global__ __launch_bounds__(FIN_T) void finalize_kernel(FinalizeArgs a) {
    __shared__ TopP s_top[FIN_T / 64];
    __shared__ int s_tok;
    const int b = blockIdx.x, tid = threadIdx.x;
    const int step = a.ds->step, pos0 = a.ds->pos0;
    TopP t{-INFINITY, 0x7fffffff, -INFINITY, 0};
    const TopP* p = (const TopP*)a.part + (size_t)b * a.n_tiles;
    for (int i = tid; i < a.n_tiles; i += FIN_T) t = top_merge(t, p[i]);
#pragma unroll
    for (int o = 32; o > 0; o >>= 1) t = top_merge(t, top_shfl(t, o));
    if ((tid & 63) == 0) s_top[tid >> 6] = t;
    __syncthreads();
    if (tid == 0) {
        for (int w = 1; w < FIN_T / 64; ++w) t = top_merge(t, s_top[w]);
        if (t.i1 < 0 || t.i1 >= a.n_vocab) {
            t.i1 = -2;
            t.v1 = t.v2 = __builtin_nanf("");
        }
        int nxt = a.eot;
        if (step < a.out_cap) {
            const int oi = b * a.out_cap + step;
            if (a.done[b]) {
                a.out_tok[oi] = -1;
                a.out_top1[oi] = -INFINITY;
                a.out_top2[oi] = -INFINITY;
            } else {
                a.out_tok[oi] = t.i1;
                a.out_top1[oi] = t.v1;
                a.out_top2[oi] = t.v2;
                nxt = t.i1;
                if (a.forced && step < a.forced_len) nxt = a.forced[b * a.forced_len + step];
                if (!a.ignore_eot && t.i1 == a.eot) a.done[b] = 1;
                if (nxt < 0 || nxt >= a.n_vocab) nxt = a.eot;
            }
        }
        a.next_tok[b] = nxt;
        s_tok = nxt;
    }
    __syncthreads();
    const int tok = s_tok;
    const int pn = min(pos0 + a.Tq, a.ctx - 1);
    const T* e = (const T*)a.emb + (size_t)tok * a.d;
    const float* pp = a.pos + (size_t)pn * a.d;
    for (int i = tid; i < a.d; i += FIN_T) a.x[(size_t)b * a.d + i] = to_f<T>(e[i]) + pp[i];
    if (tid == 0) {
        const unsigned prev = __hip_atomic_fetch_add(a.arrive, 1u, __ATOMIC_RELAXED, __HIP_MEMORY_SCOPE_AGENT);
        if (prev == (unsigned)gridDim.x - 1) {
            a.ds->pos0 = pos0 + a.Tq;
            a.ds->step = step + 1;
            __hip_atomic_store(a.arrive, 0u, __ATOMIC_RELAXED, __HIP_MEMORY_SCOPE_AGENT);
        }
    }
}

__global__ void advance_kernel(DecState* ds, int n) { ds->pos0 += n; }

__global__ void reset_kernel(DecState* ds, unsigned* arrive) {
    ds->pos0 = 0;
    ds->step = 0;
    *arrive = 0u;
}

}

void gemv_prepare(int dtype) {
    if (dtype == DT_BF16) gemv_attr_modes<bf16>();
    else if (dtype == DT_F16) gemv_attr_modes<f16>();
    else gemv_attr_modes<float>();
}

int gemv_max_image_rows(int dtype, int K) {
    const int esz = dtype_size(dtype);
    int r = 64;
    while (r > 1 && gv_img_bytes(r, K, esz) > GV_LDS_BYTES) --r;
    return r;
}

void gemv(int dtype, int mode, int asrc, const GemvArgs& a_in, hipStream_t st) {
    if (a_in.R > 64 || a_in.R <= 0) throw std::runtime_error("gemv: rows must be in 1..64");
    const int ks = dtype_size(dtype) == 2 ? 128 : 64;
    if (a_in.K % ks) throw std::runtime_error("gemv: K alignment");
    GemvArgs a = a_in;
    a.ksplit = std::max(1, a.ksplit);
    if (a.ksplit > 1 && mode != GV_PARTIAL) throw std::runtime_error("gemv: K split needs partial outputs");
    if (a.ksplit > a.K / ks) throw std::runtime_error("gemv: K split exceeds the super-steps");
    const int esz = dtype_size(dtype);
    if (asrc != A_DIRECT && gv_img_bytes(a.R, a.K, esz) > GV_LDS_BYTES)
        throw std::runtime_error("gemv: A image exceeds the LDS budget");
    if (asrc == A_LN && (a.K > 1536 || !a.ln_w || !a.ln_b))
        throw std::runtime_error("gemv: LayerNorm prologue needs K <= 1536 and LN parameters");
    if (asrc == A_LN && (a.n_pend < 0 || a.n_pend > 4 || a.n_pend == 3))
        throw std::runtime_error("gemv: pending slab count must be 0, 1, 2 or 4");
    if (a.p_resid && mode != GV_PARTIAL) throw std::runtime_error("gemv: residual rows into slab 0 need partial outputs");
    if (asrc == A_LN)
        for (int p = 0; p < 4; ++p)
            if (!a.pend[p]) throw std::runtime_error("gemv: LayerNorm prologue needs 4 pending slabs (zero slab if none)");
    if (asrc == A_ATTN && (!a.apart || a.a_splits < 2 || (a.a_splits > 4 && a.a_splits != 8) || a.a_heads * 64 != a.K))
        throw std::runtime_error("gemv: attention-merge prologue needs 2..4 or 8 chunks over all heads");
    const int code = asrc == A_LN ? LN_SRC(a.n_pend) : asrc == A_ATTN ? ATTN_SRC(a.a_splits) : asrc;
#define SPT_GV(M, S)                                                      \
    if (mode == M && code == S) {                                         \
        if (dtype == DT_BF16) gemv_launch<bf16, M, S>(a, st);             \
        else if (dtype == DT_F16) gemv_launch<f16, M, S>(a, st);          \
        else gemv_launch<float, M, S>(a, st);                             \
        return;                                                           \
    }
    SPT_GV_PAIRS(SPT_GV)
#undef SPT_GV
    throw std::runtime_error("gemv: unsupported mode / A source");
}

void dec_embed(int dtype, const int* tok, int R, int Tq, int d, const void* tok_emb, const float* pos_emb,
               const DecState* ds, float* x, hipStream_t st) {
    if (dtype == DT_BF16)
        hipLaunchKernelGGL(embed_kernel<bf16>, dim3(R), dim3(256), 0, st, tok, Tq, d, (const bf16*)tok_emb, pos_emb, ds, x);
    else if (dtype == DT_F16)
        hipLaunchKernelGGL(embed_kernel<f16>, dim3(R), dim3(256), 0, st, tok, Tq, d, (const f16*)tok_emb, pos_emb, ds, x);
    else
        hipLaunchKernelGGL(embed_kernel<float>, dim3(R), dim3(256), 0, st, tok, Tq, d, (const float*)tok_emb, pos_emb, ds, x);
}

void dec_self_attn(int dtype, const void* q, const void* cache, int B, int H, int ctx, int Tq, const DecState* ds,
                   void* out, hipStream_t st) {
    if (Tq < 1 || Tq > 4) throw std::runtime_error("dec_self_attn: 1..4 queries per sequence");
    const dim3 grid(B * H), blk(64 * AW);
#define SPT_SA(T, NQ) \
    hipLaunchKernelGGL((self_attn_kernel<T, NQ>), grid, blk, 0, st, (const T*)q, H * 64, (const T*)cache, B, H, ctx, Tq, ds, (T*)out)
    if (dtype == DT_BF16) {
        if (Tq == 1) SPT_SA(bf16, 1); else SPT_SA(bf16, 4);
    } else if (dtype == DT_F16) {
        if (Tq == 1) SPT_SA(f16, 1); else SPT_SA(f16, 4);
    } else {
        if (Tq == 1) SPT_SA(float, 1); else SPT_SA(float, 4);
    }
#undef SPT_SA
    SPT_LAUNCH_CHECK();
}

static int xattn_pf() {
    static const int pf = getenv("SPT_XATTN_PF") ? std::max(2, std::min(4, atoi(getenv("SPT_XATTN_PF")))) : 2;
    return pf;
}

void dec_cross_attn(int dtype, const void* q, const void* kv, int B, int B_layout, int H, int T_enc, int Tq, void* out,
                    hipStream_t st, int splits, float* part, const int* kvrow, int share) {
    if (Tq < 1 || Tq > 4) throw std::runtime_error("dec_cross_attn: 1..4 queries per sequence");
    if (splits < 1 || splits > 4 || (splits > 1 && !part)) throw std::runtime_error("dec_cross_attn: 1..4 key chunks");
    if (share < 1 || share > 8 || B % share) throw std::runtime_error("dec_cross_attn: rows per window 1..8, dividing B");
    if (share > 1 && !kvrow) throw std::runtime_error("dec_cross_attn: shared windows need the window map");
    if ((int64_t)cdiv(T_enc, 32) * B_layout * H * 4096 >= (int64_t)INT32_MAX)
        throw std::runtime_error("dec_cross_attn: a layer's cross K/V exceeds 2^31 elements");
    const int nq = share * Tq;
    const int NQ = nq == 1 ? 1 : Tq > 1 ? 4 : (dtype_size(dtype) == 2 ? 5 : 4);
    if (splits > 1 && nq > NQ) throw std::runtime_error("dec_cross_attn: key chunks need one query chunk per window");
    const dim3 grid((B / share) * H, splits > 1 ? splits : cdiv(nq, NQ)), blk(64 * AW);
#define SPT_XA(T, NQ_, SP, NI, ...)                                                                             \
    hipLaunchKernelGGL((cross_attn_kernel<T, NQ_, SP, AW, NI __VA_ARGS__>), grid, blk, 0, st, (const T*)q,        \
                       (const T*)kv, B_layout, H, T_enc, Tq, (T*)out, part, kvrow, share)
#define SPT_XA_T(T)                                                                       \
    if (NQ == 1) {                                                                        \
        if (splits > 1) SPT_XA(T, 1, true, 0);                                            \
        else if (xattn_pf() == 4) SPT_XA(T, 1, false, 0, , 4);                            \
        else if (xattn_pf() == 3) SPT_XA(T, 1, false, 0, , 3);                            \
        else SPT_XA(T, 1, false, 0);                                                      \
    }                                                                                     \
    else if (NQ == 4 && Tq > 1) { if (splits > 1) SPT_XA(T, 4, true, 0); else SPT_XA(T, 4, false, 0); } \
    else if (NQ == 4) { if (splits > 1) SPT_XA(T, 4, true, 4); else SPT_XA(T, 4, false, 4); } \
    else { if (splits > 1) SPT_XA(T, 5, true, 4); else SPT_XA(T, 5, false, 4); }
    if (dtype == DT_BF16) { SPT_XA_T(bf16); }
    else if (dtype == DT_F16) { SPT_XA_T(f16); }
    else { SPT_XA_T(float); }
#undef SPT_XA_T
#undef SPT_XA
    SPT_LAUNCH_CHECK();
}

void dec_cross_attn_vw(int dtype, const void* q, const void* kv, int B, int B_layout, int H, int T_enc, int Tq,
                       float* part, hipStream_t st, const int* kvrow, int share, bool per_query) {
    if (Tq < 1 || Tq > 4) throw std::runtime_error("dec_cross_attn_vw: 1..4 queries per sequence");
    if (share < 1 || share > 8 || B % share) throw std::runtime_error("dec_cross_attn_vw: rows per window 1..8, dividing B");
    if (share > 1 && !kvrow) throw std::runtime_error("dec_cross_attn_vw: shared windows need the window map");
    if ((int64_t)cdiv(T_enc, 32) * B_layout * H * 4096 >= (int64_t)INT32_MAX)
        throw std::runtime_error("dec_cross_attn_vw: a layer's cross K/V exceeds 2^31 elements");
    if (!part) throw std::runtime_error("dec_cross_attn_vw: needs the partials buffer");
    const int nq = share * Tq;
    const int NQ = (nq == 1 || (per_query && Tq == 1)) ? 1 : Tq > 1 ? 4 : (dtype_size(dtype) == 2 ? 5 : 4);
    const dim3 grid((B / share) * H, AW, cdiv(nq, NQ)), blk(64);
#define SPT_XV(T, NQ_, NI, PF)                                                                               \
    hipLaunchKernelGGL((cross_attn_vw_kernel<T, NQ_, NI, PF>), grid, blk, 0, st, (const T*)q, (const T*)kv,      \
                       B_layout, H, T_enc, Tq, part, kvrow, share)
#define SPT_XV_PF(T, NQ_, NI)                                    \
    if (xattn_pf() == 4) SPT_XV(T, NQ_, NI, 4);                  \
    else if (xattn_pf() == 3) SPT_XV(T, NQ_, NI, 3);             \
    else SPT_XV(T, NQ_, NI, 2);
#define SPT_XV_T(T)                                         \
    if (NQ == 1) { SPT_XV_PF(T, 1, 0) }                     \
    else if (NQ == 4 && Tq > 1) SPT_XV(T, 4, 0, 2);         \
    else if (NQ == 4) SPT_XV(T, 4, 4, 2);                   \
    else { SPT_XV_PF(T, 5, 4) }
    if (dtype == DT_BF16) { SPT_XV_T(bf16); }
    else if (dtype == DT_F16) { SPT_XV_T(f16); }
    else { SPT_XV_T(float); }
#undef SPT_XV_T
#undef SPT_XV_PF
#undef SPT_XV
    SPT_LAUNCH_CHECK();
}

void dec_attn_part_merge(int dtype, const float* part, int R, int H, void* out, hipStream_t st) {
    if (R < 1 || H < 1 || !part || !out) throw std::runtime_error("dec_attn_part_merge: empty or missing buffers");
    if (dtype == DT_BF16) hipLaunchKernelGGL(attn_part_merge_kernel<bf16>, dim3(R * H), dim3(64), 0, st, part, H, (bf16*)out);
    else if (dtype == DT_F16) hipLaunchKernelGGL(attn_part_merge_kernel<f16>, dim3(R * H), dim3(64), 0, st, part, H, (f16*)out);
    else hipLaunchKernelGGL(attn_part_merge_kernel<float>, dim3(R * H), dim3(64), 0, st, part, H, (float*)out);
    SPT_LAUNCH_CHECK();
}

void dec_finalize(int dtype, const FinalizeArgs& a, int B, hipStream_t st) {
    if (dtype == DT_BF16) hipLaunchKernelGGL(finalize_kernel<bf16>, dim3(B), dim3(FIN_T), 0, st, a);
    else if (dtype == DT_F16) hipLaunchKernelGGL(finalize_kernel<f16>, dim3(B), dim3(FIN_T), 0, st, a);
    else hipLaunchKernelGGL(finalize_kernel<float>, dim3(B), dim3(FIN_T), 0, st, a);
}

void dec_advance(DecState* ds, int n, hipStream_t st) {
    hipLaunchKernelGGL(advance_kernel, dim3(1), dim3(1), 0, st, ds, n);
}

void dec_reset(DecState* ds, unsigned* arrive, hipStream_t st) {
    hipLaunchKernelGGL(reset_kernel, dim3(1), dim3(1), 0, st, ds, arrive);
}

}
```

spittle_amd/csrc/k_sample.hip:

```cpp
#include "common.h"
#include "kernels.h"

namespace spt {

namespace {

constexpr int TW = 1024;

__device__ __forceinline__ float u01(uint64_t seed, int b, int step) {
    uint64_t z = seed * 0x9E3779B97F4A7C15ULL + ((uint64_t)b << 32) + (uint64_t)step + 0x632BE59BD9B4E019ULL;
    z = (z ^ (z >> 30)) * 0xBF58476D1CE4E5B9ULL;
    z = (z ^ (z >> 27)) * 0x94D049BB133111EBULL;
    z ^= z >> 31;
    return (float)(uint32_t)(z >> 40) * (1.0f / 16777216.0f);
}

struct MaxI { float v; int i; };
__device__ __forceinline__ MaxI max_merge(MaxI a, MaxI b) {
    return (b.v > a.v || (b.v == a.v && b.i < a.i)) ? b : a;
}

constexpr int VJ = 52;

struct MaskRule {
// ... 183 lines not shown
            s_scan[tid] = z;
            __syncthreads();
            for (int o = 1; o < TW; o <<= 1) {
                const float add = tid >= o ? s_scan[tid - o] : 0.0f;
                __syncthreads();
                s_scan[tid] += add;
                __syncthreads();
            }
            const float total = s_scan[TW - 1];
            const float u = u01(P.seed, b, step) * total;
            const float lo = tid ? s_scan[tid - 1] : 0.0f, hi = s_scan[tid];
            if (total > 0.0f && u >= lo && (u < hi || tid == TW - 1)) {
                float c = lo;
                int last_ok = -1;
#pragma unroll
                for (int i = 0; i < VJ; ++i) {
                    const int n = n0 + i;
                    if (i >= C || n >= n1) break;
                    if (masked(n) || (rule && n < beg)) continue;
                    last_ok = n;
                    c += expf(cv[i] - M2);
                    if (u < c) break;
                }
                if (last_ok >= 0) s_pick = last_ok;
            }
            __syncthreads();
        }
        if (tid == 0) {
            const int oi = oi0 + step;
            int tok = s_pick;
            if (tok < 0 || tok >= V) {
                a.out_tok[oi] = -2;
                a.out_plog[oi] = __builtin_nanf("");
                a.out_tid[oi] = 0.0f;
                S[3] = 2;
                a.done[b] = 1;
            } else {
                const float plog = val(tok) - s_bc[1];
                int tid_ts = tok >= beg ? tok : (ms.v > -INFINITY ? ms.i : 0);
                a.out_tok[oi] = tok;
                a.out_plog[oi] = plog;
                a.out_tid[oi] = (float)tid_ts;
                const int i = step;
                int hts = S[0], sd = S[1], rl = S[2], status = 0;
                const int seek = a.seek[b], seek_end = a.seek_end[b];
                if (tok > beg) {
                    const int sdn = 2 * (tok - beg);
                    if (hts && sd > sdn && rl < i) status = 2;
                    else { sd = sdn; rl = i + 1; hts = 1; }
                }
                if (status == 0 && (tok == eot || (P.max_tokens > 0 && i >= P.max_tokens) ||
                                    (hts && seek + sd + 100 >= seek_end))) {
                    if (rl == 0 && !P.no_ts) {
                        if (seek + sd + 100 >= seek_end) rl = i + 1;
                        else status = 2;
                    }
                    if (status == 0) {
                        if (P.no_ts) { rl = i + 1; sd = 3000; }
                        status = 1;
                    }
                }
                if (status == 0 && i == P.n_max - 1 && (rl == 0 || sd < 1500)) status = 2;
                S[0] = hts; S[1] = sd; S[2] = rl; S[3] = status;
                if (status != 0) a.done[b] = 1;
            }
        }
    } else if (tid == 0 && step < a.out_cap) {
        const int oi = b * a.out_cap + step;
        a.out_tok[oi] = -1;
        a.out_plog[oi] = -INFINITY;
        a.out_tid[oi] = -1.0f;
    }
    __syncthreads();
    if (tid == 0) {
        int nxt = (live && step < a.out_cap) ? a.out_tok[b * a.out_cap + step] : eot;
        if (live && a.forced && step < a.forced_len) nxt = a.forced[b * a.forced_len + step];
        if (nxt < 0 || nxt >= V) nxt = eot;
        a.next_tok[b] = nxt;
        s_tok = nxt;
    }
    __syncthreads();
    const int tok = s_tok;
    const int pos0 = a.ds->pos0;
    const int pn = min(pos0 + a.Tq, a.ctx - 1);
    const T* e = (const T*)a.emb + (size_t)tok * a.d;
    const float* pp = a.pos + (size_t)pn * a.d;
    for (int i = tid; i < a.d; i += TW) a.x[(size_t)b * a.d + i] = to_f<T>(e[i]) + pp[i];
    if (tid == 0) {
        const unsigned prev = __hip_atomic_fetch_add(a.arrive, 1u, __ATOMIC_RELAXED, __HIP_MEMORY_SCOPE_AGENT);
        if (prev == (unsigned)gridDim.x - 1) {
            a.ds->pos0 = pos0 + a.Tq;
            a.ds->step = step + 1;
            __hip_atomic_store(a.arrive, 0u, __ATOMIC_RELAXED, __HIP_MEMORY_SCOPE_AGENT);
        }
    }
}

__global__ __launch_bounds__(TW) void beam_topk_kernel(BeamArgs a) {
    __shared__ MaxI s_m[2][TW / 64];
    __shared__ float s_s[TW / 64];
    __shared__ MaxI s_k[TW / 64];
    const int b = blockIdx.x, tid = threadIdx.x, lane = tid & 63, wv = tid >> 6;
    const int step = a.step[0];
    const TsParams& P = *a.prm;
    const int V = a.n_vocab, beg = a.beg, eot = a.eot;
    const float* lg = a.logits + (size_t)b * a.ldl;
    const int last = a.row[4 * b + 0], pen = a.row[4 * b + 1], has_ts = a.row[4 * b + 2], seek_delta = a.row[4 * b + 3];
    const bool last_ts = step > 0 && last >= beg;
    const bool pen_ts = step < 2 || pen >= beg;
    __shared__ uint32_t s_sup[VJ * TW / 32];
    stage_suppress(s_sup, a.suppress, V);
    __syncthreads();
    const MaskRule mr(P, step, eot, beg, a.blank, last_ts, pen_ts, has_ts, seek_delta);
    auto masked = [&](int n) -> bool { return mr.masked(s_sup, n); };
    float lv[VJ];
#pragma unroll
    for (int j = 0; j < VJ; ++j) lv[j] = lg[min(tid + j * TW, V - 1)];
    uint64_t keep = 0;
#pragma unroll
    for (int j = 0; j < VJ; ++j) {
        const int n = tid + j * TW;
        keep |= (uint64_t)((n < V) & !masked(min(n, V - 1))) << j;
    }
    const MaxI none{-INFINITY, 0x7fffffff};
    MaxI mt = none, ms = none;
#pragma unroll
    for (int j = 0; j < VJ; ++j) {
        const int n = tid + j * TW;
        const MaxI c = ((keep >> j) & 1) ? MaxI{lv[j], n} : none;
        const bool t = n < beg;
        mt = max_merge(mt, t ? c : none);
        ms = max_merge(ms, t ? none : c);
    }
#pragma unroll
    for (int o = 32; o > 0; o >>= 1) {
        mt = max_merge(mt, MaxI{__shfl_xor(mt.v, o, 64), __shfl_xor(mt.i, o, 64)});
        ms = max_merge(ms, MaxI{__shfl_xor(ms.v, o, 64), __shfl_xor(ms.i, o, 64)});
    }
    if (lane == 0) { s_m[0][wv] = mt; s_m[1][wv] = ms; }
    __syncthreads();
    mt = s_m[0][0];
    ms = s_m[1][0];
    for (int w = 1; w < TW / 64; ++w) { mt = max_merge(mt, s_m[0][w]); ms = max_merge(ms, s_m[1][w]); }
    const float M = fmaxf(mt.v, ms.v);
    float sa = 0.0f, st = 0.0f;
    if (M > -INFINITY) {
#pragma unroll
        for (int j = 0; j < VJ; ++j) {
            const bool k_ = (keep >> j) & 1;
            const float ea = expf(lv[j] - M), et = expf(lv[j] - ms.v);
            sa += k_ ? ea : 0.0f;
            st += (k_ && tid + j * TW >= beg) ? et : 0.0f;
        }
    }
    sa = wave_sum(sa);
    st = wave_sum(st);
    __shared__ float s_t[TW / 64];
    __shared__ MaxI s_win;
    if (lane == 0) { s_s[wv] = sa; s_t[wv] = st; }
    __syncthreads();
    float za = 0.0f, zt = 0.0f;
    for (int w = 0; w < TW / 64; ++w) { za += s_s[w]; zt += s_t[w]; }
    const float lse = logf(za) + M;
    const float ts_lp = zt > 0.0f ? logf(zt) + ms.v - lse : -INFINITY;
    const bool rule = ms.v > -INFINITY && ts_lp > mt.v - lse;
    if (rule) {
#pragma unroll
        for (int j = 0; j < VJ; ++j)
            if (tid + j * TW < beg) keep &= ~(1ull << j);
    }
    __shared__ int s_cid[8];
    __shared__ float s_clp[8];
    const int k = a.k;
    for (int r = 0; r < k; ++r) {
        MaxI c = none;
// ... 237 lines not shown
```

spittle_amd/csrc/kernels.h:

```cpp
#pragma once
#include <hip/hip_runtime.h>
#include <stdint.h>

#include <string>

namespace spt {

enum { DT_F32 = 0, DT_BF16 = 1, DT_F16 = 2, DT_I8 = 3 };
inline int dtype_size(int dtype) { return dtype == DT_F32 ? 4 : 2; }

__host__ __device__ inline int64_t kv_layer_elems(int B, int H, int T) { return (int64_t)((T + 31) / 32) * B * H * 4096; }
__host__ __device__ inline int64_t kv_offset(int l, int kvi, int b, int h, int t, int e, int B, int H, int T) {
    return (int64_t)l * kv_layer_elems(B, H, T) + (((int64_t)(t >> 5) * B + b) * H + h) * 4096 + kvi * 2048 +
           (t & 31) * 64 + e;
}

enum { EPI_BIAS = 0, EPI_BIAS_GELU = 1, EPI_BIAS_GELU_POS = 2, EPI_BIAS_RESID = 3, EPI_KVSPLIT = 4,
       EPI_BIAS_SWISH = 5, EPI_BIAS_RELU = 6, EPI_BIAS_F32 = 7, EPI_PARTIAL = 8 };

struct GemmArgs {
    const void* A; int lda; int64_t sA;
    const void* W; int ldw;
    int M, N, K;
    const float* bias;
    void* C; int ldc; int64_t sC;
    const float* pos;
    int kv_B, kv_T, kv_H;
    float alpha = 1.0f;
    int ksplit = 1; int64_t c_split = 0;
    int nmajor = 0;
    int groups = 1;
};
void gemm_nt(int dtype, int epi, const GemmArgs& g, int batch, hipStream_t st);
void gemm_prepare();
void gemm_nt_variant(int dtype, int epi, const GemmArgs& g, int batch, int variant, hipStream_t st);

enum { WK_MAT = 0, WK_BIAS = 1, WK_LNW = 2, WK_LNB = 3, WK_TOK = 4, WK_DPOS = 5 };
void gen_weights(int store_dtype, void* dst, int64_t n, uint64_t seed, uint32_t tid, int kind,
                 int scale_exp, hipStream_t st);
void gen_conv_weights(int store_dtype, void* dst, int N, int C, int Cp, uint64_t seed, uint32_t tid,
                      int scale_exp, hipStream_t st);
void fill_f32(float* dst, int64_t n, float v, hipStream_t st);
void ggml_dequant(int type, const void* src, int64_t n, int out_dtype, void* dst, hipStream_t st);
void cache_flush(const void* p, int64_t bytes, unsigned* sink, hipStream_t st);
void set_xattn_stamp(void* p);
void dec_cross_attn_ni8(const void* q, const void* kv, int B, int B_layout, int H, int T_enc, void* out, int blocked,
                        hipStream_t st);
void stream_read(const void* p, int64_t bytes, unsigned* sink, int grid, int tpb, hipStream_t st);
void tensor_checksum(int dtype, const void* src, int64_t n, double* out2_dev, hipStream_t st);

struct MelTables {
    const float* hann;
    const float* sinv;
    const float* cosv;
    const float* filt;
    const int* grp;
};
constexpr int MEL_ROWS = 3002;
struct MelUtts {
    const int64_t* pcm_off;
    const int64_t* row_off;
    const int* n;
};
int mel_rows(int n);
void mel_frames(const float* pcm, MelUtts u, int U, int max_rows, int n_mels, MelTables t, float* mel_raw,
                unsigned* mel_max, hipStream_t st);
void mel_norm(int dtype, const float* mel_raw, const unsigned* mel_max, MelUtts u, const int* win_utt,
              const int* win_seek, int E, int n_mels, int Cp, void* mel_in, float* dbg, hipStream_t st);

void layernorm(int dtype, const float* x, int M, int d, const float* w, const float* b, void* y,
               hipStream_t st);
void layernorm_pend(int dtype, float* x, int M, int d, const float* slab, int ks, int64_t slab_stride,
                    const float* pbias, float alpha, const float* w, const float* b, void* y, bool write_x,
                    hipStream_t st);
void layernorm_pend2(int dtype2, const float* x, int M, int d, const float* slab, int ks, int64_t slab_stride,
                     const float* pbias, float alpha, const float* w, const float* b, float* y, const float* w2,
                     const float* b2, void* y2, hipStream_t st);
void to_f32(int dtype, const void* src, float* dst, int64_t n, hipStream_t st);

void enc_attention(int dtype, const void* qkv, int B, int T, int H, void* out, hipStream_t st);

struct DecState {
    int pos0;
    int step;
};

enum { GV_BIAS = 0, GV_BIAS_GELU = 1, GV_PARTIAL = 2, GV_QKV_CACHE = 3, GV_LOGITS = 4, GV_BIAS_RESID = 5 };
enum { A_DIRECT = 0, A_LN = 1, A_ATTN = 2 };
struct GemvArgs {
    const void* A; int lda; int a_row0;
    const float* ln_w; const float* ln_b;
    const float* pend[4]; int n_pend;
    float* x_out;
    const float* apart; int a_splits, a_heads;
    int R;
    const void* W; int N, K;
    const float* bias;
    void* C; int ldc;
    int ksplit; int64_t c_split;
    const float* p_resid;
    void* cache; int cache_B, cache_H, cache_ctx, Tq;
    const DecState* st;
    const uint32_t* suppress; int blank0, blank1;
    void* part; int n_tiles;
    unsigned long long* stamp;
};
constexpr int kMaxPend = 4;
void gemv(int dtype, int mode, int asrc, const GemvArgs& a, hipStream_t st);
void gemv_prepare(int dtype);
int gemv_max_image_rows(int dtype, int K);

void dec_embed(int dtype, const int* tok, int R, int Tq, int d, const void* tok_emb,
               const float* pos_emb, const DecState* ds, float* x, hipStream_t st);
void dec_self_attn(int dtype, const void* q, const void* cache, int B, int H, int ctx, int Tq,
                   const DecState* ds, void* out, hipStream_t st);
void dec_cross_attn(int dtype, const void* q, const void* kv, int B, int B_layout, int H, int T_enc, int Tq,
                    void* out, hipStream_t st, int splits = 1, float* part = nullptr, const int* kvrow = nullptr,
                    int share = 1);
void dec_cross_attn_vw(int dtype, const void* q, const void* kv, int B, int B_layout, int H, int T_enc, int Tq,
                       float* part, hipStream_t st, const int* kvrow = nullptr, int share = 1, bool per_query = false);
void dec_attn_part_merge(int dtype, const float* part, int R, int H, void* out, hipStream_t st);

struct FinalizeArgs {
    const void* part; int n_tiles;
    int eot; int ignore_eot; int n_vocab;
    const int* forced; int forced_len;
    int* next_tok;
    int* out_tok; float* out_top1; float* out_top2; int out_cap;
    int* done;
    const void* emb; const float* pos; int d, ctx, Tq;
    float* x;
    DecState* ds; unsigned* arrive;
};
void dec_finalize(int dtype, const FinalizeArgs& a, int B, hipStream_t st);
void dec_reset(DecState* ds, unsigned* arrive, hipStream_t st);



struct TsParams {
    float temperature;
    int suppress_blank;
    int no_ts;
    int max_initial;
    int n_max;
    int max_tokens;
    unsigned long long seed;
};
struct TsArgs {
    const float* logits; int ldl;
    int n_vocab, eot, beg, blank;
    const uint32_t* suppress;
    const TsParams* prm;
    const int* seek; const int* seek_end;
    int* state;
    const int* forced; int forced_len;
    int* next_tok;
    int* out_tok; float* out_plog; float* out_tid; int out_cap;
    int* done;
    const void* emb; const float* pos; int d, ctx, Tq;
    float* x;
    DecState* ds; unsigned* arrive;
    float* stat;
};
constexpr int TS_CHUNKS = 16;
void dec_ts_stats(const TsArgs& a, int B, hipStream_t st);
void dec_finalize_ts(int dtype, const TsArgs& a, int B, hipStream_t st);
struct BeamArgs {
    const float* logits; int ldl;
    int n_vocab, eot, beg, blank;
    const uint32_t* suppress;
    const TsParams* prm;
    const int* row;
    const int* step;
    int k;
    int* cand_id; float* cand_lp;
    int* tid;
    float* stat;
};
constexpr int BEAM_STAT = 6 + 4 * 8;
void dec_beam_topk(const BeamArgs& a, int B, hipStream_t st);
void dec_kv_gather(int dtype, const void* src, void* dst, const int* rows, int L, int B, int H, int ctx,
                   const DecState* ds, hipStream_t st);
void dec_advance(DecState* ds, int n, hipStream_t st);

}
```

spittle_amd/engine.py:

```python
from __future__ import annotations

import ctypes as C
from dataclasses import dataclass, field
from typing import Optional, Sequence

import numpy as np

from . import _lib as L


class TranscriptionError(RuntimeError):
    def __init__(self, status: int, message: str):
        super().__init__(f"{L.STATUS_NAMES.get(status, status)}: {message}")
        self.status = status
        self.message = message


@dataclass
class WhisperModelParams:
    dtype: str = "bf16"
    device: int = 0
    max_batch: int = 8
    seed: int = 1234
    external_weights: bool = False
# ... 133 lines not shown
            self._lib.spt_ctx_destroy(self._ctx)
            self._ctx = None

    def is_loaded(self) -> bool:
        return bool(self._ctx)

    def __del__(self):
        try:
            self.unload_model()
        except Exception:
            pass

    def _check(self, st: int):
        if st != L.SPT_OK:
            raise TranscriptionError(st, self._lib.spt_last_error(self._ctx).decode())

    def _need(self):
        if not self._ctx:
            raise TranscriptionError(L.SPT_ERR_INVALID_ARG, "Model is not loaded for transcription.")

    def transcribe_samples(self, samples, params: Optional[WhisperInferenceParams] = None) -> TranscriptionResult:
        return self.transcribe_batch([samples], params)[0]

    def transcribe_batch(self, batch: Sequence, params: Optional[WhisperInferenceParams] = None):
        self._need()
        keep: list = []
        ip = _infer_params(params, keep)
        arrs = [np.ascontiguousarray(np.asarray(s, dtype=np.float32).reshape(-1)) for s in batch]
        n = len(arrs)
        ptrs = (C.POINTER(C.c_float) * n)(*[a.ctypes.data_as(C.POINTER(C.c_float)) for a in arrs])
        lens = (C.c_size_t * n)(*[a.size for a in arrs])
        out = (C.POINTER(L.Result) * n)()
        self._check(self._lib.spt_transcribe_batch(self._ctx, ptrs, lens, n, C.byref(ip), out))
        return [_take_result(out[i]) for i in range(n)]

    def transcribe_batch_device(self, dev_ptr: int, stride: int, lengths: Sequence[int],
                                params: Optional[WhisperInferenceParams] = None):
        self._need()
        keep: list = []
        ip = _infer_params(params, keep)
        n = len(lengths)
        lens = (C.c_size_t * n)(*[int(x) for x in lengths])
        out = (C.POINTER(L.Result) * n)()
        self._check(self._lib.spt_transcribe_batch_device(self._ctx, C.c_void_p(dev_ptr), int(stride), lens, n,
                                                          C.byref(ip), out))
        return [_take_result(out[i]) for i in range(n)]

    def export_weights(self, dev_ptr: int, nbytes: int) -> None:
        self._need()
        self._check(self._lib.spt_weights_export(self._ctx, C.c_void_p(dev_ptr), C.c_size_t(nbytes)))

    def import_weights(self, dev_ptr: int, nbytes: int) -> None:
        self._need()
        self._check(self._lib.spt_weights_import(self._ctx, C.c_void_p(dev_ptr), C.c_size_t(nbytes)))

    def weights_arena(self) -> tuple:
        self._need()
        ptr, n = C.c_void_p(), C.c_size_t()
        self._check(self._lib.spt_weights_arena(self._ctx, C.byref(ptr), C.byref(n)))
        return int(ptr.value or 0), int(n.value)

    def commit_weights(self) -> None:
        self._need()
        self._check(self._lib.spt_weights_commit(self._ctx))

    def info(self) -> dict:
        self._need()
        mi = L.ModelInfo()
        self._check(self._lib.spt_ctx_info(self._ctx, C.byref(mi)))
        return {k: getattr(mi, k) for k, _ in mi._fields_}

    def timings(self) -> dict:
        self._need()
        t = L.Timings()
        self._check(self._lib.spt_get_timings(self._ctx, C.byref(t)))
        return {k: getattr(t, k) for k, _ in t._fields_}

    def call_stats(self) -> dict:
        self._need()
        t = L.CallStats()
        self._check(self._lib.spt_get_call_stats(self._ctx, C.byref(t)))
        return {k: getattr(t, k) for k, _ in t._fields_ if k != "reserved0"}

    def debug_mel(self, samples, seek: int = 0) -> np.ndarray:
        self._need()
        x = np.ascontiguousarray(np.asarray(samples, np.float32).reshape(-1))
        out = np.empty((self.info()["n_mels"], 3000), np.float32)
        self._check(self._lib.spt_debug_mel_at(self._ctx, x.ctypes.data_as(C.POINTER(C.c_float)), x.size, int(seek),
                                               out.ctypes.data_as(C.POINTER(C.c_float))))
        return out

    def debug_encode(self, mel) -> np.ndarray:
        self._need()
        info = self.info()
        m = np.ascontiguousarray(mel, dtype=np.float32)
        assert m.shape == (info["n_mels"], 3000)
        out = np.empty((info["n_audio_ctx"], info["d"]), np.float32)
        self._check(self._lib.spt_debug_encode(self._ctx, m.ctypes.data_as(C.POINTER(C.c_float)),
                                               out.ctypes.data_as(C.POINTER(C.c_float))))
        return out

    def probe(self, kernel: str, iters: int = 50) -> dict:
        self._need()
        us, work, fl = C.c_double(), C.c_double(), C.c_int32()
        self._check(self._lib.spt_probe_kernel(self._ctx, L.PROBES[kernel], int(iters), C.byref(us), C.byref(work),
                                               C.byref(fl)))
        return {"avg_us": us.value, "work": work.value, "work_is_flops": bool(fl.value)}

    def tokenize(self, text: str) -> list[int]:
        self._need()
        raw = text.encode("utf-8")
        n = C.c_int32()
        buf = (C.c_int32 * max(1, len(raw) + 1))()
        self._check(self._lib.spt_tokenize(self._ctx, raw, buf, len(raw) + 1, C.byref(n)))
        return [buf[i] for i in range(n.value)]

    def token_to_str(self, token: int) -> Optional[bytes]:
        self._need()
        return self._lib.spt_token_to_str(self._ctx, int(token))

    def weight_checksum(self, tensor_id: int):
        self._need()
        o = (C.c_double * 2)()
        self._check(self._lib.spt_debug_weight_checksum(self._ctx, int(tensor_id), o))
        return float(o[0]), float(o[1])
```

Baseline: 944.3 audio-sec/wall-sec.

## Fuse decoder cross-attention Q projection with attention via device-side granule handoff

Adds a single kernel that runs the LN2 + cross-Q GEMV in some blocks and cross-attention in others. The producer blocks publish tagged bf16 Q values, and the attention blocks prefetch K/V while spinning on those tags, which removes a kernel boundary per layer per decode step and overlaps the K/V loads with the Q projection. An epoch counter in DecState makes the tags unique per step and layer. A timeout sets an error flag, after which the whole decode is rerun on the unfused path. The scheme relies on all producer and consumer blocks being co-resident (grid size checked against the CU count). It adds spin-wait cost, an optional K/V cache-touch prefetch, and rerun overhead if the timeout fires.

```diff
diff --git a/include/spittle_hip.h b/include/spittle_hip.h
--- a/include/spittle_hip.h
+++ b/include/spittle_hip.h
@@ -134,6 +134,7 @@
 } spt_call_stats;
 
 spt_status spt_get_call_stats(const spt_ctx* ctx, spt_call_stats* s);
+spt_status spt_get_xq_stats(const spt_ctx* ctx, int32_t* fused_launches, int32_t* fallbacks);
 
 spt_status spt_weights_export(spt_ctx* ctx, void* dev_dst, size_t bytes);
 spt_status spt_weights_import(spt_ctx* ctx, const void* dev_src, size_t bytes);
diff --git a/rust/spittle-hip-sys/src/lib.rs b/rust/spittle-hip-sys/src/lib.rs
--- a/rust/spittle-hip-sys/src/lib.rs
+++ b/rust/spittle-hip-sys/src/lib.rs
@@ -200,6 +200,7 @@
 
     pub fn spt_get_timings(ctx: *const spt_ctx, t: *mut spt_timings) -> spt_status;
     pub fn spt_get_call_stats(ctx: *const spt_ctx, s: *mut spt_call_stats) -> spt_status;
+    pub fn spt_get_xq_stats(ctx: *const spt_ctx, fused_launches: *mut i32, fallbacks: *mut i32) -> spt_status;
 
     pub fn spt_weights_export(ctx: *mut spt_ctx, dev_dst: *mut c_void, bytes: usize) -> spt_status;
     pub fn spt_weights_import(ctx: *mut spt_ctx, dev_src: *const c_void, bytes: usize) -> spt_status;
diff --git a/spittle_amd/_lib.py b/spittle_amd/_lib.py
--- a/spittle_amd/_lib.py
+++ b/spittle_amd/_lib.py
@@ -14,7 +14,7 @@
 EXPORTS = [
     "spt_version", "spt_default_model_params", "spt_default_infer_params", "spt_ctx_create",
     "spt_ctx_destroy", "spt_last_error", "spt_ctx_info", "spt_transcribe", "spt_transcribe_batch",
-    "spt_transcribe_batch_device", "spt_result_free", "spt_get_timings", "spt_get_call_stats", "spt_debug_mel",
+    "spt_transcribe_batch_device", "spt_result_free", "spt_get_timings", "spt_get_call_stats", "spt_get_xq_stats", "spt_debug_mel",
     "spt_debug_mel_at", "spt_debug_encode", "spt_debug_weight_checksum", "spt_probe_kernel", "spt_language_code",
     "spt_tokenize", "spt_token_to_str", "spt_debug_ggml_tokenize", "spt_debug_ggml_dequant",
     "spt_weights_export", "spt_weights_import", "spt_weights_arena", "spt_weights_commit",
@@ -234,6 +234,7 @@
     L.spt_debug_ggml_dequant.argtypes = [C.c_int32, C.c_void_p, C.c_int64, fp]
     L.spt_get_timings.argtypes = [vp, C.POINTER(Timings)]
     L.spt_get_call_stats.argtypes = [vp, C.POINTER(CallStats)]
+    L.spt_get_xq_stats.argtypes = [vp, ip, ip]
     L.spt_debug_mel.argtypes = [vp, fp, C.c_size_t, fp]
     L.spt_debug_mel_at.argtypes = [vp, fp, C.c_size_t, C.c_int32, fp]
     L.spt_debug_encode.argtypes = [vp, fp, fp]
@@ -386,7 +387,7 @@
             getattr(L, fn).restype = C.c_int
     for fn in ("spt_weights_arena", "spt_weights_commit", "spt_ctx_create_replicas", "spt_transcribe_batch_replicas",
                "spt_weights_export", "spt_weights_import", "spt_ctx_info", "spt_transcribe", "spt_transcribe_batch", "spt_transcribe_batch_device",
-               "spt_get_timings", "spt_get_call_stats", "spt_debug_mel", "spt_debug_mel_at", "spt_debug_encode", "spt_debug_weight_checksum",
+               "spt_get_timings", "spt_get_call_stats", "spt_get_xq_stats", "spt_debug_mel", "spt_debug_mel_at", "spt_debug_encode", "spt_debug_weight_checksum",
                "spt_probe_kernel", "spt_tokenize", "spt_debug_ggml_tokenize", "spt_debug_ggml_dequant"):
         getattr(L, fn).restype = C.c_int
     _lib = L
diff --git a/spittle_amd/csrc/capi.cpp b/spittle_amd/csrc/capi.cpp
--- a/spittle_amd/csrc/capi.cpp
+++ b/spittle_amd/csrc/capi.cpp
@@ -601,6 +601,14 @@
     return SPT_OK;
 }
 
+spt_status spt_get_xq_stats(const spt_ctx* ctx, int32_t* fused_launches, int32_t* fallbacks) {
+    if (!ctx) return SPT_ERR_INVALID_ARG;
+    const spt::CallStats& c = ctx->eng->call_stats();
+    if (fused_launches) *fused_launches = c.xq_fused;
+    if (fallbacks) *fallbacks = c.xq_fallbacks;
+    return SPT_OK;
+}
+
 spt_status spt_weights_export(spt_ctx* ctx, void* dev_dst, size_t bytes) {
     if (!ctx || !dev_dst) return fail(ctx, SPT_ERR_INVALID_ARG, "null argument");
     try {
diff --git a/spittle_amd/csrc/dec_attn.h b/spittle_amd/csrc/dec_attn.h
--- a/spittle_amd/csrc/dec_attn.h
+++ b/spittle_amd/csrc/dec_attn.h
@@ -153,6 +153,27 @@
             blk += NW;
         }
     }
+    template <int MAXB>
+    __device__ __forceinline__ void ring_fill(int blk, int nblk) {
+        static_assert(MAXB <= 8, "AttnWave: ring_fill / ring_run are the unrolled schedule");
+        const int cnt = blk < nblk ? (nblk - 1 - blk) / NW + 1 : 1;
+        const int mine = blk + (cnt - 1) * NW;
+#pragma unroll
+        for (int d = 0; d < PF - 1 && d < MAXB; ++d) load_blk(kc_[d], vc_[d], min(blk + d * NW, mine));
+    }
+    template <int MAXB>
+    __device__ __forceinline__ void ring_run(int blk, int nblk, const float (&qv)[NQ][8], const int (&lim)[NQ], int Tq) {
+        if (blk >= nblk) return;
+        const int cnt = (nblk - 1 - blk) / NW + 1;
+        const int mine = blk + (cnt - 1) * NW;
+#pragma unroll
+        for (int i = 0; i < MAXB; ++i) {
+            if (i >= cnt) break;
+            if (i + PF - 1 < MAXB)
+                load_blk(kc_[(i + PF - 1) % PF], vc_[(i + PF - 1) % PF], min(blk + (i + PF - 1) * NW, mine));
+            process(kc_[i % PF], vc_[i % PF], (blk + i * NW) * KB, qv, lim, Tq);
+        }
+    }
     __device__ __forceinline__ void to_lds(float (*s_m)[NQ], float (*s_l)[NQ], float (*s_o)[NQ][64], int wid,
                                            int lane) {
         const int g = lane & 7;
diff --git a/spittle_amd/csrc/engine.cpp b/spittle_amd/csrc/engine.cpp
--- a/spittle_amd/csrc/engine.cpp
+++ b/spittle_amd/csrc/engine.cpp
@@ -90,6 +90,7 @@
     if (const char* g = getenv("SPT_DECODE_GROUPS")) n_groups_ = std::max(1, std::min(4, atoi(g)));
     if (const char* v = getenv("SPT_XATTN_SPLIT")) xsplit_ = std::max(1, std::min(4, atoi(v)));
     select();
+    HIP_CHECK(hipDeviceGetAttribute(&n_cu_, hipDeviceAttributeMultiprocessorCount, dev_));
     HIP_CHECK(hipStreamCreateWithFlags(&st_, hipStreamNonBlocking));
     ev_.resize(12);
     for (auto& e : ev_) HIP_CHECK(hipEventCreate(&e));
@@ -131,7 +132,7 @@
     if (st_) (void)hipStreamSynchronize(st_);
     for (auto& g : groups_) {
         if (g.st) (void)hipStreamSynchronize(g.st);
-        for (auto& kv : g.graphs) (void)hipGraphExecDestroy(kv.second);
+        for (auto& kv : g.graphs) (void)hipGraphExecDestroy(kv.second.exec);
         if (g.ev) (void)hipEventDestroy(g.ev);
         if (g.st) (void)hipStreamDestroy(g.st);
     }
@@ -553,6 +554,7 @@
         suppress_ = (uint32_t*)c.take((V / 32 + 1) * 4);
         suppress_lang_ = (uint32_t*)c.take((V / 32 + 1) * 4);
         scratch_ = (double*)c.take(64);
+        xq_err_ = (unsigned*)c.take(64);
         for (DecGroup& g : groups_) {
             g.dx = (float*)c.take(R * d * 4);
             g.dq = A(R * d);
@@ -585,6 +587,7 @@
             g.cand_lp = (float*)c.take(B * 8 * 4);
             g.beam_tid = (int*)c.take(B * 4);
             g.kvrow = (int*)c.take(B * 4);
+            g.xq_gran = (unsigned long long*)c.take(16 * d * 8);
         }
         zero_ = (float*)c.take(R * d * 4);
         if (!pass) {
@@ -861,6 +864,14 @@
     const int xs = vw ? (vw_merge ? 1 : 8) : mapped ? 1 : xsplit_;
     const int ks = esz_ == 2 ? 128 : 64;
     hipStream_t st = g.st;
+    const bool fuse = xq_on_ && probe_kind_ < 0 && Tq == 1 && !vw && !mapped && xs == 1 && dm_.n_dec <= 64 &&
+                      dec_xq_fused_ok(dt_, B, d, H, T, n_cu_);
+    xq_enq_ = fuse ? dm_.n_dec : 0;
+    if (fuse) {
+        hipStreamCaptureStatus cap = hipStreamCaptureStatusNone;
+        HIP_CHECK(hipStreamIsCapturing(st, &cap));
+        if (cap == hipStreamCaptureStatusNone) cs_.xq_fused += xq_enq_;
+    }
     float* xc = g.dx;
     float* xo = g.dx2;
     int np = 0;
@@ -905,11 +916,19 @@
         a = GemvArgs{};
         ln_input(a); a.lda = d; a.ln_w = e.ln2_w; a.ln_b = e.ln2_b; a.R = R;
         a.W = e.cq_w; a.N = d; a.K = d; a.bias = e.cq_b; a.C = g.dq; a.ldc = d;
-        gemv(dt_, GV_BIAS, A_LN, a, st);
+        if (fuse) {
+            if (np != 0) throw std::runtime_error("fused cross-Q launch: pending slabs before LN2");
+            XqFuseArgs x{};
+            x.kv = ckv_l; x.B_layout = E; x.H = H; x.T_enc = T; x.out = g.dao; x.gran = g.xq_gran; x.ds = g.ds;
+            x.err = xq_err_; x.layer = l;
+            dec_xq_fused(dt_, a, x, B, st);
+        } else {
+            gemv(dt_, GV_BIAS, A_LN, a, st);
+        }
         consumed();
         pmark(0, l, 0);
-        if (vw)
-        {
+        if (fuse) {
+        } else if (vw) {
             dec_cross_attn_vw(dt_, g.dq, ckv_l, B, E, H, T, Tq, g.xpart, st, mapped ? g.kvrow : nullptr,
                               mapped ? g.share : 1, per_query);
             if (vw_merge) dec_attn_part_merge(dt_, g.xpart, R, H, g.dao, st);
@@ -1128,6 +1147,13 @@
         }
         DecodeRequest dq;
         dq.flags = 4u;
+        const bool xq_on = xq_on_;
+        xq_on_ = false;
+        struct XqRestore {
+            bool& on;
+            bool v;
+            ~XqRestore() { on = v; }
+        } xq_restore{xq_on_, xq_on};
         for (DecGroup* g : act) {
             reset_outputs(*g);
             upload_tokens(*g, [&](int, int) { return sp.sot; }, 1);
@@ -1205,10 +1231,11 @@
                 if (e != hipSuccess) throw HipError(std::string("pass failed: ") + hipGetErrorString(e));
             }
     } else if (rq.n_steps > 1) {
-        std::vector<hipGraphExec_t> ex;
+        std::vector<PassGraph> ex;
         for (DecGroup* g : act) {
             GraphKey key{g->B, E, g->b0, out_cap, rq.n_forced, rq.flags, rq.full};
             key.share = S;
+            key.fuse = xq_on_;
             auto it = g->graphs.find(key);
             if (it == g->graphs.end()) {
                 hipGraph_t graph;
@@ -1218,14 +1245,17 @@
                 hipGraphExec_t exec;
                 HIP_CHECK(hipGraphInstantiate(&exec, graph, nullptr, nullptr, 0));
                 HIP_CHECK(hipGraphDestroy(graph));
-                it = g->graphs.emplace(key, exec).first;
+                it = g->graphs.emplace(key, PassGraph{exec, xq_enq_}).first;
             }
             ex.push_back(it->second);
         }
         const bool early_exit = !(rq.flags & 4u);
         std::vector<int> hdone(B);
         for (int s = 1; s < rq.n_steps; ++s) {
-            for (size_t i = 0; i < act.size(); ++i) HIP_CHECK(hipGraphLaunch(ex[i], act[i]->st));
+            for (size_t i = 0; i < act.size(); ++i) {
+                HIP_CHECK(hipGraphLaunch(ex[i].exec, act[i]->st));
+                cs_.xq_fused += ex[i].fused;
+            }
             ++passes;
             if (early_exit && (s % 16) == 0) {
                 bool all = true;
@@ -1256,11 +1286,33 @@
                     int* ts_state_out) {
     select();
     require_weights();
+    const char* xq_env = getenv("SPT_XQ_FUSE");
+    xq_on_ = rq.beam_k == 0 && !(xq_env && atoi(xq_env) == 0);
+    struct XqOff {
+        bool& on;
+        ~XqOff() { on = false; }
+    } xq_off{xq_on_};
+    const int fused0 = cs_.xq_fused;
     HIP_CHECK(hipEventRecord(ev_[6], st_));
     run_decode(B, rq, tokens, top1, top2, lang_out, ts_state_out);
     HIP_CHECK(hipEventRecord(ev_[7], st_));
     HIP_CHECK(hipStreamSynchronize(st_));
     HIP_CHECK(hipGetLastError());
+    if (cs_.xq_fused > fused0) {
+        unsigned err = 0;
+        HIP_CHECK(hipMemcpy(&err, xq_err_, 4, hipMemcpyDeviceToHost));
+        const char* force = getenv("SPT_XQ_FUSE_FORCE_FALLBACK");
+        if (err || (force && atoi(force) != 0)) {
+            HIP_CHECK(hipMemset(xq_err_, 0, 4));
+            xq_on_ = false;
+            cs_.xq_fallbacks++;
+            HIP_CHECK(hipEventRecord(ev_[6], st_));
+            run_decode(B, rq, tokens, top1, top2, lang_out, ts_state_out);
+            HIP_CHECK(hipEventRecord(ev_[7], st_));
+            HIP_CHECK(hipStreamSynchronize(st_));
+            HIP_CHECK(hipGetLastError());
+        }
+    }
     tm_.batch = B;
     cs_.engine_calls++;
     cs_.decoder_passes += tm_.n_decode_passes;
@@ -1412,9 +1464,9 @@
             hipGraphExec_t exec;
             HIP_CHECK(hipGraphInstantiate(&exec, graph, nullptr, nullptr, 0));
             HIP_CHECK(hipGraphDestroy(graph));
-            it = g.graphs.emplace(key, exec).first;
-        }
-        HIP_CHECK(hipGraphLaunch(it->second, g.st));
+            it = g.graphs.emplace(key, PassGraph{exec, 0}).first;
+        }
+        HIP_CHECK(hipGraphLaunch(it->second.exec, g.st));
     }
     HIP_CHECK(hipEventRecord(ev_[9], g.st));
     read_cands(B, out);
diff --git a/spittle_amd/csrc/engine.h b/spittle_amd/csrc/engine.h
--- a/spittle_amd/csrc/engine.h
+++ b/spittle_amd/csrc/engine.h
@@ -54,6 +54,8 @@
     int engine_calls = 0, decoder_passes = 0, beam_steps = 0, encoder_windows = 0;
     int pd_passes = 0;
     int pd_fallbacks = 0;
+    int xq_fused = 0;
+    int xq_fallbacks = 0;
     double device_ms = 0, encoder_ms = 0, decode_ms = 0;
 };
 
@@ -107,8 +109,10 @@
         uint32_t flags;
         bool full;
         int share = 0;
+        bool fuse = false;
         bool operator<(const GraphKey& o) const {
             if (full != o.full) return full < o.full;
+            if (fuse != o.fuse) return fuse < o.fuse;
             if (B != o.B) return B < o.B;
             if (share != o.share) return share < o.share;
             if (B_total != o.B_total) return B_total < o.B_total;
@@ -117,6 +121,10 @@
             if (n_forced != o.n_forced) return n_forced < o.n_forced;
             return flags < o.flags;
         }
+    };
+    struct PassGraph {
+        hipGraphExec_t exec;
+        int fused;
     };
     struct DecGroup {
         hipStream_t st = nullptr;
@@ -143,7 +151,8 @@
         float* cand_lp = nullptr;
         int* kvrow = nullptr;
         int share = 0;
-        std::map<GraphKey, hipGraphExec_t> graphs;
+        unsigned long long* xq_gran = nullptr;
+        std::map<GraphKey, PassGraph> graphs;
         std::vector<int> host_tok;
         size_t host_used = 0;
     };
@@ -179,6 +188,10 @@
     static constexpr int fc2_split_ = 2;
     bool pend_fold_ = true;
     void ln_source(GemvArgs& a, float* xc, float* pend, int np, int64_t slab) const;
+    bool xq_on_ = false;
+    int xq_enq_ = 0;
+    int n_cu_ = 0;
+    unsigned* xq_err_ = nullptr;
     int xsplit_ = 1;
     int n_groups_ = 1;
     int max_rows_ = 64;
diff --git a/spittle_amd/csrc/k_dec.hip b/spittle_amd/csrc/k_dec.hip
--- a/spittle_amd/csrc/k_dec.hip
+++ b/spittle_amd/csrc/k_dec.hip
@@ -99,8 +99,9 @@
             a.stamp[2 * (blockIdx.x + blockIdx.y * gridDim.x) + (i)] = __builtin_amdgcn_s_memrealtime(); \
     } while (0)
 
-template <typename T, int MODE, int ASRC, int RG, int NWV, int CT, int MAXJ, bool EXACT = false>
-__global__ __launch_bounds__(64 * NWV) void gemv_kernel(GemvArgs a) {
+template <typename T, int MODE, int ASRC, int RG, int NWV, int CT, int MAXJ, bool EXACT = false, bool PUB = false>
+__device__ __forceinline__ void gemv_body(const GemvArgs& a, unsigned long long* gran = nullptr, unsigned tag = 0) {
+    static_assert(!PUB || (MODE == GV_BIAS && sizeof(T) == 2), "gemv: granules carry one 16-bit GV_BIAS element");
     GV_STAMP(0);
     constexpr int KS = GV<T>::KS;
     constexpr int CPE = 16 / sizeof(T);
@@ -379,7 +380,14 @@
             if (row >= a.R) continue;
             const float y = acc[g][r] + bv;
             if constexpr (MODE == GV_BIAS) {
-                ((T*)a.C)[(size_t)row * a.ldc + n] = from_f<T>(y);
+                const T yt = from_f<T>(y);
+                ((T*)a.C)[(size_t)row * a.ldc + n] = yt;
+                if constexpr (PUB) {
+                    unsigned short bits;
+                    __builtin_memcpy(&bits, &yt, 2);
+                    __hip_atomic_store(gran + (size_t)row * a.N + n, ((unsigned long long)tag << 32) | bits,
+                                       __ATOMIC_RELAXED, __HIP_MEMORY_SCOPE_AGENT);
+                }
             } else if constexpr (MODE == GV_BIAS_GELU) {
                 ((T*)a.C)[(size_t)row * a.ldc + n] = from_f<T>(gelu_tanh(y));
             } else if constexpr (MODE == GV_PARTIAL) {
@@ -403,6 +411,11 @@
         }
     }
     GV_STAMP(1);
+}
+
+template <typename T, int MODE, int ASRC, int RG, int NWV, int CT, int MAXJ, bool EXACT = false>
+__global__ __launch_bounds__(64 * NWV) void gemv_kernel(GemvArgs a) {
+    gemv_body<T, MODE, ASRC, RG, NWV, CT, MAXJ, EXACT>(a);
 }
 
 template <typename T, int MODE, int ASRC, int RG, int NWV, int CT, int MAXJ, bool EXACT = false>
@@ -630,6 +643,88 @@
     }
 }
 
+template <typename T, int TOUCH, int PF = 3>
+__global__ __launch_bounds__(640) void xq_fused_kernel(GemvArgs a, XqFuseArgs x) {
+    const int n_prod = a.N / 16;
+    const unsigned tag =
+        (__hip_atomic_load(&x.ds->epoch, __ATOMIC_RELAXED, __HIP_MEMORY_SCOPE_WORKGROUP) + 1u) * 64u + (unsigned)x.layer;
+    if ((int)blockIdx.x < n_prod) {
+        gemv_body<T, GV_BIAS, LN_SRC(0), 1, 10, 1, 1, true, true>(a, x.gran, tag);
+        return;
+    }
+    typedef AttnWave<T, 1, 0, AW, PF> W;
+    constexpr int MAXB = (1500 / W::KB + 1 + AW - 1) / AW;
+    extern __shared__ __attribute__((aligned(16))) char smem[];
+    float (*s_o)[1][64] = (float (*)[1][64])smem;
+    float (*s_m)[1] = (float (*)[1])(smem + AW * 256);
+    float (*s_l)[1] = (float (*)[1])(smem + AW * 256 + AW * 4);
+    unsigned short* s_q = (unsigned short*)(smem + AW * 256 + AW * 8);
+    int* s_ok = (int*)(smem + AW * 256 + AW * 8 + 128);
+    const int cb = (int)blockIdx.x - n_prod, j = cb / x.H, h = cb - j * x.H;
+    const int tid = threadIdx.x, lane = tid & 63, wid = tid >> 6, g = lane & 7;
+    if (wid > AW) return;
+    const int nblk = cdiv(x.T_enc, W::KB);
+    W aw;
+    unsigned touch[TOUCH > 0 ? TOUCH : 1] = {};
+    if (wid < AW) {
+        const size_t kvo = ((size_t)j * x.H + h) * 4096 + 8 * g;
+        aw.init((const T*)x.kv + kvo, (const T*)x.kv + kvo + 2048, x.T_enc, lane, (int64_t)x.B_layout * x.H * 4096);
+        aw.template ring_fill<MAXB>(wid, nblk);
+        if constexpr (TOUCH > 0) {
+            const T* base = (const T*)x.kv + ((size_t)j * x.H + h) * 4096 + (lane < 32 ? 0 : 2048);
+#pragma unroll
+            for (int t = 0; t < TOUCH; ++t) {
+                const int key = min((wid + (PF - 1 + t) * AW) * W::KB + (lane & 31), x.T_enc - 1);
+                touch[t] = *(const unsigned*)(base + (uint32_t)((key >> 5) * aw.bstride + (key & 31) * 64));
+            }
+        }
+    } else {
+        unsigned long long* gp = x.gran + ((size_t)j * x.H + h) * 64 + lane;
+        bool ok = false;
+        if (__hip_atomic_load(x.err, __ATOMIC_RELAXED, __HIP_MEMORY_SCOPE_AGENT) == 0u) {
+            const long long t0 = wall_clock64();
+            for (;;) {
+                const unsigned long long v = __hip_atomic_load(gp, __ATOMIC_RELAXED, __HIP_MEMORY_SCOPE_AGENT);
+                if (__all((unsigned)(v >> 32) == tag)) {
+                    s_q[lane] = (unsigned short)v;
+                    ok = true;
+                    break;
+                }
+                if (wall_clock64() - t0 > kXqTimeoutTicks) break;
+                __builtin_amdgcn_s_sleep(2);
+            }
+        }
+        if (lane == 0) {
+            *s_ok = ok ? 1 : 0;
+            if (!ok) __hip_atomic_store(x.err, 1u, __ATOMIC_RELAXED, __HIP_MEMORY_SCOPE_AGENT);
+        }
+    }
+    __syncthreads();
+    if (wid >= AW || !*s_ok) return;
+    float qv[1][8];
+    int lim[1] = {x.T_enc};
+#pragma unroll
+    for (int e = 0; e < 8; ++e) {
+        T qt;
+        __builtin_memcpy(&qt, &s_q[8 * g + e], 2);
+        qv[0][e] = to_f<T>(qt) * kLog2Scale;
+    }
+    aw.template ring_run<MAXB>(wid, nblk, qv, lim, 1);
+    aw.to_lds(s_m, s_l, s_o, wid, lane);
+    __syncthreads();
+    if (tid < 64) {
+        float M, L, O;
+        attn_merge<1, AW>(s_m, s_l, s_o, 0, tid, M, L, O);
+        ((T*)x.out)[((size_t)j * x.H + h) * 64 + tid] = from_f<T>(O / L);
+    }
+    if constexpr (TOUCH > 0) {
+        unsigned u = 0;
+#pragma unroll
+        for (int t = 0; t < TOUCH; ++t) u ^= touch[t];
+        if (x.layer < 0 && u == 0x9e3779b9u) __hip_atomic_store(x.err, 2u, __ATOMIC_RELAXED, __HIP_MEMORY_SCOPE_AGENT);
+    }
+}
+
 template <typename T, int NQ, int NIX = 0, int PF = 2>
 __global__ __launch_bounds__(64) void cross_attn_vw_kernel(const T* __restrict__ q, const T* __restrict__ kv,
                                                            int B_layout, int H, int T_enc, int Tq,
@@ -706,6 +801,7 @@
     __shared__ int s_tok;
     const int b = blockIdx.x, tid = threadIdx.x;
     const int step = a.ds->step, pos0 = a.ds->pos0;
+    const unsigned epoch = a.ds->epoch;
     TopP t{-INFINITY, 0x7fffffff, -INFINITY, 0};
     const TopP* p = (const TopP*)a.part + (size_t)b * a.n_tiles;
     for (int i = tid; i < a.n_tiles; i += FIN_T) t = top_merge(t, p[i]);
@@ -750,12 +846,16 @@
         if (prev == (unsigned)gridDim.x - 1) {
             a.ds->pos0 = pos0 + a.Tq;
             a.ds->step = step + 1;
+            a.ds->epoch = epoch + 1u;
             __hip_atomic_store(a.arrive, 0u, __ATOMIC_RELAXED, __HIP_MEMORY_SCOPE_AGENT);
         }
     }
 }
 
-__global__ void advance_kernel(DecState* ds, int n) { ds->pos0 += n; }
+__global__ void advance_kernel(DecState* ds, int n) {
+    ds->pos0 += n;
+    ds->epoch += 1u;
+}
 
 __global__ void reset_kernel(DecState* ds, unsigned* arrive) {
     ds->pos0 = 0;
@@ -909,6 +1009,36 @@
     SPT_LAUNCH_CHECK();
 }
 
+bool dec_xq_fused_ok(int dtype, int B, int d, int H, int T_enc, int n_cu) {
+    static const bool exact_ln = !getenv("GV_EXACT_LN") || atoi(getenv("GV_EXACT_LN")) != 0;
+    return exact_ln && dtype_size(dtype) == 2 && d == 10 * GV<bf16>::KS && H * 64 == d && B >= 1 && B <= 16 &&
+           T_enc >= 256 && cdiv(T_enc, 32) <= 48 && d / 16 + B * H <= n_cu;
+}
+
+void dec_xq_fused(int dtype, const GemvArgs& cq, const XqFuseArgs& x, int B, hipStream_t st) {
+    if (dtype_size(dtype) != 2 || cq.R != B || B < 1 || B > 16 || cq.N != x.H * 64 || cq.K != 10 * GV<bf16>::KS ||
+        cq.N % 16 || cq.n_pend != 0 || !cq.ln_w || !cq.ln_b || !cq.C || x.T_enc < 256 || cdiv(x.T_enc, 32) > 48 ||
+        x.layer < 0 || x.layer >= 64 || !x.kv || !x.out || !x.gran || !x.ds || !x.err)
+        throw std::runtime_error("dec_xq_fused: not the fused launch's shape");
+    for (int p = 0; p < 4; ++p)
+        if (!cq.pend[p]) throw std::runtime_error("dec_xq_fused: LayerNorm prologue needs 4 pending slabs (zero slab if none)");
+    if ((int64_t)cdiv(x.T_enc, 32) * x.B_layout * x.H * 4096 >= (int64_t)INT32_MAX)
+        throw std::runtime_error("dec_xq_fused: a layer's cross K/V exceeds 2^31 elements");
+    GemvArgs a = cq;
+    a.ksplit = 1;
+    const int lds = std::max(4096, gv_img_bytes(a.R, a.K, 2) + 10 * 64 * (int)sizeof(f32x4));
+    const dim3 grid(a.N / 16 + B * x.H), blk(640);
+    static const bool touch = !getenv("SPT_XQ_TOUCH") || atoi(getenv("SPT_XQ_TOUCH")) != 0;
+    if (dtype == DT_BF16) {
+        if (touch) hipLaunchKernelGGL((xq_fused_kernel<bf16, 2>), grid, blk, lds, st, a, x);
+        else hipLaunchKernelGGL((xq_fused_kernel<bf16, 0>), grid, blk, lds, st, a, x);
+    } else {
+        if (touch) hipLaunchKernelGGL((xq_fused_kernel<f16, 2>), grid, blk, lds, st, a, x);
+        else hipLaunchKernelGGL((xq_fused_kernel<f16, 0>), grid, blk, lds, st, a, x);
+    }
+    SPT_LAUNCH_CHECK();
+}
+
 void dec_attn_part_merge(int dtype, const float* part, int R, int H, void* out, hipStream_t st) {
     if (R < 1 || H < 1 || !part || !out) throw std::runtime_error("dec_attn_part_merge: empty or missing buffers");
     if (dtype == DT_BF16) hipLaunchKernelGGL(attn_part_merge_kernel<bf16>, dim3(R * H), dim3(64), 0, st, part, H, (bf16*)out);
diff --git a/spittle_amd/csrc/k_sample.hip b/spittle_amd/csrc/k_sample.hip
--- a/spittle_amd/csrc/k_sample.hip
+++ b/spittle_amd/csrc/k_sample.hip
@@ -289,6 +289,7 @@
     __syncthreads();
     const int tok = s_tok;
     const int pos0 = a.ds->pos0;
+    const unsigned epoch = a.ds->epoch;
     const int pn = min(pos0 + a.Tq, a.ctx - 1);
     const T* e = (const T*)a.emb + (size_t)tok * a.d;
     const float* pp = a.pos + (size_t)pn * a.d;
@@ -298,6 +299,7 @@
         if (prev == (unsigned)gridDim.x - 1) {
             a.ds->pos0 = pos0 + a.Tq;
             a.ds->step = step + 1;
+            a.ds->epoch = epoch + 1u;
             __hip_atomic_store(a.arrive, 0u, __ATOMIC_RELAXED, __HIP_MEMORY_SCOPE_AGENT);
         }
     }
diff --git a/spittle_amd/csrc/kernels.h b/spittle_amd/csrc/kernels.h
--- a/spittle_amd/csrc/kernels.h
+++ b/spittle_amd/csrc/kernels.h
@@ -83,6 +83,7 @@
 struct DecState {
     int pos0;
     int step;
+    unsigned epoch;
 };
 
 enum { GV_BIAS = 0, GV_BIAS_GELU = 1, GV_PARTIAL = 2, GV_QKV_CACHE = 3, GV_LOGITS = 4, GV_BIAS_RESID = 5 };
@@ -119,6 +120,18 @@
                     int share = 1);
 void dec_cross_attn_vw(int dtype, const void* q, const void* kv, int B, int B_layout, int H, int T_enc, int Tq,
                        float* part, hipStream_t st, const int* kvrow = nullptr, int share = 1, bool per_query = false);
+struct XqFuseArgs {
+    const void* kv; int B_layout, H, T_enc;
+    void* out;
+    unsigned long long* gran;
+    const DecState* ds;
+    unsigned* err;
+    int layer;
+};
+constexpr long long kXqTimeoutTicks = 2000000;
+bool dec_xq_fused_ok(int dtype, int B, int d, int H, int T_enc, int n_cu);
+void dec_xq_fused(int dtype, const GemvArgs& cq, const XqFuseArgs& x, int B, hipStream_t st);
+
 void dec_attn_part_merge(int dtype, const float* part, int R, int H, void* out, hipStream_t st);
 
 struct FinalizeArgs {
diff --git a/spittle_amd/engine.py b/spittle_amd/engine.py
--- a/spittle_amd/engine.py
+++ b/spittle_amd/engine.py
@@ -239,6 +239,12 @@
         self._check(self._lib.spt_get_call_stats(self._ctx, C.byref(t)))
         return {k: getattr(t, k) for k, _ in t._fields_ if k != "reserved0"}
 
+    def xq_stats(self) -> dict:
+        self._need()
+        f, b = C.c_int32(0), C.c_int32(0)
+        self._check(self._lib.spt_get_xq_stats(self._ctx, C.byref(f), C.byref(b)))
+        return {"fused_launches": f.value, "fallbacks": b.value}
+
     def debug_mel(self, samples, seek: int = 0) -> np.ndarray:
         self._need()
         x = np.ascontiguousarray(np.asarray(samples, np.float32).reshape(-1))
```

Result: faster. 982.5 audio-sec/wall-sec (median of 6 runs) (+4.1%).
